# seanome/kmerseek

Hardware: AMD Instinct MI355X
Metric: k-mers hashed+matched/sec (higher is better)
Workload: dtype u64

## Files before the change

### include/kmerseek_amd.h

```cpp
#ifndef KMERSEEK_AMD_H
#define KMERSEEK_AMD_H

#include <stddef.h>
#include <stdint.h>

#ifdef __cplusplus
extern "C" {
#endif

#define KS_ABI_VERSION 1

typedef enum ks_status {
    KS_OK = 0,
    KS_ERR_INVALID_MOLTYPE = 1,
    KS_ERR_INVALID_KSIZE = 2,
    KS_ERR_INVALID_RESIDUE = 3,
    KS_ERR_INVALID_ARG = 4,
    KS_ERR_OOM = 5,
    KS_ERR_HIP = 6,
    KS_ERR_NO_DEVICE = 7,
    KS_ERR_CAPACITY = 8,
    KS_ERR_INVALID_SCALED = 9
} ks_status;

typedef enum ks_moltype { KS_PROTEIN = 0, KS_DAYHOFF = 1, KS_HP = 2 } ks_moltype;

#define KS_SEED_DEFAULT 42ull
#define KS_MAX_KSIZE 128u

typedef struct ks_params {
    uint32_t ksize;
    uint32_t scaled;
    uint32_t moltype;
    uint32_t flags;
    uint64_t seed;
} ks_params;

typedef struct ks_ctx ks_ctx;
typedef struct ks_sketches ks_sketches;
typedef struct ks_index ks_index;
typedef struct ks_hits ks_hits;
typedef struct ks_kmerpos ks_kmerpos;
typedef struct ks_matchpos ks_matchpos;
typedef struct ks_regions ks_regions;


uint32_t ks_abi_version(void);
const char *ks_status_string(int status);

int ks_moltype_from_string(const char *name, uint32_t *moltype_out);

uint64_t ks_max_hash(uint32_t scaled);

int ks_ctx_create(int device, void *hip_stream, ks_ctx **out);
void ks_ctx_destroy(ks_ctx *ctx);
const char *ks_last_error(const ks_ctx *ctx);
void *ks_ctx_stream(const ks_ctx *ctx);
int ks_ctx_synchronize(ks_ctx *ctx);
int ks_ctx_pool_stats(const ks_ctx *ctx, uint64_t *n_blocks, uint64_t *bytes_held, uint64_t *bytes_in_use,
                      uint64_t *n_mallocs);

int ks_ctx_sketch_stats(const ks_ctx *ctx, uint64_t out[4]);
int ks_ctx_search_stats(const ks_ctx *ctx, uint64_t out[2]);
int ks_ctx_fused_stats(const ks_ctx *ctx, uint64_t out[2]);
int ks_ctx_qfilter_stats(const ks_ctx *ctx, uint64_t out[2]);
int ks_ctx_reload_debug_env(ks_ctx *ctx);
int ks_debug_guard_selftest(const char *what);

int ks_dev_malloc(ks_ctx *ctx, uint64_t bytes, void **out);
int ks_dev_free(ks_ctx *ctx, void *ptr);
int ks_dev_upload(ks_ctx *ctx, void *dst_device, const void *src_host, uint64_t bytes);
int ks_dev_download(ks_ctx *ctx, void *dst_host, const void *src_device, uint64_t bytes);

int ks_host_alloc(ks_ctx *ctx, uint64_t bytes, void **out);
int ks_host_free(ks_ctx *ctx, void *ptr);


typedef struct ks_residue_error {
    uint32_t seq_index;
    uint32_t position;
    uint8_t residue;
} ks_residue_error;

int ks_validate_and_resolve(const uint8_t *seq, uint64_t len, int upper, uint64_t rng_seed,
                            uint8_t *out, uint64_t *out_len, ks_residue_error *err);


int ks_sketch_batch(ks_ctx *ctx, const uint8_t *residues, const uint64_t *seq_offsets,
                    uint32_t n_seqs, const ks_params *params, ks_sketches **out);

int ks_sketch_batch_device(ks_ctx *ctx, const uint8_t *d_residues, const uint64_t *d_seq_offsets,
                           uint32_t n_seqs, uint64_t n_residues, uint32_t max_seq_len,
                           const ks_params *params, ks_sketches **out);

int ks_sketch_queries_device(ks_ctx *ctx, const ks_index *index, const uint8_t *d_residues,
                             const uint64_t *d_seq_offsets, uint32_t n_seqs, uint64_t n_residues,
                             uint32_t max_seq_len, ks_sketches **out);

int ks_sketch_search_device(ks_ctx *ctx, const ks_index *index, const uint8_t *d_residues,
                            const uint64_t *d_seq_offsets, uint32_t n_seqs, uint64_t n_residues,
                            uint32_t max_seq_len, ks_sketches **sketches_out, ks_hits **hits_out);
int ks_sketch_search(ks_ctx *ctx, const ks_index *index, const uint8_t *residues, const uint64_t *seq_offsets,
                     uint32_t n_seqs, ks_sketches **sketches_out, ks_hits **hits_out);

uint32_t ks_sketches_n_seqs(const ks_sketches *s);
uint64_t ks_sketches_n_hashes(const ks_sketches *s);
uint64_t ks_sketches_n_windows(const ks_sketches *s);
int ks_sketches_has_postings(const ks_sketches *s);
void ks_sketches_params(const ks_sketches *s, ks_params *out);
const uint64_t *ks_sketches_device_offsets(const ks_sketches *s);
const uint64_t *ks_sketches_device_hashes(const ks_sketches *s);
const uint32_t *ks_sketches_device_abunds(const ks_sketches *s);
int ks_sketches_copy_to_host(ks_ctx *ctx, const ks_sketches *s, uint64_t *offsets,
                             uint64_t *hashes, uint32_t *abunds);
int ks_sketches_from_host(ks_ctx *ctx, const uint64_t *offsets, const uint64_t *hashes,
                          const uint32_t *abunds, uint32_t n_seqs, const ks_params *params,
                          ks_sketches **out);
int ks_sketches_union(ks_ctx *ctx, const ks_sketches *in, ks_sketches **out);
void ks_sketches_free(ks_sketches *s);


uint64_t ks_translate6_bound(uint64_t n_nt);
int ks_translate6_device(ks_ctx *ctx, const uint8_t *d_nt, const uint64_t *d_offsets, uint32_t n_seqs, uint64_t n_nt,
                         uint8_t *d_frames ,
                         uint64_t *d_frame_offsets , uint64_t *n_residues_out);
int ks_sketch_translated_device(ks_ctx *ctx, const uint8_t *d_nt, const uint64_t *d_offsets, uint32_t n_seqs, uint64_t n_nt,
                                uint32_t max_seq_len , const ks_params *params, ks_sketches **out);
int ks_sketch_translated(ks_ctx *ctx, const uint8_t *nt, const uint64_t *offsets, uint32_t n_seqs, const ks_params *params,
                         ks_sketches **out);
int ks_sketches_union_groups(ks_ctx *ctx, const ks_sketches *in, const uint32_t *group_offsets, uint32_t n_groups, ks_sketches **out);
uint32_t ks_debug_translate_chunk(void);
uint32_t ks_debug_union_rank_max(void);


int ks_kmer_positions(ks_ctx *ctx, const uint8_t *residues, const uint64_t *seq_offsets,
                      uint32_t n_seqs, const ks_params *params, ks_kmerpos **out);
int ks_kmer_positions_device(ks_ctx *ctx, const uint8_t *d_residues, const uint64_t *d_seq_offsets, uint32_t n_seqs,
                             uint64_t n_residues, const ks_params *params, ks_kmerpos **out);
uint64_t ks_kmerpos_count(const ks_kmerpos *p);
void ks_kmerpos_params(const ks_kmerpos *p, ks_params *out);
int ks_kmerpos_copy_to_host(ks_ctx *ctx, const ks_kmerpos *p, uint32_t *seq, uint32_t *start,
                            uint64_t *hash);
void ks_kmerpos_free(ks_kmerpos *p);


int ks_index_build(ks_ctx *ctx, const ks_sketches *targets, ks_index **out);
uint32_t ks_index_n_targets(const ks_index *ix);
uint64_t ks_index_n_postings(const ks_index *ix);
void ks_index_free(ks_index *ix);

int ks_search(ks_ctx *ctx, const ks_index *index, const ks_sketches *queries, ks_hits **out);
uint64_t ks_hits_count(const ks_hits *h);
uint64_t ks_hits_n_pair_instances(const ks_hits *h);
int ks_hits_partition_path(const ks_hits *h);
int ks_hits_bucket_posting_bytes(const ks_hits *h);
int ks_hits_copy_to_host(ks_ctx *ctx, const ks_hits *h, uint32_t *qid, uint32_t *tid,
                         uint32_t *intersect, uint64_t *n_weighted);
const uint32_t *ks_hits_device_qid(const ks_hits *h);
const uint32_t *ks_hits_device_tid(const ks_hits *h);
const uint32_t *ks_hits_device_intersect(const ks_hits *h);
const uint64_t *ks_hits_device_n_weighted(const ks_hits *h);
int ks_hits_copy_to_device(ks_ctx *ctx, const ks_hits *h, uint32_t qid_base, uint32_t tid_base, uint32_t *d_qid,
                           uint32_t *d_tid, uint32_t *d_intersect, uint64_t *d_n_weighted);
int ks_hits_pack64_to_device(ks_ctx *ctx, const ks_hits *h, uint32_t qid_base, uint32_t tid_base, int qbits, int tbits,
                             uint64_t *d_packed, uint32_t *d_esc_row, uint32_t *d_esc_intersect, uint64_t *d_esc_n_weighted,
                             uint32_t *d_n_esc, uint32_t esc_cap);
int ks_hits_unpack64_device(ks_ctx *ctx, const uint64_t *d_packed, uint64_t n, int qbits, int tbits, uint32_t *d_qid,
                            uint32_t *d_tid, uint32_t *d_intersect, uint64_t *d_n_weighted);
int ks_hits_merge_by_qid_device(ks_ctx *ctx, const uint32_t *d_qid, const uint32_t *d_tid, const uint32_t *d_intersect,
                                const uint64_t *d_n_weighted, const uint64_t *block_rows, uint32_t n_blocks, uint32_t n_queries,
                                uint32_t *d_out_qid, uint32_t *d_out_tid, uint32_t *d_out_intersect, uint64_t *d_out_n_weighted);
void ks_hits_free(ks_hits *h);


#define KS_SEARCH_ABUND_STATS 1u
typedef struct ks_search_opts {
    uint32_t flags;
    uint32_t reserved;
    double min_containment;
} ks_search_opts;
int ks_search_ex(ks_ctx *ctx, const ks_index *index, const ks_sketches *queries, const ks_search_opts *opts, ks_hits **out);
int ks_sketch_search_device_ex(ks_ctx *ctx, const ks_index *index, const uint8_t *d_residues, const uint64_t *d_seq_offsets,
                               uint32_t n_seqs, uint64_t n_residues, uint32_t max_seq_len, const ks_search_opts *opts,
                               ks_sketches **sketches_out, ks_hits **hits_out);
int ks_sketch_search_ex(ks_ctx *ctx, const ks_index *index, const uint8_t *residues, const uint64_t *seq_offsets,
                        uint32_t n_seqs, const ks_search_opts *opts, ks_sketches **sketches_out, ks_hits **hits_out);
int ks_hits_has_abund_stats(const ks_hits *h);
const uint64_t *ks_hits_device_median2(const ks_hits *h);
const double *ks_hits_device_abund_ss(const ks_hits *h);
int ks_hits_copy_abund_stats_to_host(ks_ctx *ctx, const ks_hits *h, uint64_t *median2, double *ss);


typedef struct ks_matchpos_opts {
    uint32_t flags;
    uint32_t reserved;
    uint64_t max_pairs;
} ks_matchpos_opts;
int ks_match_positions(ks_ctx *ctx, const ks_kmerpos *q_pos, const ks_kmerpos *t_pos, const ks_hits *hits,
                       const ks_matchpos_opts *opts, ks_matchpos **out);
uint64_t ks_matchpos_n_rows(const ks_matchpos *m);
uint64_t ks_matchpos_n_pairs(const ks_matchpos *m);
uint32_t ks_matchpos_n_slices(const ks_matchpos *m);
const uint64_t *ks_matchpos_device_row_offsets(const ks_matchpos *m);
const uint32_t *ks_matchpos_device_q_start(const ks_matchpos *m);
const uint32_t *ks_matchpos_device_t_start(const ks_matchpos *m);
const uint32_t *ks_matchpos_device_q_lo(const ks_matchpos *m);
const uint32_t *ks_matchpos_device_q_hi(const ks_matchpos *m);
const uint32_t *ks_matchpos_device_t_lo(const ks_matchpos *m);
const uint32_t *ks_matchpos_device_t_hi(const ks_matchpos *m);
int ks_matchpos_copy_to_host(ks_ctx *ctx, const ks_matchpos *m, uint64_t *row_offsets, uint32_t *q_start, uint32_t *t_start,
                             uint32_t *q_lo, uint32_t *q_hi, uint32_t *t_lo, uint32_t *t_hi);
void ks_matchpos_free(ks_matchpos *m);


typedef struct ks_regions_opts {
    uint32_t flags;
    uint32_t min_kmers;
// ... 129 lines not shown
```

### kmerseek_amd/_lib.py

```python
from __future__ import annotations

import ctypes as C
import os
import sys

HERE = os.path.dirname(os.path.abspath(__file__))
SO_PATH = os.environ.get("KMERSEEK_AMD_LIB") or os.path.join(HERE, "libkmerseek_amd.so")

KS_OK = 0
KS_ERR_INVALID_MOLTYPE = 1
KS_ERR_INVALID_KSIZE = 2
KS_ERR_INVALID_RESIDUE = 3
KS_ERR_INVALID_ARG = 4
KS_ERR_OOM = 5
KS_ERR_HIP = 6
KS_ERR_NO_DEVICE = 7
KS_ERR_CAPACITY = 8
KS_ERR_INVALID_SCALED = 9

KS_PROTEIN, KS_DAYHOFF, KS_HP = 0, 1, 2
KS_SEED_DEFAULT = 42


class ks_params(C.Structure):
    _fields_ = [("ksize", C.c_uint32), ("scaled", C.c_uint32), ("moltype", C.c_uint32),
                ("flags", C.c_uint32), ("seed", C.c_uint64)]


class ks_residue_error(C.Structure):
    _fields_ = [("seq_index", C.c_uint32), ("position", C.c_uint32), ("residue", C.c_uint8)]


KS_SEARCH_ABUND_STATS = 1


class ks_search_opts(C.Structure):
    _fields_ = [("flags", C.c_uint32), ("reserved", C.c_uint32), ("min_containment", C.c_double)]


class ks_matchpos_opts(C.Structure):
    _fields_ = [("flags", C.c_uint32), ("reserved", C.c_uint32), ("max_pairs", C.c_uint64)]


class ks_regions_opts(C.Structure):
    _fields_ = [("flags", C.c_uint32), ("min_kmers", C.c_uint32), ("max_gap", C.c_uint32), ("reserved", C.c_uint32)]


class ks_signif_opts(C.Structure):
    _fields_ = [("flags", C.c_uint32), ("reserved", C.c_uint32)]


KS_BEST_INTERSECT, KS_BEST_TARGET_CONTAINMENT, KS_BEST_MAX_CONTAINMENT, KS_BEST_JACCARD, KS_BEST_SCORE = 0, 1, 2, 3, 4


class ks_best_opts(C.Structure):
    _fields_ = [("rank_by", C.c_uint32), ("k", C.c_uint32), ("flags", C.c_uint32), ("reserved", C.c_uint32)]


class ks_cluster_opts(C.Structure):
    _fields_ = [("similarity", C.c_uint32), ("n_nodes", C.c_uint32), ("threshold", C.c_double), ("flags", C.c_uint32),
                ("reserved", C.c_uint32)]


KS_GREEDY_ASSIGN_FIRST, KS_GREEDY_ASSIGN_BEST = 0, 1


class ks_greedy_opts(C.Structure):
    _fields_ = [("similarity", C.c_uint32), ("n_nodes", C.c_uint32), ("threshold", C.c_double), ("assign", C.c_uint32),
                ("flags", C.c_uint32)]


class ks_gather_opts(C.Structure):
    _fields_ = [("min_unique", C.c_uint32), ("max_results", C.c_uint32), ("flags", C.c_uint32), ("reserved", C.c_uint32)]


class ks_kernel_time(C.Structure):
    _fields_ = [("name", C.c_char * 48), ("launches", C.c_uint64), ("total_ms", C.c_double)]


_vp = C.c_void_p
_u8p = C.POINTER(C.c_uint8)
_u32p = C.POINTER(C.c_uint32)
_u64p = C.POINTER(C.c_uint64)
_pp = C.POINTER(C.c_void_p)
_parp = C.POINTER(ks_params)

SIGNATURES = {
    "ks_abi_version": (C.c_uint32, []),
    "ks_status_string": (C.c_char_p, [C.c_int]),
    "ks_moltype_from_string": (C.c_int, [C.c_char_p, _u32p]),
    "ks_max_hash": (C.c_uint64, [C.c_uint32]),
    "ks_ctx_create": (C.c_int, [C.c_int, _vp, _pp]),
    "ks_ctx_destroy": (None, [_vp]),
    "ks_last_error": (C.c_char_p, [_vp]),
    "ks_ctx_stream": (_vp, [_vp]),
    "ks_ctx_synchronize": (C.c_int, [_vp]),
    "ks_ctx_sketch_stats": (C.c_int, [_vp, C.POINTER(C.c_uint64 * 4)]),
    "ks_ctx_search_stats": (C.c_int, [_vp, C.POINTER(C.c_uint64 * 2)]),
    "ks_ctx_fused_stats": (C.c_int, [_vp, C.POINTER(C.c_uint64 * 2)]),
    "ks_ctx_qfilter_stats": (C.c_int, [_vp, C.POINTER(C.c_uint64 * 2)]),
    "ks_ctx_reload_debug_env": (C.c_int, [_vp]),
    "ks_debug_guard_selftest": (C.c_int, [C.c_char_p]),
    "ks_host_alloc": (C.c_int, [_vp, C.c_uint64, _pp]),
    "ks_host_free": (C.c_int, [_vp, _vp]),
    "ks_dev_malloc": (C.c_int, [_vp, C.c_uint64, _pp]),
    "ks_dev_free": (C.c_int, [_vp, _vp]),
    "ks_dev_upload": (C.c_int, [_vp, _vp, _vp, C.c_uint64]),
    "ks_dev_download": (C.c_int, [_vp, _vp, _vp, C.c_uint64]),
    "ks_ctx_pool_stats": (C.c_int, [_vp, _u64p, _u64p, _u64p, _u64p]),
    "ks_validate_and_resolve": (C.c_int, [C.c_char_p, C.c_uint64, C.c_int, C.c_uint64, C.c_char_p, _u64p,
                                          C.POINTER(ks_residue_error)]),
    "ks_sketch_batch": (C.c_int, [_vp, _vp, _vp, C.c_uint32, _parp, _pp]),
    "ks_sketch_batch_device": (C.c_int, [_vp, _vp, _vp, C.c_uint32, C.c_uint64, C.c_uint32, _parp, _pp]),
    "ks_sketch_queries_device": (C.c_int, [_vp, _vp, _vp, _vp, C.c_uint32, C.c_uint64, C.c_uint32, _pp]),
    "ks_sketch_search_device": (C.c_int, [_vp, _vp, _vp, _vp, C.c_uint32, C.c_uint64, C.c_uint32, _pp, _pp]),
    "ks_sketch_search": (C.c_int, [_vp, _vp, _vp, _vp, C.c_uint32, _pp, _pp]),
    "ks_sketches_has_postings": (C.c_int, [_vp]),
    "ks_sketches_n_seqs": (C.c_uint32, [_vp]),
    "ks_sketches_n_hashes": (C.c_uint64, [_vp]),
    "ks_sketches_n_windows": (C.c_uint64, [_vp]),
    "ks_sketches_params": (None, [_vp, _parp]),
    "ks_sketches_device_offsets": (_vp, [_vp]),
    "ks_sketches_device_hashes": (_vp, [_vp]),
    "ks_sketches_device_abunds": (_vp, [_vp]),
    "ks_sketches_copy_to_host": (C.c_int, [_vp, _vp, _vp, _vp, _vp]),
    "ks_sketches_from_host": (C.c_int, [_vp, _vp, _vp, _vp, C.c_uint32, _parp, _pp]),
    "ks_sketches_union": (C.c_int, [_vp, _vp, _pp]),
    "ks_sketches_free": (None, [_vp]),
    "ks_translate6_bound": (C.c_uint64, [C.c_uint64]),
    "ks_translate6_device": (C.c_int, [_vp, _vp, _vp, C.c_uint32, C.c_uint64, _vp, _vp, _u64p]),
    "ks_sketch_translated_device": (C.c_int, [_vp, _vp, _vp, C.c_uint32, C.c_uint64, C.c_uint32, _parp, _pp]),
    "ks_sketch_translated": (C.c_int, [_vp, _vp, _vp, C.c_uint32, _parp, _pp]),
    "ks_sketches_union_groups": (C.c_int, [_vp, _vp, _u32p, C.c_uint32, _pp]),
    "ks_debug_translate_chunk": (C.c_uint32, []),
    "ks_debug_union_rank_max": (C.c_uint32, []),
    "ks_kmer_positions": (C.c_int, [_vp, _vp, _vp, C.c_uint32, _parp, _pp]),
    "ks_kmer_positions_device": (C.c_int, [_vp, _vp, _vp, C.c_uint32, C.c_uint64, _parp, _pp]),
    "ks_kmerpos_count": (C.c_uint64, [_vp]),
    "ks_kmerpos_params": (None, [_vp, _parp]),
    "ks_kmerpos_copy_to_host": (C.c_int, [_vp, _vp, _vp, _vp, _vp]),
    "ks_kmerpos_free": (None, [_vp]),
    "ks_index_build": (C.c_int, [_vp, _vp, _pp]),
    "ks_index_n_targets": (C.c_uint32, [_vp]),
    "ks_index_n_postings": (C.c_uint64, [_vp]),
    "ks_index_free": (None, [_vp]),
    "ks_search": (C.c_int, [_vp, _vp, _vp, _pp]),
    "ks_hits_count": (C.c_uint64, [_vp]),
    "ks_hits_n_pair_instances": (C.c_uint64, [_vp]),
    "ks_hits_partition_path": (C.c_int, [_vp]),
    "ks_hits_bucket_posting_bytes": (C.c_int, [_vp]),
    "ks_hits_copy_to_host": (C.c_int, [_vp, _vp, _vp, _vp, _vp, _vp]),
    "ks_hits_device_qid": (_vp, [_vp]),
    "ks_hits_device_tid": (_vp, [_vp]),
    "ks_hits_device_intersect": (_vp, [_vp]),
    "ks_hits_device_n_weighted": (_vp, [_vp]),
    "ks_hits_copy_to_device": (C.c_int, [_vp, _vp, C.c_uint32, C.c_uint32, _vp, _vp, _vp, _vp]),
    "ks_hits_pack64_to_device": (C.c_int, [_vp, _vp, C.c_uint32, C.c_uint32, C.c_int, C.c_int, _vp, _vp, _vp, _vp, _vp, C.c_uint32]),
    "ks_hits_unpack64_device": (C.c_int, [_vp, _vp, C.c_uint64, C.c_int, C.c_int, _vp, _vp, _vp, _vp]),
    "ks_hits_merge_by_qid_device": (C.c_int, [_vp, _vp, _vp, _vp, _vp, C.POINTER(C.c_uint64), C.c_uint32, C.c_uint32, _vp, _vp, _vp, _vp]),
    "ks_hits_free": (None, [_vp]),
    "ks_search_ex": (C.c_int, [_vp, _vp, _vp, C.POINTER(ks_search_opts), _pp]),
    "ks_sketch_search_device_ex": (C.c_int, [_vp, _vp, _vp, _vp, C.c_uint32, C.c_uint64, C.c_uint32, C.POINTER(ks_search_opts), _pp,
                                             _pp]),
    "ks_sketch_search_ex": (C.c_int, [_vp, _vp, _vp, _vp, C.c_uint32, C.POINTER(ks_search_opts), _pp, _pp]),
    "ks_hits_has_abund_stats": (C.c_int, [_vp]),
    "ks_hits_device_median2": (_vp, [_vp]),
    "ks_hits_device_abund_ss": (_vp, [_vp]),
    "ks_hits_copy_abund_stats_to_host": (C.c_int, [_vp, _vp, _vp, _vp]),
    "ks_match_positions": (C.c_int, [_vp, _vp, _vp, _vp, C.POINTER(ks_matchpos_opts), _pp]),
    "ks_matchpos_n_rows": (C.c_uint64, [_vp]),
    "ks_matchpos_n_pairs": (C.c_uint64, [_vp]),
    "ks_matchpos_n_slices": (C.c_uint32, [_vp]),
    "ks_matchpos_device_row_offsets": (_vp, [_vp]),
    "ks_matchpos_device_q_start": (_vp, [_vp]),
    "ks_matchpos_device_t_start": (_vp, [_vp]),
    "ks_matchpos_device_q_lo": (_vp, [_vp]),
    "ks_matchpos_device_q_hi": (_vp, [_vp]),
    "ks_matchpos_device_t_lo": (_vp, [_vp]),
    "ks_matchpos_device_t_hi": (_vp, [_vp]),
    "ks_matchpos_copy_to_host": (C.c_int, [_vp, _vp, _vp, _vp, _vp, _vp, _vp, _vp, _vp]),
    "ks_matchpos_free": (None, [_vp]),
    "ks_match_regions": (C.c_int, [_vp, _vp, C.POINTER(ks_regions_opts), _pp]),
    "ks_regions_n_rows": (C.c_uint64, [_vp]),
    "ks_regions_n_regions": (C.c_uint64, [_vp]),
    "ks_regions_n_slices": (C.c_uint32, [_vp]),
    "ks_regions_device_row_offsets": (_vp, [_vp]),
    "ks_regions_device_q_start": (_vp, [_vp]),
    "ks_regions_device_t_start": (_vp, [_vp]),
    "ks_regions_device_length": (_vp, [_vp]),
    "ks_regions_device_n_kmers": (_vp, [_vp]),
    "ks_regions_device_covered": (_vp, [_vp]),
    "ks_regions_copy_to_host": (C.c_int, [_vp, _vp, _vp, _vp, _vp, _vp, _vp, _vp]),
    "ks_regions_free": (None, [_vp]),
    "ks_corpus_build": (C.c_int, [_vp, _vp, _pp]),
    "ks_corpus_n_hashes": (C.c_uint64, [_vp]),
    "ks_corpus_n_docs": (C.c_uint32, [_vp]),
    "ks_corpus_total_abund": (C.c_uint64, [_vp]),
    "ks_corpus_copy_to_host": (C.c_int, [_vp, _vp, _vp, _vp, _vp]),
    "ks_corpus_free": (None, [_vp]),
    "ks_hits_significance": (C.c_int, [_vp, _vp, _vp, _vp, _vp, _vp, C.POINTER(ks_signif_opts), _pp]),
    "ks_signif_n_rows": (C.c_uint64, [_vp]),
    "ks_signif_device_prob_overlap": (_vp, [_vp]),
    "ks_signif_device_tf_idf": (_vp, [_vp]),
    "ks_signif_copy_to_host": (C.c_int, [_vp, _vp, _vp, _vp]),
    "ks_signif_free": (None, [_vp]),
    "ks_hits_best": (C.c_int, [_vp, _vp, _vp, _vp, _vp, C.POINTER(ks_best_opts), _pp]),
    "ks_hits_device_rank": (_vp, [_vp]),
    "ks_hits_device_src_row": (_vp, [_vp]),
    "ks_hits_copy_best_to_host": (C.c_int, [_vp, _vp, _vp, _vp]),
    "ks_hits_gather": (C.c_int, [_vp, _vp, _vp, _vp, C.POINTER(ks_gather_opts), _pp]),
    "ks_hits_device_unique_intersect": (_vp, [_vp]),
    "ks_hits_device_remaining": (_vp, [_vp]),
    "ks_hits_device_unique_weighted": (_vp, [_vp]),
    "ks_hits_copy_gather_to_host": (C.c_int, [_vp, _vp, _vp, _vp, _vp]),
    "ks_hits_cluster": (C.c_int, [_vp, _vp, _vp, _vp, C.POINTER(ks_cluster_opts), _pp]),
    "ks_clusters_n_nodes": (C.c_uint32, [_vp]),
    "ks_clusters_n_clusters": (C.c_uint32, [_vp]),
    "ks_clusters_n_edges": (C.c_uint64, [_vp]),
    "ks_clusters_largest": (C.c_uint32, [_vp]),
    "ks_clusters_device_label": (_vp, [_vp]),
    "ks_clusters_device_cluster_id": (_vp, [_vp]),
    "ks_clusters_device_offsets": (_vp, [_vp]),
    "ks_clusters_device_members": (_vp, [_vp]),
    "ks_clusters_device_representative": (_vp, [_vp]),
    "ks_clusters_copy_to_host": (C.c_int, [_vp, _vp, _vp, _vp, _vp, _vp, _vp]),
    "ks_clusters_free": (None, [_vp]),
    "ks_hits_cluster_greedy": (C.c_int, [_vp, _vp, _vp, _vp, C.POINTER(ks_greedy_opts), _pp]),
    "ks_clusters_n_rounds": (C.c_uint32, [_vp]),
    "ks_debug_greedy_tail_edges": (C.c_uint32, []),
    "ks_timing_enable": (C.c_int, [_vp, C.c_int]),
    "ks_timing_reset": (C.c_int, [_vp]),
    "ks_timing_get": (C.c_int, [_vp, C.POINTER(ks_kernel_time), C.c_uint32, _u32p]),
    "ks_bench_gather_rates": (C.c_int, [_vp, C.POINTER(C.c_double * 2)]),
    "ks_bench_device_rates": (C.c_int, [_vp, C.POINTER(C.c_double), C.POINTER(C.c_double), C.POINTER(C.c_double)]),
}

_lib = None


class KmerseekLibraryError(RuntimeError):
    pass


def load():
    global _lib
    if _lib is not None:
        return _lib
    if not os.path.exists(SO_PATH):
        raise KmerseekLibraryError(
            f"{SO_PATH} not found: build it with `python -m kmerseek_amd.build` (hipcc, gfx950). "
            "There is no CPU fallback.")
    if "torch" not in sys.modules and os.environ.get("KS_NO_TORCH_PRELOAD") != "1":
# ... 18 lines not shown
```

### kmerseek_amd/csrc/ks_api.hip

```cpp
#include "ks_device.h"

extern "C" int ks_sketch_batch_device(ks_ctx *ctx, const uint8_t *d_residues, const uint64_t *d_seq_offsets,
                                      uint32_t n_seqs, uint64_t n_residues, uint32_t max_seq_len,
                                      const ks_params *params, ks_sketches **out) {
    return ks_guard(ctx, [&]() -> int {
    if (!ctx) return KS_ERR_INVALID_ARG;
    if (!out || (!d_seq_offsets) || (!d_residues && n_residues)) return ks_fail(ctx, KS_ERR_INVALID_ARG, "NULL argument");
    return ks_sketch_device_impl(ctx, d_residues, d_seq_offsets, n_seqs, n_residues, max_seq_len, params, 0, 0, 0, out);
    });
}

extern "C" int ks_sketch_queries_device(ks_ctx *ctx, const ks_index *index, const uint8_t *d_residues,
                                        const uint64_t *d_seq_offsets, uint32_t n_seqs, uint64_t n_residues,
                                        uint32_t max_seq_len, ks_sketches **out) {
    return ks_guard(ctx, [&]() -> int {
    if (!ctx) return KS_ERR_INVALID_ARG;
    if (!index || !out || (!d_seq_offsets) || (!d_residues && n_residues)) return ks_fail(ctx, KS_ERR_INVALID_ARG, "NULL argument");
    return ks_sketch_device_impl(ctx, d_residues, d_seq_offsets, n_seqs, n_residues, max_seq_len, &index->params,
                                 index->pbits, (index->fp_layout && index->fp_shift == 32 - index->pbits) ? 1 : 0, 0, out);
    });
}

struct ks_upload {
    ks_ctx *ctx;
// ... 133 lines not shown
    return ks_guard(ctx, [&]() -> int {
    if (!ctx) return KS_ERR_INVALID_ARG;
    if (!offsets || !out) return ks_fail(ctx, KS_ERR_INVALID_ARG, "NULL argument");
    KS_TRY(ks_check_params(ctx, params));
    if (offsets[0] != 0) return ks_fail(ctx, KS_ERR_INVALID_ARG, "offsets[0] must be 0");
    const u64 n = offsets[n_seqs];
    if (n && (!hashes || !abunds)) return ks_fail(ctx, KS_ERR_INVALID_ARG, "hashes/abunds is NULL");
    const u64 max_hash = ks_max_hash(params->scaled);
    for (u32 s = 0; s < n_seqs; s++) {
        if (offsets[s + 1] < offsets[s]) return ks_fail(ctx, KS_ERR_INVALID_ARG, "offsets must be ascending");
        for (u64 j = offsets[s]; j < offsets[s + 1]; j++) {
            if (hashes[j] == 0 || hashes[j] > max_hash)
                return ks_fail(ctx, KS_ERR_INVALID_ARG, "sketch %u holds hash %llu outside (0, max_hash(scaled=%u)]", s,
                               (unsigned long long)hashes[j], params->scaled);
            if (j > offsets[s] && hashes[j] <= hashes[j - 1])
                return ks_fail(ctx, KS_ERR_INVALID_ARG, "sketch %u is not strictly ascending", s);
        }
    }
    KS_HIP(ctx, hipSetDevice(ctx->device));
    ks_result<ks_sketches> S(ctx, out, ks_sketches_free);
    S->params = *params; S->n_seqs = n_seqs; S->n_hashes = S->n_slots = n;
    KS_TRY(ks_alloc(ctx, &S->d_offsets, (size_t)n_seqs + 1));
    KS_TRY(ks_alloc(ctx, &S->d_hashes, (size_t)n));
    KS_TRY(ks_alloc(ctx, &S->d_abunds, (size_t)n));
    KS_HIP(ctx, hipMemcpyAsync(S->d_offsets, offsets, ((size_t)n_seqs + 1) * sizeof(u64), hipMemcpyHostToDevice, ctx->stream));
    if (n) {
        KS_HIP(ctx, hipMemcpyAsync(S->d_hashes, hashes, (size_t)n * sizeof(u64), hipMemcpyHostToDevice, ctx->stream));
        KS_HIP(ctx, hipMemcpyAsync(S->d_abunds, abunds, (size_t)n * sizeof(u32), hipMemcpyHostToDevice, ctx->stream));
    }
    KS_HIP(ctx, hipStreamSynchronize(ctx->stream));
    return S.commit();
    });
}

extern "C" int ks_sketches_union(ks_ctx *ctx, const ks_sketches *in, ks_sketches **out) {
    return ks_guard(ctx, [&]() -> int {
    if (!ctx) return KS_ERR_INVALID_ARG;
    return ks_union_impl(ctx, in, out);
    });
}

extern "C" void ks_sketches_free(ks_sketches *s) {
    if (!s) return;
    ks_pool_free(s->ctx, s->d_offsets);
    ks_pool_free(s->ctx, s->d_hashes);
    ks_pool_free(s->ctx, s->d_abunds);
    ks_pool_free(s->ctx, s->d_counts);
    ks_pool_free(s->ctx, s->part_keys);
    ks_pool_free(s->ctx, s->part_vals);
    if (s->ctl_block) ks_pool_free(s->ctx, s->ctl_block);
    else ks_pool_free(s->ctx, s->part_len);
    delete s;
}

int ks_kmerpos_device_impl(ks_ctx *ctx, const u8 *d_res, const u64 *d_offs, u32 n_seqs, u64 n_res, const ks_params *p,
                           ks_kmerpos **out) {
    KS_TRY(ks_check_params(ctx, p));
    if (((uintptr_t)d_res & 15) != 0) return ks_fail(ctx, KS_ERR_INVALID_ARG, "d_residues must be 16-byte aligned");
    KS_HIP(ctx, hipSetDevice(ctx->device));
    ks_result<ks_kmerpos> K(ctx, out, ks_kmerpos_free);
    K->params = *p; K->n_seqs = n_seqs;
    const size_t cap = (n_res == 0 || n_seqs == 0) ? 1 : (size_t)n_res;
    KS_TRY(ks_alloc(ctx, &K->d_seq, cap));
    KS_TRY(ks_alloc(ctx, &K->d_start, cap));
    KS_TRY(ks_alloc(ctx, &K->d_hash, cap));
    if (n_res != 0 && n_seqs != 0)
        KS_TRY(ks_kmerpos_tiles_launch(ctx, d_res, d_offs, n_seqs, n_res, p, K->d_seq, K->d_start, K->d_hash, &K->n));
    return K.commit();
}

extern "C" int ks_kmer_positions(ks_ctx *ctx, const uint8_t *residues, const uint64_t *seq_offsets, uint32_t n_seqs,
                                 const ks_params *params, ks_kmerpos **out) {
    return ks_guard(ctx, [&]() -> int {
    if (!ctx) return KS_ERR_INVALID_ARG;
    if (!out) return ks_fail(ctx, KS_ERR_INVALID_ARG, "out is NULL");
    KS_TRY(ks_check_params(ctx, params));
    ks_upload U(ctx);
    KS_TRY(U.upload(residues, seq_offsets, n_seqs));
    return ks_kmerpos_device_impl(ctx, U.d_res, U.d_offs, n_seqs, U.n_res, params, out);
    });
}

extern "C" int ks_kmer_positions_device(ks_ctx *ctx, const uint8_t *d_residues, const uint64_t *d_seq_offsets, uint32_t n_seqs,
                                        uint64_t n_residues, const ks_params *params, ks_kmerpos **out) {
    return ks_guard(ctx, [&]() -> int {
    if (!ctx) return KS_ERR_INVALID_ARG;
    if (!out) return ks_fail(ctx, KS_ERR_INVALID_ARG, "out is NULL");
    if (n_seqs && (!d_seq_offsets || (n_residues && !d_residues))) return ks_fail(ctx, KS_ERR_INVALID_ARG, "NULL device buffer");
    return ks_kmerpos_device_impl(ctx, d_residues, d_seq_offsets, n_seqs, n_residues, params, out);
    });
}

extern "C" uint64_t ks_kmerpos_count(const ks_kmerpos *p) { return p ? p->n : 0; }
extern "C" void ks_kmerpos_params(const ks_kmerpos *p, ks_params *out) { if (p && out) *out = p->params; }

extern "C" int ks_kmerpos_copy_to_host(ks_ctx *ctx, const ks_kmerpos *p, uint32_t *seq, uint32_t *start, uint64_t *hash) {
    return ks_guard(ctx, [&]() -> int {
    if (!ctx || !p) return KS_ERR_INVALID_ARG;
    const size_t n = (size_t)p->n;
    return ks_columns_to_host(ctx, {{seq, p->d_seq, n * sizeof(u32)}, {start, p->d_start, n * sizeof(u32)}, {hash, p->d_hash, n * sizeof(u64)}});
    });
}

extern "C" void ks_kmerpos_free(ks_kmerpos *p) {
    if (!p) return;
    ks_pool_free(p->ctx, p->d_seq);
    ks_pool_free(p->ctx, p->d_start);
    ks_pool_free(p->ctx, p->d_hash);
    delete p;
}

extern "C" int ks_index_build(ks_ctx *ctx, const ks_sketches *targets, ks_index **out) {
    return ks_guard(ctx, [&]() -> int {
    if (!ctx) return KS_ERR_INVALID_ARG;
    return ks_index_build_impl(ctx, targets, out);
    });
}
extern "C" uint32_t ks_index_n_targets(const ks_index *ix) { return ix ? ix->n_targets : 0; }
extern "C" uint64_t ks_index_n_postings(const ks_index *ix) { return ix ? ix->n_postings : 0; }
extern "C" void ks_index_free(ks_index *ix) {
    if (!ix) return;
    ks_pool_free(ix->ctx, ix->d_keys);
    ks_pool_free(ix->ctx, ix->d_tids);
    ks_pool_free(ix->ctx, ix->d_abunds);
    ks_pool_free(ix->ctx, ix->d_fp);
    ks_pool_free(ix->ctx, ix->d_post);
    ks_pool_free(ix->ctx, ix->d_bmeta);
    ks_pool_free(ix->ctx, ix->d_presence);
    ks_pool_free(ix->ctx, ix->d_dir);
    delete ix;
}

extern "C" int ks_search(ks_ctx *ctx, const ks_index *index, const ks_sketches *queries, ks_hits **out) {
    return ks_guard(ctx, [&]() -> int {
    if (!ctx) return KS_ERR_INVALID_ARG;
    return ks_search_impl(ctx, index, queries, out);
    });
}
extern "C" int ks_search_ex(ks_ctx *ctx, const ks_index *index, const ks_sketches *queries, const ks_search_opts *opts, ks_hits **out) {
    return ks_guard(ctx, [&]() -> int {
    KS_TRY(ks_search_opts_check(ctx, opts));
    if (!ctx) return KS_ERR_INVALID_ARG;
    return ks_search_impl(ctx, index, queries, out, nullptr, opts);
    });
}
static int sketch_search_impl(ks_ctx *ctx, const ks_index *index, const uint8_t *d_residues, const uint64_t *d_seq_offsets, uint32_t n_seqs,
                              uint64_t n_residues, uint32_t max_seq_len, const ks_search_opts *opts, ks_sketches **sketches_out,
                              ks_hits **hits_out) {
    *hits_out = nullptr;
    if (sketches_out) *sketches_out = nullptr;
    const int fmt10 = (index->fp_layout && index->fp_shift == 32 - index->pbits) ? 1 : 0;
    ks_sketches *S = nullptr;
    ks_hits *H = nullptr;
    int st = ks_sketch_device_impl(ctx, d_residues, d_seq_offsets, n_seqs, n_residues, max_seq_len, &index->params, index->pbits, fmt10,
                                   ks_dbg(ctx, KS_DBG_NO_DEFER) ? 0 : 1, &S);
    if (st != KS_OK) return st;
    const bool deferred = S->pending != 0;
    int redo = 0;
    st = ks_search_impl(ctx, index, S, &H, &redo, opts);
    if (S->pending) {
        const ks_fetch_seg f = ks_sketch_pending_seg(S);
        int r2 = 0;
        int st2 = ks_stream_wait_fetch(ctx, &f, 1);
        if (st2 == KS_OK) st2 = ks_sketch_finish_pending(S, &r2);
        if (st == KS_OK) { st = st2; redo = r2; }
    }
    if (st == KS_OK && redo) {
        ks_hits_free(H); H = nullptr;
        ks_sketches_free(S); S = nullptr;
        ctx->fused_redos++;
        st = ks_sketch_device_impl(ctx, d_residues, d_seq_offsets, n_seqs, n_residues, max_seq_len, &index->params, index->pbits, fmt10, 0, &S);
        if (st == KS_OK) st = ks_search_impl(ctx, index, S, &H, nullptr, opts);
    }
    if (st != KS_OK) { ks_hits_free(H); ks_sketches_free(S); return st; }
    if (deferred) ctx->fused_deferred++;
    *hits_out = H;
    if (sketches_out) *sketches_out = S; else ks_sketches_free(S);
    return KS_OK;
}

extern "C" int ks_sketch_search_device_ex(ks_ctx *ctx, const ks_index *index, const uint8_t *d_residues,
                                          const uint64_t *d_seq_offsets, uint32_t n_seqs, uint64_t n_residues,
                                          uint32_t max_seq_len, const ks_search_opts *opts, ks_sketches **sketches_out,
                                          ks_hits **hits_out) {
    return ks_guard(ctx, [&]() -> int {
    KS_TRY(ks_search_opts_check(ctx, opts));
    if (!ctx) return KS_ERR_INVALID_ARG;
    if (!index || !hits_out || (!d_seq_offsets) || (!d_residues && n_residues)) return ks_fail(ctx, KS_ERR_INVALID_ARG, "NULL argument");
    return sketch_search_impl(ctx, index, d_residues, d_seq_offsets, n_seqs, n_residues, max_seq_len, opts, sketches_out, hits_out);
    });
}
extern "C" int ks_sketch_search_device(ks_ctx *ctx, const ks_index *index, const uint8_t *d_residues,
                                       const uint64_t *d_seq_offsets, uint32_t n_seqs, uint64_t n_residues,
                                       uint32_t max_seq_len, ks_sketches **sketches_out, ks_hits **hits_out) {
    return ks_guard(ctx, [&]() -> int {
    return ks_sketch_search_device_ex(ctx, index, d_residues, d_seq_offsets, n_seqs, n_residues, max_seq_len, nullptr, sketches_out,
                                      hits_out);
    });
}

extern "C" int ks_sketch_search_ex(ks_ctx *ctx, const ks_index *index, const uint8_t *residues, const uint64_t *seq_offsets,
                                   uint32_t n_seqs, const ks_search_opts *opts, ks_sketches **sketches_out, ks_hits **hits_out) {
    return ks_guard(ctx, [&]() -> int {
    KS_TRY(ks_search_opts_check(ctx, opts));
    if (!ctx) return KS_ERR_INVALID_ARG;
    if (!index || !hits_out) return ks_fail(ctx, KS_ERR_INVALID_ARG, "NULL argument");
    ks_upload U(ctx);
    KS_TRY(U.upload(residues, seq_offsets, n_seqs));
    return sketch_search_impl(ctx, index, U.d_res, U.d_offs, n_seqs, U.n_res, U.max_len, opts, sketches_out, hits_out);
    });
}
extern "C" int ks_sketch_search(ks_ctx *ctx, const ks_index *index, const uint8_t *residues, const uint64_t *seq_offsets,
                                uint32_t n_seqs, ks_sketches **sketches_out, ks_hits **hits_out) {
    return ks_guard(ctx, [&]() -> int {
    return ks_sketch_search_ex(ctx, index, residues, seq_offsets, n_seqs, nullptr, sketches_out, hits_out);
    });
}
extern "C" uint64_t ks_hits_count(const ks_hits *h) { return h ? h->n_hits : 0; }
extern "C" uint64_t ks_hits_n_pair_instances(const ks_hits *h) { return h ? h->n_pair_instances : 0; }
extern "C" int ks_hits_partition_path(const ks_hits *h) {
    return ks_guard(nullptr, [&]() -> int { return h ? h->partition_path : -1; 
    });
}
extern "C" int ks_hits_bucket_posting_bytes(const ks_hits *h) {
    return ks_guard(nullptr, [&]() -> int { return h ? h->bucket_posting_bytes : -1;
    });
}
extern "C" int ks_hits_copy_to_host(ks_ctx *ctx, const ks_hits *h, uint32_t *qid, uint32_t *tid, uint32_t *intersect,
                                    uint64_t *n_weighted) {
    return ks_guard(ctx, [&]() -> int {
    if (!ctx || !h) return KS_ERR_INVALID_ARG;
    const size_t n = (size_t)h->n_hits;
    return ks_columns_to_host(ctx, {{qid, h->d_qid, n * sizeof(u32)}, {tid, h->d_tid, n * sizeof(u32)},
                                    {intersect, h->d_isect, n * sizeof(u32)}, {n_weighted, h->d_nw, n * sizeof(u64)}});
    });
}
extern "C" const uint32_t *ks_hits_device_qid(const ks_hits *h) { return h ? h->d_qid : nullptr; }
extern "C" const uint32_t *ks_hits_device_tid(const ks_hits *h) { return h ? h->d_tid : nullptr; }
extern "C" const uint32_t *ks_hits_device_intersect(const ks_hits *h) { return h ? h->d_isect : nullptr; }
extern "C" const uint64_t *ks_hits_device_n_weighted(const ks_hits *h) { return h ? h->d_nw : nullptr; }

__global__ __launch_bounds__(256) void k_copy_add_u32(const u32 *in, u32 *out, u64 n, u32 add) {
    const u64 i = (u64)blockIdx.x * blockDim.x + threadIdx.x;
    if (i < n) out[i] = in[i] + add;
}

extern "C" int ks_hits_copy_to_device(ks_ctx *ctx, const ks_hits *h, uint32_t qid_base, uint32_t tid_base, uint32_t *d_qid,
                                      uint32_t *d_tid, uint32_t *d_intersect, uint64_t *d_n_weighted) {
    return ks_guard(ctx, [&]() -> int {
    if (!ctx || !h) return KS_ERR_INVALID_ARG;
    KS_HIP(ctx, hipSetDevice(ctx->device));
    const u64 n = h->n_hits;
    if (n == 0) return KS_OK;
    const u32 g = (u32)((n + 255) / 256);
    if (d_qid) KS_LAUNCH(ctx, "hits_copy", k_copy_add_u32, g, 256, (const u32 *)h->d_qid, d_qid, n, qid_base);
    if (d_tid) KS_LAUNCH(ctx, "hits_copy", k_copy_add_u32, g, 256, (const u32 *)h->d_tid, d_tid, n, tid_base);
    if (d_intersect) KS_HIP(ctx, hipMemcpyAsync(d_intersect, h->d_isect, (size_t)n * sizeof(u32), hipMemcpyDeviceToDevice, ctx->stream));
    if (d_n_weighted) KS_HIP(ctx, hipMemcpyAsync(d_n_weighted, h->d_nw, (size_t)n * sizeof(u64), hipMemcpyDeviceToDevice, ctx->stream));
    return KS_OK;
    });
}

__global__ __launch_bounds__(256) void k_hits_pack64(const u32 *qid, const u32 *tid, const u32 *isect, const u64 *nw, u64 n, u32 qid_base,
                                                     u32 tid_base, int qbits, int tbits, int vbits, u64 *packed, u32 *esc_row, u32 *esc_isect,
                                                     u64 *esc_nw, u32 *n_esc, u32 esc_cap) {
    const u64 i = (u64)blockIdx.x * blockDim.x + threadIdx.x;
    if (i >= n) return;
    const u64 vmax = (1ULL << vbits) - 1ULL;
    u64 a = isect[i], b = nw[i];
    if (a >= vmax || b >= vmax) {
        const u32 e = atomicAdd(n_esc, 1u);
        if (e < esc_cap) { esc_row[e] = (u32)i; esc_isect[e] = (u32)a; esc_nw[e] = b; }
        a = vmax; b = vmax;
    }
    const u64 q = (u64)qid[i] + qid_base, t = (u64)tid[i] + tid_base;
    if ((q >> qbits) != 0 || (t >> tbits) != 0) atomicOr(n_esc, 0x80000000u);
    packed[i] = (((q << tbits) | t) << (2 * vbits)) | (a << vbits) | b;
}

extern "C" int ks_hits_pack64_to_device(ks_ctx *ctx, const ks_hits *h, uint32_t qid_base, uint32_t tid_base, int qbits, int tbits,
                                        uint64_t *d_packed, uint32_t *d_esc_row, uint32_t *d_esc_intersect, uint64_t *d_esc_n_weighted,
                                        uint32_t *d_n_esc, uint32_t esc_cap) {
    return ks_guard(ctx, [&]() -> int {
    if (!ctx || !h) return KS_ERR_INVALID_ARG;
    if (qbits < 1 || tbits < 1 || qbits + tbits > 48) return ks_fail(ctx, KS_ERR_INVALID_ARG, "pack64: %d + %d id bits leave fewer than 8 value bits", qbits, tbits);
    KS_HIP(ctx, hipSetDevice(ctx->device));
    const u64 n = h->n_hits;
    if (!d_n_esc) return ks_fail(ctx, KS_ERR_INVALID_ARG, "NULL argument");
    KS_HIP(ctx, hipMemsetAsync(d_n_esc, 0, sizeof(u32), ctx->stream));
    if (n == 0) return KS_OK;
    if (n >= 0xffffffffULL) return ks_fail(ctx, KS_ERR_CAPACITY, "pack64: %llu rows (escape rows are 32-bit indices)", (unsigned long long)n);
    if (!d_packed || (esc_cap && (!d_esc_row || !d_esc_intersect || !d_esc_n_weighted))) return ks_fail(ctx, KS_ERR_INVALID_ARG, "NULL argument");
    KS_LAUNCH(ctx, "hits_pack", k_hits_pack64, (u32)((n + 255) / 256), 256, (const u32 *)h->d_qid, (const u32 *)h->d_tid, (const u32 *)h->d_isect,
              (const u64 *)h->d_nw, n, qid_base, tid_base, qbits, tbits, (64 - qbits - tbits) / 2, d_packed, d_esc_row, d_esc_intersect, d_esc_n_weighted,
              d_n_esc, esc_cap);
    return KS_OK;
    });
}

__global__ __launch_bounds__(256) void k_hits_unpack64(const u64 *packed, u64 n, int qbits, int tbits, int vbits, u32 *qid, u32 *tid,
                                                       u32 *isect, u64 *nw) {
    const u64 i = (u64)blockIdx.x * blockDim.x + threadIdx.x;
    if (i >= n) return;
    const u64 w = packed[i], vmax = (1ULL << vbits) - 1ULL;
    qid[i] = (u32)((w >> (tbits + 2 * vbits)) & ((1ULL << qbits) - 1ULL));
    tid[i] = (u32)((w >> (2 * vbits)) & ((1ULL << tbits) - 1ULL));
    isect[i] = (u32)((w >> vbits) & vmax);
    nw[i] = w & vmax;
}

extern "C" int ks_hits_unpack64_device(ks_ctx *ctx, const uint64_t *d_packed, uint64_t n, int qbits, int tbits, uint32_t *d_qid,
                                       uint32_t *d_tid, uint32_t *d_intersect, uint64_t *d_n_weighted) {
    return ks_guard(ctx, [&]() -> int {
    if (!ctx) return KS_ERR_INVALID_ARG;
    if (qbits < 1 || tbits < 1 || qbits + tbits > 48) return ks_fail(ctx, KS_ERR_INVALID_ARG, "unpack64: %d + %d id bits leave fewer than 8 value bits", qbits, tbits);
    if (n == 0) return KS_OK;
    if (!d_packed || !d_qid || !d_tid || !d_intersect || !d_n_weighted) return ks_fail(ctx, KS_ERR_INVALID_ARG, "NULL argument");
    if (n > 0xffffffffULL * 256ULL) return ks_fail(ctx, KS_ERR_INVALID_ARG, "unpack64: too many rows");
    KS_HIP(ctx, hipSetDevice(ctx->device));
    KS_LAUNCH(ctx, "hits_unpack", k_hits_unpack64, (u32)((n + 255) / 256), 256, (const u64 *)d_packed, n, qbits, tbits, (64 - qbits - tbits) / 2,
              d_qid, d_tid, d_intersect, (u64 *)d_n_weighted);
    return KS_OK;
    });
}

struct hm_blocks { u64 base[65]; u32 n; };

__global__ __launch_bounds__(256) void k_hm_starts(const u32 *qid, hm_blocks B, u32 nq, u32 *first) {
// ... 99 lines not shown
```

### kmerseek_amd/csrc/ks_common.h

```cpp
#pragma once

#include <hip/hip_runtime.h>

#include <cstdint>
#include <cstdio>
#include <cstring>
#include <functional>
#include <initializer_list>
#include <new>
#include <stdexcept>
#include <string>
#include <vector>

#include "../../include/kmerseek_amd.h"

typedef uint8_t u8;
typedef uint16_t u16;
typedef uint32_t u32;
typedef uint64_t u64;
typedef int32_t i32;
typedef int64_t i64;

#define KS_WAVE 64

struct ks_pool_block {
    void *ptr;
    size_t size;
    bool in_use;
};

struct ks_timer_slot {
    hipEvent_t a, b;
    int name_id;
};

struct ks_copy_engine;

#define KS_DBG_LIST(X)                                                                                                   \
    X(STAGED_H2D) X(PLAIN_COPIES) X(PAIRS_LSD) X(MSD_LDS_CAP) X(SCAN_3PASS) X(INDEX_LSD) X(JOIN_FP) X(FP_COARSEN)        \
    X(PAIR_LIMIT) X(PBITS_MAX) X(RECORD_BITS) X(ONE_CURSOR) X(JOIN_SEGS) X(JOIN_SEG_CAP) X(JOIN_SPARSE)                \
    X(NO_ROWS_HINT) X(ROWS_TICKET) X(FORCE_ROWS_TICKET_RETRY) X(FORCE_TICKET_RETRY) X(NO_PLAN) X(NO_COMPACT) X(SPAN)      \
    X(NO_PACK) X(PLAN_SYNC) X(TILE_R) X(OUT_CAP) X(POOL_CAP) X(THROW) X(QCAP) X(LOOKBACK_SKIP) X(SYNC_API) X(POSTINGS12) X(POSTINGS10) X(NO_DEFER) X(BUCKET) X(JOIN_SPLIT) X(SUBSHIFT) X(MATCHPOS_ROW_BITS) X(SIGNIF_WAVE_ROWS) X(BEST_PATH) X(REGIONS_ROW_BITS) X(QFILTER) X(QFILTER_OCC) X(CLUSTER_PATH) X(GATHER_PATH) X(GREEDY_PATH) X(UNION_PATH)
enum ks_dbg_id {
#define KS_DBG_ENUM(n) KS_DBG_##n,
    KS_DBG_LIST(KS_DBG_ENUM)
#undef KS_DBG_ENUM
    KS_DBG_COUNT
};
struct ks_debug {
    bool set[KS_DBG_COUNT];
    char val[KS_DBG_COUNT][32];
};
void ks_debug_load(ks_debug *d);

struct ks_ctx {
    int device = 0;
    ks_copy_engine *copy = nullptr;
    hipStream_t stream = nullptr;
    bool own_stream = false;
    int n_cus = 256;
    ks_debug dbg;
    u64 pool_cap = 0;
    std::string err;
    std::vector<ks_pool_block> pool;
    u64 pool_mallocs = 0;
    int timing = 0;
    std::vector<std::string> t_names;
    std::vector<u64> t_launches;
    std::vector<double> t_ms;
    std::vector<ks_timer_slot> t_pending;
    std::vector<std::pair<hipEvent_t, hipEvent_t>> t_free;
    bool t_open = false;
    u64 *h_pin = nullptr;
    u64 pair_cap_hint = 0;
    u64 rows_hint = 0;
    bool sketch_use_ticket = false;
    u64 sketch_ticket_fallbacks = 0, sketch_compact_fallbacks = 0, sketch_cap_fallbacks = 0;
    bool rows_use_ticket = false; u64 rows_ticket_fallbacks = 0;
    u64 fused_deferred = 0, fused_redos = 0;
    u64 join_retries = 0;
    bool qfilter_pays = true;
    u64 qfilter_seen = 0, qfilter_dropped = 0;
    unsigned long long *scan_ring = nullptr;
    u32 *scan_ticket = nullptr;
    u32 scan_ticket_base = 0;
    u8 *d_lut = nullptr;
    unsigned long long *h_flag = nullptr;
    unsigned long long wait_seq = 0;
};

int ks_stream_wait(ks_ctx *ctx);
#define KS_FETCH_MAX 4
struct ks_fetch_seg {
    const void *src;
    u32 *dst;
    u32 rows, row_words, src_stride;
};
static inline ks_fetch_seg ks_fetch_words(const void *src, void *dst, u32 n_words32) { return ks_fetch_seg{src, (u32 *)dst, 1u, n_words32, n_words32}; }
int ks_stream_wait_fetch(ks_ctx *ctx, const ks_fetch_seg *segs, int n);

void *ks_pool_alloc(ks_ctx *ctx, size_t bytes);
void ks_pool_free(ks_ctx *ctx, void *ptr);
void ks_pool_trim(ks_ctx *ctx);

int ks_fail(ks_ctx *ctx, int status, const char *fmt, ...);
static inline const char *ks_dbg(const ks_ctx *ctx, int id) { return (ctx && ctx->dbg.set[id]) ? ctx->dbg.val[id] : nullptr; }

int ks_guard_fail(ks_ctx *ctx, int status, const char *what) noexcept;
void ks_guard_enter(ks_ctx *ctx);
template <typename F>
static inline int ks_guard(ks_ctx *ctx, F &&body) noexcept {
    try {
        ks_guard_enter(ctx);
        return body();
    } catch (const std::bad_alloc &) {
        return ks_guard_fail(ctx, KS_ERR_OOM, "out of host memory (std::bad_alloc)");
    } catch (const std::exception &e) {
        return ks_guard_fail(ctx, KS_ERR_HIP, e.what());
    } catch (...) {
        return ks_guard_fail(ctx, KS_ERR_HIP, "unknown exception");
    }
}

void ks_timer_begin(ks_ctx *ctx, const char *name);
void ks_timer_end(ks_ctx *ctx);

#define KS_HIP(ctx, expr)                                                                          \
    do {                                                                                           \
        hipError_t e__ = (expr);                                                                   \
        if (e__ != hipSuccess)                                                                     \
            return ks_fail(ctx, KS_ERR_HIP, "%s failed: %s (%s:%d)", #expr, hipGetErrorString(e__), \
                           __FILE__, __LINE__);                                                    \
    } while (0)

#define KS_TRY(expr)                        \
    do {                                    \
        int s__ = (expr);                   \
        if (s__ != KS_OK) return s__;       \
    } while (0)

#define KS_LAUNCH(ctx, name, kernel, grid, block, ...)                                   \
    do {                                                                                 \
        ks_timer_begin(ctx, name);                                                       \
        hipLaunchKernelGGL(kernel, dim3(grid), dim3(block), 0, (ctx)->stream, __VA_ARGS__); \
        ks_timer_end(ctx);                                                               \
        KS_HIP(ctx, hipGetLastError());                                                  \
    } while (0)

template <typename T>
static inline int ks_alloc(ks_ctx *ctx, T **out, size_t count) {
    void *p = ks_pool_alloc(ctx, (count ? count : 1) * sizeof(T));
    if (!p) return KS_ERR_OOM;
    *out = (T *)p;
    return KS_OK;
}

struct ks_scratch {
    ks_ctx *ctx;
    void *blk[16];
    int n = 0;
    explicit ks_scratch(ks_ctx *c) : ctx(c) {}
    ks_scratch(const ks_scratch &) = delete;
    ~ks_scratch() { for (int i = 0; i < n; i++) ks_pool_free(ctx, blk[i]); }
    template <typename T> int alloc(T **out, size_t count) {
        if (n == 16) return ks_fail(ctx, KS_ERR_HIP, "internal error: scratch table full");
        KS_TRY(ks_alloc(ctx, out, count));
        blk[n++] = *out;
        return KS_OK;
    }
    void free(void *p) { if (forget(p)) ks_pool_free(ctx, p); }
    template <typename T> T *keep(T *p) { forget(p); return p; }
    bool forget(void *p) {
        for (int i = 0; p && i < n; i++)
            if (blk[i] == p) { blk[i] = blk[--n]; return true; }
        return false;
    }
};

struct ks_ctl {
    u64 *dev = nullptr;
    u64 *host = nullptr;
    u32 n_words = 0;
    int init(ks_ctx *ctx, ks_scratch &sc, u32 pin_slot, u32 n_bad, u32 n_count) {
        n_words = n_bad + n_count;
        host = ctx->h_pin + pin_slot;
        KS_TRY(sc.alloc(&dev, n_words));
        KS_HIP(ctx, hipMemsetAsync(dev, 0xff, n_bad * sizeof(u64), ctx->stream));
        KS_HIP(ctx, hipMemsetAsync(dev + n_bad, 0, n_count * sizeof(u64), ctx->stream));
        return KS_OK;
    }
    unsigned long long *words() const { return (unsigned long long *)dev; }
    u32 *low32(u32 i) const { return (u32 *)(dev + i); }
    ks_fetch_seg fetch() const { return ks_fetch_words(dev, host, 2 * n_words); }
    u64 operator[](u32 i) const { return host[i]; }
    bool bad(u32 i) const { return host[i] != ~0ULL; }
};

template <typename T>
struct ks_result {
    T *obj = nullptr;
    T **out;
    void (*free_fn)(T *);
    ks_result(ks_ctx *ctx, T **out_, void (*f)(T *)) : out(out_), free_fn(f) {
        *out = nullptr;
        obj = new T();
        obj->ctx = ctx;
    }
    ks_result(const ks_result &) = delete;
    ~ks_result() {
        if (!obj) return;
        (void)hipStreamSynchronize(obj->ctx->stream);
        free_fn(obj);
    }
    T *operator->() const { return obj; }
    operator T *() const { return obj; }
    int commit() { *out = obj; obj = nullptr; return KS_OK; }
};

struct ks_sketches {
    ks_ctx *ctx;
    ks_params params;
    u32 n_seqs;
    u64 n_hashes;
    u64 n_windows;
    u64 *d_offsets;
    u64 *d_hashes;
    u32 *d_abunds;
    u32 *d_counts;
    u64 n_slots;
    bool gapped;
    u64 *part_keys;
    u32 *part_vals;
    u32 *part_len;
// ... 46 lines not shown
};

struct __attribute__((aligned(16))) ks_bmeta {
    u64 base;
    u32 slot_mul;
    u32 pad;
};

struct ks_index {
    ks_ctx *ctx;
    ks_params params;
    u32 n_targets;
    u64 n_postings;
    u64 *d_keys;
    u32 *d_tids;
    u32 *d_abunds;
    u32 *d_fp;
    ks_post *d_post;
    ks_bmeta *d_bmeta;
    bool fp_layout;
    int fp_shift;
    u32 max_abund;
    u64 *d_dir;
    int pbits;
    u32 *d_presence;
    u32 pres_K;
    int pres_bits;
};

struct ks_hits {
    ks_ctx *ctx;
    u64 n_hits;
    u64 n_pair_instances;
    int partition_path;
    int bucket_posting_bytes;
    u32 *d_qid, *d_tid, *d_isect;
    u64 *d_nw;
    u64 *d_block;
    bool has_stats;
    u64 *d_median2;
    double *d_ss;
    u32 *d_rank, *d_src_row;
    u32 *d_ga_unique, *d_ga_remaining;
    u64 *d_ga_weighted;
};

struct ks_kmerpos {
    ks_ctx *ctx;
    ks_params params;
    u32 n_seqs;
    u64 n;
    u32 *d_seq, *d_start;
    u64 *d_hash;
};

struct ks_matchpos {
    ks_ctx *ctx;
    ks_params params;
    u64 n_rows, n_pairs;
    u32 n_slices;
    u32 max_qs, max_ts;
    u64 *d_row_offsets;
    u32 *d_qstart, *d_tstart;
    u32 *d_qlo, *d_qhi, *d_tlo, *d_thi;
};

struct ks_regions {
    ks_ctx *ctx;
    u64 n_rows, n_regions;
    u32 n_slices;
    u64 *d_row_offsets;
    u32 *d_qstart, *d_tstart, *d_length, *d_nkmers, *d_covered;
};

struct ks_clusters {
    ks_ctx *ctx;
    u32 n_nodes, n_clusters, largest;
    u64 n_edges;
    u32 n_rounds;
    u32 *d_label, *d_cluster_id, *d_members, *d_rep;
    u64 *d_offsets;
};
enum { CL_BAD_ID = 0, CL_BAD_SIZE = 1, CL_EDGES = 2, CL_CLUSTERS = 3, CL_LARGEST = 4 };
int ks_clusters_alloc(ks_ctx *ctx, ks_clusters *K, u32 n);
struct ks_label_scratch { u32 *root_idx, *sizes; u64 *rep, *ka, *kb; };
int ks_clusters_from_labels(ks_ctx *ctx, ks_clusters *K, const ks_sketches *nodes, const ks_label_scratch &W, const ks_ctl &ctl);
int ks_clusters_finish(ks_ctx *ctx, const char *what, ks_clusters *K, const ks_ctl &ctl);
int ks_cluster_words_check(ks_ctx *ctx, const char *what, u32 similarity, u32 n_nodes, double threshold, const ks_sketches *nodes,
                           const double *d_score);

struct ks_slice_fmt {
    int pt, pqt;
    u32 row0, slice_rows;
};
struct ks_row_slices {
    u64 per_slice, n_slices;
    int low_bits;
    ks_slice_fmt fmt(u64 s, u64 n_rows, int pt) const {
        ks_slice_fmt F;
        F.pt = pt; F.pqt = low_bits;
        F.row0 = (u32)(s * per_slice);
        F.slice_rows = (u32)(n_rows - F.row0 < per_slice ? n_rows - F.row0 : per_slice);
        return F;
    }
};
int ks_key_bits(u64 v);
int ks_row_slices_plan(ks_ctx *ctx, int dbg_id, const char *what, int low_bits, u64 n_rows, ks_row_slices *out);
int ks_sort_live_keys(ks_ctx *ctx, u64 *ka, u64 *kb, u64 n, int nbits, u64 **sorted);

enum : u32 { KS_COLS_RANKED = 1u, KS_COLS_GATHER = 2u };
int ks_hits_alloc_cols(ks_ctx *ctx, ks_hits *H, size_t n, u32 extra);
void ks_hits_inherit(ks_hits *B, const ks_hits *H);
#define KS_RANK_NONE 0xffffffffu
struct ks_gather_cols { const u32 *unique, *remaining; const u64 *weighted; };
int ks_hits_move_ranked(ks_ctx *ctx, const ks_hits *H, u32 n_rows, const u32 *dst, const u32 *rank, u32 cap, ks_hits *B,
                        const ks_gather_cols *ga);
int ks_hits_select_plan(ks_ctx *ctx, const char *what, const ks_hits *H, const ks_sketches *Q, u32 per_query, u32 *n, u64 *cap);
int ks_hits_select_tail(ks_ctx *ctx, const char *what, const ks_hits *H, u32 n_rows, u32 *flags, const u32 *rank, u64 cap,
                        const ks_gather_cols *ga, const ks_ctl &ctl, u32 kept, const std::function<int()> &checks, ks_hits *B);

int ks_scan_u32_to_u64(ks_ctx *ctx, const u32 *in, u64 *out, u64 n);
int ks_scan_status_fetch(ks_ctx *ctx);
int ks_scan_status_check(ks_ctx *ctx);
int ks_stream_wait_fetch_scans(ks_ctx *ctx, std::initializer_list<ks_fetch_seg> segs);
int ks_scan_u32_inplace(ks_ctx *ctx, u32 *data, u64 n, u32 *d_total);

enum { KS_SORT_INDEX = 0, KS_SORT_QPART = 1, KS_SORT_PAIRS = 2 };
struct ks_rs_segments {
    const u32 *len;
    u64 cap;
    u32 regions;
    u32 sub_shift;
};
int ks_radix_sort_u32(ks_ctx *ctx, int tag, const u64 *keys_in, const u32 *vals_in, u64 *ka, u32 *va, u64 *kb, u32 *vb,
                      u64 n, const int *shifts, int n_shifts, u64 **keys_out, u32 **vals_out,
                      const ks_rs_segments *seg = nullptr, u32 pfxK = 0);
int ks_radix_sort_keys(ks_ctx *ctx, int tag, const u64 *keys_in, u64 *ka, u64 *kb, u64 n, const int *shifts, int n_shifts,
                       u64 **keys_out);
#define KS_BSLOT(d, r, n_hi) ((r) * (n_hi) + (d))
#define KS_QF_KEPT 1
int ks_bucket_scatter_u32(ks_ctx *ctx, const u64 *keys_in, const u32 *vals_in, const ks_rs_segments *seg, int shift,
                          u32 pfxK, u64 *bkeys, u32 *bvals, u32 *bcur, u32 bcap, unsigned long long *status, u32 n_hi, int vfmt,
                          const u32 *presence, u32 presK, u32 fix_s);
int ks_index_sort_partitioned(ks_ctx *ctx, const u64 *keys_in, const u64 *vals_in, u64 n, u64 max_hash, u64 *okeys, u32 *otids,
                              u32 *oabunds, u32 *d_max_abund, int *overflowed);
#define KS_MSD_MAX_SEGS 64
struct ks_msd_segs {
    u32 n;
    u32 tile_start[KS_MSD_MAX_SEGS + 1];
    u32 count[KS_MSD_MAX_SEGS];
    u64 seg_cap;
};
int ks_sort_pairs_msd(ks_ctx *ctx, u64 *ka, u64 *kb, u64 n, int lo_bit, int nbits, int *done, const ks_msd_segs *segs = nullptr);
int ks_radix_sort_u64(ks_ctx *ctx, int tag, const u64 *keys_in, const u64 *vals_in, u64 *ka, u64 *va, u64 *kb, u64 *vb,
                      u64 n, const int *shifts, int n_shifts, u64 **keys_out, u64 **vals_out);

struct ks_runs { u64 *keys; u32 *vals; u64 *row_start; u32 n_rows; };
int ks_sorted_runs(ks_ctx *ctx, const ks_sketches *in, ks_scratch &sc, ks_runs *out);
int ks_row_list_alloc(ks_ctx *ctx, ks_scratch &sc, size_t n_rows, u32 **list);
int ks_seg_list_alloc(ks_ctx *ctx, ks_scratch &sc, size_t cap, u32 **list);
int ks_seg_path_knob(const ks_ctx *ctx, int dbg_id, bool *small);
struct ks_rows_in { const ks_sketches *q; u64 n_pairs; int tbits, abits; bool stats; double min_c; };
int ks_search_rows(ks_ctx *ctx, const ks_rows_in &R, ks_hits *H, const u64 *pk);

int ks_sketch_device_impl(ks_ctx *ctx, const u8 *d_res, const u64 *d_offs, u32 n_seqs, u64 n_res,
                          u32 max_seq_len, const ks_params *p, int part_pbits, int part_fmt10, int allow_defer, ks_sketches **out);
int ks_sketch_finish_pending(ks_sketches *S, int *redo);
ks_fetch_seg ks_sketch_pending_seg(const ks_sketches *S);
int ks_join_pbits(const ks_ctx *ctx, u64 n_postings, u64 per_bucket);
u32 ks_join_prefix_mul(int pbits, u64 max_hash);
struct sk_args;
struct ks_deferred { u32 *med_ids, *long_ids, *n_cls; u64 *lg_hash; u32 *lg_abund; };
int ks_sketch_long_launch(ks_ctx *ctx, const sk_args &A, const ks_deferred &D, u64 n_long, u32 max_len, ks_scratch &sc);
int ks_sketch_place_launch(ks_ctx *ctx, const sk_args &A, const ks_deferred &D, u64 n_med, u64 n_long);
int ks_kmerpos_tiles_launch(ks_ctx *ctx, const u8 *d_res, const u64 *d_offs, u32 n_seqs, u64 n_res, const ks_params *p, u32 *d_seq,
                            u32 *d_start, u64 *d_hash, u64 *n_out);
int ks_kmerpos_device_impl(ks_ctx *ctx, const u8 *d_res, const u64 *d_offs, u32 n_seqs, u64 n_res,
                           const ks_params *p, ks_kmerpos **out);
int ks_index_build_impl(ks_ctx *ctx, const ks_sketches *t, ks_index **out);
int ks_search_impl(ks_ctx *ctx, const ks_index *ix, const ks_sketches *q, ks_hits **out, int *sketch_redo = nullptr,
                   const ks_search_opts *opts = nullptr);
int ks_search_opts_check(ks_ctx *ctx, const ks_search_opts *opts);
int ks_union_impl(ks_ctx *ctx, const ks_sketches *in, ks_sketches **out);
int ks_union_groups_impl(ks_ctx *ctx, const ks_sketches *in, const u32 *group_offsets, u32 n_groups, ks_sketches **out);
int ks_sketch_translated_impl(ks_ctx *ctx, const u8 *d_nt, const u64 *d_offs, u32 n_seqs, u64 n_nt, u32 max_seq_len, const ks_params *p,
                              ks_sketches **out);

int ks_check_params(ks_ctx *ctx, const ks_params *p);
bool ks_same_params(const ks_params &a, const ks_params &b);
int ks_params_check_same(ks_ctx *ctx, const char *pass, const char *noun, const ks_params &a, const ks_params &b);
template <typename... In>
static inline int ks_inputs_check_ctx(ks_ctx *ctx, const char *pass, const In *...in) {
    if (((!in || in->ctx == ctx) && ...)) return KS_OK;
    return ks_fail(ctx, KS_ERR_INVALID_ARG, "%s: an input of another context", pass);
}
int ks_opts_words_check(ks_ctx *ctx, const char *what, u32 flags, u32 allowed, u32 reserved);
int ks_sketches_make_dense(ks_ctx *ctx, ks_sketches *s);

int ks_copy_h2d(ks_ctx *ctx, void *dst_device, const void *src_host, size_t bytes);
int ks_copy_d2h(ks_ctx *ctx, void *dst_host, const void *src_device, size_t bytes);
struct ks_column { void *dst; const void *src; size_t bytes; };
int ks_columns_to_host(ks_ctx *ctx, std::initializer_list<ks_column> cols);
void ks_copy_engine_destroy(ks_ctx *ctx);
```

### kmerseek_amd/csrc/ks_ctx.hip

```cpp
#include <cstdarg>
#include <algorithm>

#include "ks_common.h"

int ks_fail(ks_ctx *ctx, int status, const char *fmt, ...) {
    char buf[512];
    va_list ap;
    va_start(ap, fmt);
    vsnprintf(buf, sizeof buf, fmt, ap);
    va_end(ap);
    if (ctx) {
        try { ctx->err = buf; } catch (...) { }
    }
    return status;
}

extern "C" uint32_t ks_abi_version(void) { return KS_ABI_VERSION; }

extern "C" const char *ks_status_string(int s) {
    switch (s) {
    case KS_OK: return "ok";
    case KS_ERR_INVALID_MOLTYPE: return "invalid moltype";
    case KS_ERR_INVALID_KSIZE: return "invalid k-mer size";
    case KS_ERR_INVALID_RESIDUE: return "invalid amino acid";
// ... 60 lines not shown
                case 'C': e = 'a'; break;
                case 'A': case 'G': case 'P': case 'S': case 'T': e = 'b'; break;
                case 'D': case 'E': case 'N': case 'Q': e = 'c'; break;
                case 'H': case 'K': case 'R': e = 'd'; break;
                case 'I': case 'L': case 'M': case 'V': e = 'e'; break;
                case 'F': case 'W': case 'Y': e = 'f'; break;
                default: e = 'X';
                }
            } else if (m == KS_HP) {
                switch (c) {
                case 'A': case 'F': case 'G': case 'I': case 'L': case 'M': case 'P': case 'V':
                case 'W': case 'Y': e = 'h'; break;
                case 'N': case 'C': case 'S': case 'T': case 'D': case 'E': case 'R': case 'H':
                case 'K': case 'Q': e = 'p'; break;
                default: e = 'X';
                }
            }
            lut[m * 256 + b] = e;
        }
}

void ks_debug_load(ks_debug *d) {
    static const char *const names[KS_DBG_COUNT] = {
#define KS_DBG_NAME(n) "KS_DEBUG_" #n,
        KS_DBG_LIST(KS_DBG_NAME)
#undef KS_DBG_NAME
    };
    for (int i = 0; i < KS_DBG_COUNT; i++) {
        const char *v = getenv(names[i]);
        d->set[i] = v != nullptr;
        d->val[i][0] = 0;
        if (v) { strncpy(d->val[i], v, sizeof d->val[i] - 1); d->val[i][sizeof d->val[i] - 1] = 0; }
    }
}
static void debug_apply(ks_ctx *ctx) {
    ks_debug_load(&ctx->dbg);
    const char *cap = ks_dbg(ctx, KS_DBG_POOL_CAP);
    ctx->pool_cap = cap ? strtoull(cap, nullptr, 10) : 0;
}
extern "C" int ks_ctx_reload_debug_env(ks_ctx *ctx) {
    if (!ctx) return KS_ERR_INVALID_ARG;
    debug_apply(ctx);
    return KS_OK;
}

int ks_guard_fail(ks_ctx *ctx, int status, const char *what) noexcept {
    if (ctx) {
        try {
            ctx->err.assign(status == KS_ERR_OOM ? "" : "internal error: ");
            ctx->err.append(what ? what : "?");
        } catch (...) {
        }
    }
    return status;
}
void ks_guard_enter(ks_ctx *ctx) {
    const char *t = ks_dbg(ctx, KS_DBG_THROW);
    if (!t) return;
    if (!strcmp(t, "bad_alloc")) throw std::bad_alloc();
    if (!strcmp(t, "runtime")) throw std::runtime_error("KS_DEBUG_THROW");
    if (!strcmp(t, "other")) throw 42;
}

extern "C" int ks_debug_guard_selftest(const char *what) {
    return ks_guard(nullptr, [&]() -> int {
        if (what && !strcmp(what, "bad_alloc")) { std::vector<char> v; v.reserve((size_t)-1 / 2); }
        if (what && !strcmp(what, "runtime")) throw std::runtime_error("selftest");
        if (what && !strcmp(what, "other")) throw 42;
        return KS_OK;
    });
}

extern "C" int ks_ctx_create(int device, void *hip_stream, ks_ctx **out) {
    if (!out) return KS_ERR_INVALID_ARG;
    *out = nullptr;
    int n = 0;
    if (hipGetDeviceCount(&n) != hipSuccess || n <= 0) return KS_ERR_NO_DEVICE;
    if (device < 0 || device >= n) return KS_ERR_INVALID_ARG;
    ks_ctx *ctx = new (std::nothrow) ks_ctx();
    if (!ctx) return KS_ERR_OOM;
    ctx->device = device;
    try { ctx->err.reserve(640); ctx->pool.reserve(256); } catch (...) { delete ctx; return KS_ERR_OOM; }
    debug_apply(ctx);
    if (hipSetDevice(device) != hipSuccess) { delete ctx; return KS_ERR_HIP; }
    hipDeviceProp_t prop;
    if (hipGetDeviceProperties(&prop, device) == hipSuccess) ctx->n_cus = prop.multiProcessorCount;
    if (hip_stream) {
        ctx->stream = (hipStream_t)hip_stream;
    } else {
        if (hipStreamCreateWithFlags(&ctx->stream, hipStreamNonBlocking) != hipSuccess) { delete ctx; return KS_ERR_HIP; }
        ctx->own_stream = true;
    }
    if (hipHostMalloc((void **)&ctx->h_pin, KS_PIN_WORDS * sizeof(u64), hipHostMallocCoherent) != hipSuccess) { delete ctx; return KS_ERR_HIP; }
    if (hipHostMalloc((void **)&ctx->h_flag, 64, hipHostMallocCoherent) != hipSuccess) { (void)hipGetLastError(); ctx->h_flag = nullptr; }
    else *ctx->h_flag = 0;
    if (hipMalloc((void **)&ctx->d_lut, 3 * 256) != hipSuccess) { delete ctx; return KS_ERR_OOM; }
    u8 lut[768];
    build_luts(lut);
    if (hipMemcpy(ctx->d_lut, lut, sizeof lut, hipMemcpyHostToDevice) != hipSuccess) { delete ctx; return KS_ERR_HIP; }
    *out = ctx;
    return KS_OK;
}

extern "C" void ks_ctx_destroy(ks_ctx *ctx) {
    if (!ctx) return;
    (void)hipSetDevice(ctx->device);
    (void)hipStreamSynchronize(ctx->stream);
    ks_copy_engine_destroy(ctx);
    for (auto &t : ctx->t_pending) { (void)hipEventDestroy(t.a); (void)hipEventDestroy(t.b); }
    for (auto &t : ctx->t_free) { (void)hipEventDestroy(t.first); (void)hipEventDestroy(t.second); }
    for (auto &b : ctx->pool) (void)hipFree(b.ptr);
    if (ctx->d_lut) (void)hipFree(ctx->d_lut);
    if (ctx->h_pin) (void)hipHostFree(ctx->h_pin);
    if (ctx->h_flag) (void)hipHostFree(ctx->h_flag);
    if (ctx->scan_ring) (void)hipFree(ctx->scan_ring);
    if (ctx->scan_ticket) (void)hipFree(ctx->scan_ticket);
    if (ctx->own_stream) (void)hipStreamDestroy(ctx->stream);
    delete ctx;
}

extern "C" const char *ks_last_error(const ks_ctx *ctx) { return ctx ? ctx->err.c_str() : "no context"; }
extern "C" void *ks_ctx_stream(const ks_ctx *ctx) { return ctx ? (void *)ctx->stream : nullptr; }
extern "C" int ks_ctx_synchronize(ks_ctx *ctx) {
    return ks_guard(ctx, [&]() -> int {
    if (!ctx) return KS_ERR_INVALID_ARG;
    KS_HIP(ctx, hipStreamSynchronize(ctx->stream));
    return KS_OK;
    });
}

extern "C" int ks_ctx_pool_stats(const ks_ctx *ctx, uint64_t *n_blocks, uint64_t *bytes_held, uint64_t *bytes_in_use,
                                 uint64_t *n_mallocs) {
    return ks_guard((ks_ctx *)ctx, [&]() -> int {
    if (!ctx) return KS_ERR_INVALID_ARG;
    u64 held = 0, used = 0;
    for (auto &b : ctx->pool) { held += b.size; if (b.in_use) used += b.size; }
    if (n_blocks) *n_blocks = ctx->pool.size();
    if (bytes_held) *bytes_held = held;
    if (bytes_in_use) *bytes_in_use = used;
    if (n_mallocs) *n_mallocs = ctx->pool_mallocs;
    return KS_OK;
    });
}

extern "C" int ks_ctx_sketch_stats(const ks_ctx *ctx, uint64_t out[4]) {
    return ks_guard((ks_ctx *)ctx, [&]() -> int {
    if (!ctx || !out) return KS_ERR_INVALID_ARG;
    out[0] = ctx->sketch_ticket_fallbacks; out[1] = ctx->sketch_use_ticket ? 1 : 0;
    out[2] = ctx->sketch_compact_fallbacks; out[3] = ctx->sketch_cap_fallbacks;
    return KS_OK;
    });
}

extern "C" int ks_ctx_search_stats(const ks_ctx *ctx, uint64_t out[2]) {
    return ks_guard((ks_ctx *)ctx, [&]() -> int {
    if (!ctx || !out) return KS_ERR_INVALID_ARG;
    out[0] = ctx->join_retries; out[1] = ctx->rows_ticket_fallbacks;
    return KS_OK;
    });
}

extern "C" int ks_ctx_qfilter_stats(const ks_ctx *ctx, uint64_t out[2]) {
    return ks_guard((ks_ctx *)ctx, [&]() -> int {
    if (!ctx || !out) return KS_ERR_INVALID_ARG;
    out[0] = ctx->qfilter_seen; out[1] = ctx->qfilter_dropped;
    return KS_OK;
    });
}

extern "C" int ks_ctx_fused_stats(const ks_ctx *ctx, uint64_t out[2]) {
    return ks_guard((ks_ctx *)ctx, [&]() -> int {
    if (!ctx || !out) return KS_ERR_INVALID_ARG;
    out[0] = ctx->fused_deferred; out[1] = ctx->fused_redos;
    return KS_OK;
    });
}

extern "C" int ks_dev_malloc(ks_ctx *ctx, uint64_t bytes, void **out) {
    return ks_guard(ctx, [&]() -> int {
    if (!ctx || !out) return KS_ERR_INVALID_ARG;
    KS_HIP(ctx, hipSetDevice(ctx->device));
    if (hipMalloc(out, bytes ? bytes : 256) != hipSuccess) { (void)hipGetLastError(); return ks_fail(ctx, KS_ERR_OOM, "hipMalloc(%llu) failed", (unsigned long long)bytes); }
    return KS_OK;
    });
}
extern "C" int ks_dev_free(ks_ctx *ctx, void *ptr) {
    return ks_guard(ctx, [&]() -> int {
    if (!ctx) return KS_ERR_INVALID_ARG;
    KS_HIP(ctx, hipStreamSynchronize(ctx->stream));
    KS_HIP(ctx, hipFree(ptr));
    return KS_OK;
    });
}
extern "C" int ks_dev_upload(ks_ctx *ctx, void *dst, const void *src, uint64_t bytes) {
    return ks_guard(ctx, [&]() -> int {
    if (!ctx || (bytes && (!dst || !src))) return KS_ERR_INVALID_ARG;
    KS_HIP(ctx, hipSetDevice(ctx->device));
    KS_TRY(ks_copy_h2d(ctx, dst, src, (size_t)bytes));
    KS_HIP(ctx, hipStreamSynchronize(ctx->stream));
    return KS_OK;
    });
}
extern "C" int ks_dev_download(ks_ctx *ctx, void *dst, const void *src, uint64_t bytes) {
    return ks_guard(ctx, [&]() -> int {
    if (!ctx || (bytes && (!dst || !src))) return KS_ERR_INVALID_ARG;
    KS_HIP(ctx, hipSetDevice(ctx->device));
    KS_TRY(ks_copy_d2h(ctx, dst, src, (size_t)bytes));
    KS_HIP(ctx, hipStreamSynchronize(ctx->stream));
    return KS_OK;
    });
}

__global__ void k_host_stamp(unsigned long long *flag, unsigned long long seq) {
    __hip_atomic_store(flag, seq, __ATOMIC_RELEASE, __HIP_MEMORY_SCOPE_SYSTEM);
}
struct ks_fetch_args { ks_fetch_seg seg[KS_FETCH_MAX]; int n; };
__global__ __launch_bounds__(256) void k_host_report(ks_fetch_args F, unsigned long long *flag, unsigned long long seq) {
    for (int s = 0; s < F.n; s++) {
        const ks_fetch_seg g = F.seg[s];
        const u32 total = g.rows * g.row_words;
        for (u32 i = threadIdx.x; i < total; i += blockDim.x) {
            const u32 r = i / g.row_words, c = i - r * g.row_words;
            const u32 v = __hip_atomic_load((const u32 *)g.src + (size_t)r * g.src_stride + c, __ATOMIC_RELAXED, __HIP_MEMORY_SCOPE_AGENT);
            __hip_atomic_store(g.dst + i, v, __ATOMIC_RELAXED, __HIP_MEMORY_SCOPE_SYSTEM);
        }
    }
    __threadfence_system();
    __syncthreads();
    if (threadIdx.x == 0) __hip_atomic_store(flag, seq, __ATOMIC_RELEASE, __HIP_MEMORY_SCOPE_SYSTEM);
}

static int stream_wait_poll(ks_ctx *ctx, unsigned long long seq);

int ks_stream_wait_fetch(ks_ctx *ctx, const ks_fetch_seg *segs, int n) {
    if (n > KS_FETCH_MAX) return ks_fail(ctx, KS_ERR_INVALID_ARG, "too many fetch segments");
    if (!ctx->h_flag || ks_dbg(ctx, KS_DBG_SYNC_API)) {
        for (int i = 0; i < n; i++) {
            const ks_fetch_seg &g = segs[i];
            if (g.rows == 1 || g.src_stride == g.row_words)
                KS_HIP(ctx, hipMemcpyAsync(g.dst, g.src, (size_t)g.rows * g.row_words * sizeof(u32), hipMemcpyDeviceToHost, ctx->stream));
            else
                KS_HIP(ctx, hipMemcpy2DAsync(g.dst, (size_t)g.row_words * sizeof(u32), g.src, (size_t)g.src_stride * sizeof(u32),
                                            (size_t)g.row_words * sizeof(u32), g.rows, hipMemcpyDeviceToHost, ctx->stream));
        }
        KS_HIP(ctx, hipStreamSynchronize(ctx->stream));
        return KS_OK;
    }
    ks_fetch_args F;
    memset(&F, 0, sizeof F);
    for (int i = 0; i < n; i++) F.seg[i] = segs[i];
    F.n = n;
    const unsigned long long seq = ++ctx->wait_seq;
    hipLaunchKernelGGL(k_host_report, dim3(1), dim3(256), 0, ctx->stream, F, ctx->h_flag, seq);
    if (hipGetLastError() != hipSuccess) return ks_fail(ctx, KS_ERR_HIP, "k_host_report launch failed");
    return stream_wait_poll(ctx, seq);
}

int ks_stream_wait(ks_ctx *ctx) {
    if (!ctx->h_flag || ks_dbg(ctx, KS_DBG_SYNC_API)) {
        KS_HIP(ctx, hipStreamSynchronize(ctx->stream));
        return KS_OK;
    }
    const unsigned long long seq = ++ctx->wait_seq;
    hipLaunchKernelGGL(k_host_stamp, dim3(1), dim3(1), 0, ctx->stream, ctx->h_flag, seq);
    if (hipGetLastError() != hipSuccess) { KS_HIP(ctx, hipStreamSynchronize(ctx->stream)); return KS_OK; }
    return stream_wait_poll(ctx, seq);
}

static int stream_wait_poll(ks_ctx *ctx, unsigned long long seq) {
    for (unsigned spins = 1;; spins++) {
        if (__atomic_load_n(ctx->h_flag, __ATOMIC_ACQUIRE) == seq) return KS_OK;
        if ((spins & 0xfffu) == 0) {
            const hipError_t q = hipStreamQuery(ctx->stream);
            if (q == hipSuccess) {
                if (__atomic_load_n(ctx->h_flag, __ATOMIC_ACQUIRE) == seq) return KS_OK;
                KS_HIP(ctx, hipStreamSynchronize(ctx->stream));
                return KS_OK;
            }
            if (q != hipErrorNotReady) return ks_fail(ctx, KS_ERR_HIP, "stream failed: %s", hipGetErrorString(q));
            if (spins > (1u << 26)) { KS_HIP(ctx, hipStreamSynchronize(ctx->stream)); return KS_OK; }
        }
#if defined(__x86_64__)
        __builtin_ia32_pause();
#endif
    }
}

static size_t pool_class(size_t bytes) {
    if (bytes <= 4096) return (bytes + 255) & ~(size_t)255;
    const int e = 63 - __builtin_clzll((unsigned long long)(bytes - 1));
    const size_t step = (size_t)1 << (e - 2);
    return (bytes + step - 1) & ~(step - 1);
}

void *ks_pool_alloc(ks_ctx *ctx, size_t bytes) {
    if (bytes == 0) bytes = 256;
    const size_t want = pool_class(bytes);
    for (size_t i = 0; i < ctx->pool.size(); i++) {
        auto &b = ctx->pool[i];
        if (!b.in_use && b.size == want) { b.in_use = true; return b.ptr; }
    }
    if (ctx->pool_cap) {
        size_t held = 0;
        for (auto &b : ctx->pool) held += b.size;
        if (held + want > ctx->pool_cap) {
            ks_fail(ctx, KS_ERR_OOM, "device pool cap: %zu bytes held, %zu wanted, cap %llu", held, want, (unsigned long long)ctx->pool_cap);
            return nullptr;
        }
    }
    void *p = nullptr;
    hipError_t e = hipMalloc(&p, want);
    if (e != hipSuccess) {
        (void)hipGetLastError();
        int best = -1;
        for (size_t i = 0; i < ctx->pool.size(); i++) {
            auto &b = ctx->pool[i];
            if (!b.in_use && b.size >= want && (best < 0 || b.size < ctx->pool[best].size)) best = (int)i;
        }
        if (best >= 0) { ctx->pool[best].in_use = true; return ctx->pool[best].ptr; }
        ks_pool_trim(ctx);
        e = hipMalloc(&p, want);
    }
    if (e != hipSuccess) {
        (void)hipGetLastError();
        ks_fail(ctx, KS_ERR_OOM, "hipMalloc(%zu) failed: %s", want, hipGetErrorString(e));
        return nullptr;
// ... 259 lines not shown
```

### kmerseek_amd/csrc/ks_msd.hip

```cpp
#include <type_traits>

#include "ks_device.h"

#define MS_THREADS 512
#define MS_IPT 16
#define MS_TILE (MS_THREADS * MS_IPT)
#define MS_WAVES (MS_THREADS / 64)
static_assert(MS_TILE == 8192, "ks_search.hip counts the level-1 tiles of a segmented list in units of 8192 records");
#define MS_SUB 8u

template <int NB>
KS_DEV u32 ms_digit(u64 key, int shift, u32 base, u32 mask) {
    if constexpr (NB == 256) return (u32)(key >> shift) & 255u;
    else return ((u32)(key >> shift) & mask) - base;
}
template <int NB>
KS_DEV u32 ms_base(const u64 *keys, u64 tile_base, int shift, u32 mask, int bits2) {
    if constexpr (NB == 256) return 0u;
    else return (((u32)(keys[tile_base] >> shift) & mask) >> bits2) << bits2;
}

template <int SEG>
KS_DEV void ms_tile_range(u32 t, u64 n, const ks_msd_segs &S, u64 *base, u32 *nvalid) {
    if constexpr (SEG == 0) {
// ... 176 lines not shown
            if (r < nr) {
                const u32 li = (u32)r * 64 + lane;
                const u32 d = li < nb ? ((u32)(key[r] >> shift) & mask) : 255u;
                rank[r] = ks_match8_rank(d, wc);
            }
        }
        __builtin_amdgcn_wave_barrier();
        {
            const uint4 c = *(const uint4 *)&wc[4 * lane];
            const u32 tot = c.x + c.y + c.z + c.w;
            u32 ex = ks_wave_incl_scan(tot) - tot;
            uint4 o;
            o.x = ex; ex += c.x; o.y = ex; ex += c.y; o.z = ex; ex += c.z; o.w = ex;
            *(uint4 *)&wc[4 * lane] = o;
        }
        __builtin_amdgcn_wave_barrier();
#pragma unroll
        for (int r = 0; r < ML_IPT; r++)
            if (r < nr) wstage[wc[rank[r] >> 16] + (rank[r] & 0xffffu)] = key[r];
        __builtin_amdgcn_wave_barrier();
#pragma unroll
        for (int r = 0; r < ML_IPT; r++) {
            const u32 li = (u32)r * 64 + lane;
            if (r < nr) key[r] = li < nb ? wstage[li] : ~0ULL;
        }
        __builtin_amdgcn_wave_barrier();
    }
#pragma unroll
    for (int r = 0; r < ML_IPT; r++) {
        const u32 li = (u32)r * 64 + lane;
        if (r < nr && li < nb) keys[s + li] = key[r];
    }
}

__global__ __launch_bounds__(ML_THREADS) void k_msd_local(u64 *keys, const u32 *off, u32 n_buckets, int lo_bit, int rem_bits, u32 lds_cap,
                                                          u32 *big ) {
    __shared__ u32 wcnt[ML_WAVES][256];
    __shared__ __attribute__((aligned(16))) u64 stage[ML_CAP];
    const u32 lane = threadIdx.x & 63, wave = threadIdx.x >> 6;
    if (rem_bits <= 0) return;
    const u32 wave_cap = lds_cap < ML_WCAP ? lds_cap : ML_WCAP;
    const u32 bw = blockIdx.x * ML_WAVES + wave;
    if (bw < n_buckets) {
        const u64 s = bw ? off[bw - 1] : 0, nb64 = (u64)off[bw] - s;
        if (nb64 > 1 && nb64 <= wave_cap) ml_sort_wave(keys, s, (u32)nb64, lo_bit, rem_bits, wcnt[wave], stage + wave * ML_WCAP, lane);
        else if (nb64 > wave_cap && lane == 0) big[1 + atomicAdd(&big[0], 1u)] = bw;
    }
}

__global__ __launch_bounds__(ML_THREADS) void k_msd_local_big(u64 *keys, u64 *scratch, const u32 *off, const u32 *big, int lo_bit, int rem_bits,
                                                              u32 lds_cap) {
    __shared__ u32 wcnt[ML_WAVES][256];
    __shared__ u32 dcount[256], dstart[256], cursor[256];
    __shared__ u32 scan_smem[ML_WAVES + 1];
    __shared__ __attribute__((aligned(16))) u64 stage[ML_CAP];
    const u32 tid = threadIdx.x, lane = tid & 63, wave = tid >> 6;
    if (rem_bits <= 0) return;
    const int n_pass = (rem_bits + 7) / 8;
    const u32 wloc = wave * (64 * ML_IPT);
    const u32 n_big = big[0];
    for (u32 w = blockIdx.x; w < n_big; w += gridDim.x) {
        const u32 bb = big[1 + w];
        const u64 s = bb ? off[bb - 1] : 0, e = off[bb];
        const u64 nb64 = e - s;
        __syncthreads();
        u64 key[ML_IPT];
        u32 rank[ML_IPT];
        if (nb64 <= lds_cap) {
            const u32 nb = (u32)nb64;
#pragma unroll
            for (int r = 0; r < ML_IPT; r++) {
                const u32 li = wloc + (u32)r * 64 + lane;
                key[r] = li < nb ? keys[s + li] : ~0ULL;
            }
            for (int p = 0; p < n_pass; p++) {
                const int shift = lo_bit + 8 * p;
                const u32 mask = (rem_bits - 8 * p) >= 8 ? 255u : ((1u << (rem_bits - 8 * p)) - 1u);
                for (int ww = 0; ww < ML_WAVES; ww++) wcnt[ww][tid] = 0;
                __syncthreads();
                ml_rank(key, rank, nb, wloc, lane, wave, shift, mask, wcnt);
                __syncthreads();
                ml_offsets(wcnt, dcount, dstart, scan_smem);
                __syncthreads();
#pragma unroll
                for (int r = 0; r < ML_IPT; r++) stage[wcnt[wave][rank[r] >> 16] + (rank[r] & 0xffffu)] = key[r];
                __syncthreads();
#pragma unroll
                for (int r = 0; r < ML_IPT; r++) {
                    const u32 li = wloc + (u32)r * 64 + lane;
                    key[r] = li < nb ? stage[li] : ~0ULL;
                }
                __syncthreads();
            }
#pragma unroll
            for (int r = 0; r < ML_IPT; r++) {
                const u32 li = wloc + (u32)r * 64 + lane;
                if (li < nb) keys[s + li] = key[r];
            }
            continue;
        }
        u64 *src = keys + s, *dst = scratch + s;
        for (int p = 0; p < n_pass; p++) {
            const int shift = lo_bit + 8 * p;
            const u32 mask = (rem_bits - 8 * p) >= 8 ? 255u : ((1u << (rem_bits - 8 * p)) - 1u);
            cursor[tid] = 0;
            __syncthreads();
            for (u64 t0 = 0; t0 < nb64; t0 += ML_CAP)
                for (u32 i = tid; i < ML_CAP && t0 + i < nb64; i += ML_THREADS) atomicAdd(&cursor[(u32)(src[t0 + i] >> shift) & mask], 1u);
            __syncthreads();
            {
                u32 total;
                const u32 ex = ks_block_excl_scan(cursor[tid], scan_smem, &total);
                __syncthreads();
                cursor[tid] = ex;
            }
            __syncthreads();
            for (u64 t0 = 0; t0 < nb64; t0 += ML_CAP) {
                const u32 nv = (nb64 - t0) < ML_CAP ? (u32)(nb64 - t0) : ML_CAP;
#pragma unroll
                for (int r = 0; r < ML_IPT; r++) {
                    const u32 li = wloc + (u32)r * 64 + lane;
                    key[r] = li < nv ? src[t0 + li] : ~0ULL;
                }
                for (int ww = 0; ww < ML_WAVES; ww++) wcnt[ww][tid] = 0;
                __syncthreads();
                ml_rank(key, rank, nv, wloc, lane, wave, shift, mask, wcnt);
                __syncthreads();
                ml_offsets(wcnt, dcount, dstart, scan_smem);
                __syncthreads();
#pragma unroll
                for (int r = 0; r < ML_IPT; r++) {
                    const u32 li = wloc + (u32)r * 64 + lane;
                    if (li < nv) {
                        const u32 d = rank[r] >> 16;
                        dst[(u64)cursor[d] + (wcnt[wave][d] - dstart[d]) + (rank[r] & 0xffffu)] = key[r];
                    }
                }
                __syncthreads();
                if (tid == mask && nv < ML_CAP) dcount[mask] -= ML_CAP - nv;
                __syncthreads();
                cursor[tid] += dcount[tid];
                __syncthreads();
            }
            __threadfence();
            __syncthreads();
            u64 *t = src; src = dst; dst = t;
        }
        if (src != keys + s) {
            for (u64 i = tid; i < nb64; i += ML_THREADS) dst[i] = src[i];
        }
    }
}

int ks_sort_pairs_msd(ks_ctx *ctx, u64 *ka, u64 *kb, u64 n, int lo_bit, int nbits, int *done, const ks_msd_segs *segs) {
    *done = 0;
    if (nbits <= 16 || n < 65536 || n >= 0xffffffffULL || ks_dbg(ctx, KS_DBG_PAIRS_LSD)) return KS_OK;
    int bits2 = 0;
    while (bits2 < 9 && (n >> (8 + bits2)) > (bits2 < 8 ? 768u : 560u)) bits2++;
    for (int b = bits2 + 1; b <= 8 && nbits - 8 - b > 0; b++)
        if ((nbits - 8 - b + 7) / 8 < (nbits - 8 - bits2 + 7) / 8) { bits2 = b; break; }
    if (nbits - 8 - bits2 <= 0) bits2 = nbits - 9 > 0 ? nbits - 9 : 0;
    const int shift1 = lo_bit + nbits - 8, shift2 = shift1 - bits2;
    const u32 mask2 = (1u << (8 + bits2)) - 1u, n_buckets = 1u << (8 + bits2);
    const u32 n_tiles = (u32)((n + MS_TILE - 1) / MS_TILE);
    const u32 n_tiles1 = segs ? segs->tile_start[segs->n] : n_tiles;
    ks_msd_segs no_segs;
    no_segs.n = 0;
    u32 lds_cap = ML_CAP;
    if (const char *f = ks_dbg(ctx, KS_DBG_MSD_LDS_CAP)) {
        const u32 v = (u32)atoi(f);
        if (v >= 2 && v < ML_CAP) lds_cap = v;
    }
    u32 *blk = nullptr;
    const u32 n_sub = bits2 > 0 ? MS_SUB : 1u, sub_stride = bits2 > 0 ? 256u : 0u;
    const size_t off2_words = bits2 > 0 ? (size_t)n_buckets + 1 : 0, n_zero = 256 * MS_SUB + off2_words + 1;
    int st = ks_alloc(ctx, &blk, n_zero + (size_t)(n_buckets > 65536u ? n_buckets : 65536u) + 1);
    u32 *off1 = blk, *off2 = blk ? blk + 256 * MS_SUB : nullptr, *big = blk ? blk + 256 * MS_SUB + off2_words : nullptr;
    u64 *sorted_in = ka;
    if (st == KS_OK) {
        (void)hipMemsetAsync(blk, 0, n_zero * sizeof(u32), ctx->stream);
        ks_timer_begin(ctx, "msd_hist");
        if (segs) hipLaunchKernelGGL((k_msd_hist<256, 1>), dim3(n_tiles1), dim3(MS_THREADS), 0, ctx->stream, (const u64 *)ka, n, shift1, off1, 255u, 0, sub_stride, *segs);
        else hipLaunchKernelGGL((k_msd_hist<256, 0>), dim3(n_tiles), dim3(MS_THREADS), 0, ctx->stream, (const u64 *)ka, n, shift1, off1, 255u, 0, sub_stride, no_segs);
        ks_timer_end(ctx);
        ks_timer_begin(ctx, "msd_scan");
        hipLaunchKernelGGL(k_msd_scan256, dim3(1), dim3(256), 0, ctx->stream, off1, n_sub);
        ks_timer_end(ctx);
        ks_timer_begin(ctx, "msd_scatter");
        if (segs) hipLaunchKernelGGL((k_msd_scatter<256, 1>), dim3(n_tiles1), dim3(MS_THREADS), 0, ctx->stream, (const u64 *)ka, kb, n, shift1, off1, 255u, 0,
                                     sub_stride, *segs);
        else hipLaunchKernelGGL((k_msd_scatter<256, 0>), dim3(n_tiles), dim3(MS_THREADS), 0, ctx->stream, (const u64 *)ka, kb, n, shift1, off1, 255u, 0,
                                sub_stride, no_segs);
        ks_timer_end(ctx);
        sorted_in = kb;
    }
    const u32 *off = off1;
    if (st == KS_OK && bits2 > 0) {
        ks_timer_begin(ctx, "msd_hist");
        if (bits2 <= 8) hipLaunchKernelGGL((k_msd_hist<512>), dim3(n_tiles), dim3(MS_THREADS), 0, ctx->stream, (const u64 *)kb, n, shift2, off2, mask2, bits2, 0u, no_segs);
        else hipLaunchKernelGGL((k_msd_hist<1024>), dim3(n_tiles), dim3(MS_THREADS), 0, ctx->stream, (const u64 *)kb, n, shift2, off2, mask2, bits2, 0u, no_segs);
        ks_timer_end(ctx);
        st = ks_scan_u32_inplace(ctx, off2, n_buckets, nullptr);
        if (st == KS_OK) {
            ks_timer_begin(ctx, "msd_scatter");
            if (bits2 <= 8) hipLaunchKernelGGL((k_msd_scatter<512>), dim3(n_tiles), dim3(MS_THREADS), 0, ctx->stream, (const u64 *)kb, ka, n, shift2, off2, mask2, bits2, 0u, no_segs);
            else hipLaunchKernelGGL((k_msd_scatter<1024>), dim3(n_tiles), dim3(MS_THREADS), 0, ctx->stream, (const u64 *)kb, ka, n, shift2, off2, mask2, bits2, 0u, no_segs);
            ks_timer_end(ctx);
            sorted_in = ka;
            off = off2;
        }
    }
    if (st == KS_OK) {
        u64 *other = sorted_in == ka ? kb : ka;
        ks_timer_begin(ctx, "msd_local");
        hipLaunchKernelGGL(k_msd_local, dim3((n_buckets + ML_WAVES - 1) / ML_WAVES), dim3(ML_THREADS), 0, ctx->stream, sorted_in, off,
                           n_buckets, lo_bit, shift2 - lo_bit, lds_cap, big);
        ks_timer_end(ctx);
        ks_timer_begin(ctx, "msd_local_big");
        hipLaunchKernelGGL(k_msd_local_big, dim3(n_buckets < 2048 ? n_buckets : 2048), dim3(ML_THREADS), 0, ctx->stream, sorted_in, other, off,
                           (const u32 *)big, lo_bit, shift2 - lo_bit, lds_cap);
        ks_timer_end(ctx);
        if (sorted_in != ka)
            if (hipMemcpyAsync(ka, kb, (size_t)n * sizeof(u64), hipMemcpyDeviceToDevice, ctx->stream) != hipSuccess)
                st = ks_fail(ctx, KS_ERR_HIP, "msd sort: copy back failed");
        if (st == KS_OK && hipGetLastError() != hipSuccess) st = ks_fail(ctx, KS_ERR_HIP, "msd sort launch failed");
        if (st == KS_OK) *done = 1;
    }
    ks_pool_free(ctx, blk);
    return st;
}
```

### kmerseek_amd/csrc/ks_rows.hip

```cpp
#include "ks_device.h"

__global__ __launch_bounds__(256) void k_pair_heads(const u64 *keys, u64 n, u32 *heads) {
    u64 i = (u64)blockIdx.x * blockDim.x + threadIdx.x;
    if (i >= n) return;
    heads[i] = (i == 0 || keys[i] != keys[i - 1]) ? 1u : 0u;
}

__global__ __launch_bounds__(256) void k_pair_rows(const u64 *keys, const u32 *hidx, u64 n, u32 n_rows, u64 *row_start) {
    u64 i = (u64)blockIdx.x * blockDim.x + threadIdx.x;
    if (i >= n) return;
    bool head = (i == 0) || keys[i] != keys[i - 1];
    if (head) row_start[hidx[i]] = i;
    if (i == 0) row_start[n_rows] = n;
}

int ks_sorted_runs(ks_ctx *ctx, const ks_sketches *in, ks_scratch &sc, ks_runs *out) {
    const u64 n = in->n_hashes;
    u64 *k0 = nullptr, *k1 = nullptr;
    u32 *v0 = nullptr, *v1 = nullptr, *heads = nullptr, *d_nrows = nullptr;
    KS_TRY(sc.alloc(&k0, (size_t)n)); KS_TRY(sc.alloc(&k1, (size_t)n));
    KS_TRY(sc.alloc(&v0, (size_t)n)); KS_TRY(sc.alloc(&v1, (size_t)n));
    const int shifts[8] = {0, 8, 16, 24, 32, 40, 48, 56};
    KS_TRY(ks_radix_sort_u32(ctx, KS_SORT_PAIRS, in->d_hashes, in->d_abunds, k0, v0, k1, v1, n, shifts, 8, &out->keys, &out->vals));
    KS_TRY(sc.alloc(&heads, (size_t)n));
    KS_TRY(sc.alloc(&d_nrows, 1));
    const u32 g = (u32)((n + 255) / 256);
    KS_LAUNCH(ctx, "run_heads", k_pair_heads, g, 256, (const u64 *)out->keys, n, heads);
    KS_TRY(ks_scan_u32_inplace(ctx, heads, n, d_nrows));
    u64 *const rb = ctx->h_pin + KS_PIN_READ;
    KS_HIP(ctx, hipMemcpyAsync(rb, d_nrows, sizeof(u32), hipMemcpyDeviceToHost, ctx->stream));
    KS_TRY(ks_scan_status_fetch(ctx));
    KS_HIP(ctx, hipStreamSynchronize(ctx->stream));
    KS_TRY(ks_scan_status_check(ctx));
    const u32 n_rows = *(u32 *)rb;
    if (n_rows == 0 || n_rows > n) return ks_fail(ctx, KS_ERR_HIP, "internal error: %u runs in %llu sorted postings", n_rows, (unsigned long long)n);
    out->n_rows = n_rows;
    KS_TRY(sc.alloc(&out->row_start, (size_t)n_rows + 1));
    KS_LAUNCH(ctx, "run_starts", k_pair_rows, g, 256, (const u64 *)out->keys, (const u32 *)heads, n, n_rows, out->row_start);
    return KS_OK;
}

#define PF_THREADS 256
#define PF_IPT 8
#define PF_TILE (PF_THREADS * PF_IPT)
#define PF_WAVES (PF_THREADS / 64)

__global__ __launch_bounds__(PF_THREADS) void k_pair_rows_fused(const u64 *keys, u64 n, u32 *qid, u32 *tid, u32 *isect, unsigned long long *nw,
                                                                int tbits, int abits, u32 rows_cap, unsigned long long *status,
                                                                u32 *ticket , u32 *n_rows_out,
                                                                int use_ticket) {
    __shared__ u32 tile_s;
    __shared__ u32 wcount[PF_IPT][PF_WAVES];
    __shared__ unsigned long long base_s;
    const u32 tid_ = threadIdx.x, lane = tid_ & 63, wave = tid_ >> 6;
    if (use_ticket) {
        if (tid_ == 0) tile_s = atomicAdd(&ticket[0], 1u);
        __syncthreads();
    }
    const u32 tile = use_ticket ? tile_s : blockIdx.x;
    const u64 b0 = (u64)tile * PF_TILE;
    u64 key[PF_IPT];
    u32 headbits = 0;
#pragma unroll
    for (int r = 0; r < PF_IPT; r++) {
        const u64 i = b0 + (u64)r * PF_THREADS + tid_;
        key[r] = i < n ? keys[i] : 0;
    }
    u64 pp = 0;
    {
        const u64 iw = b0 + (u64)lane * PF_THREADS + (tid_ & ~63u);
        if (lane < PF_IPT && iw > 0 && iw < n) pp = keys[iw - 1];
    }
#pragma unroll
    for (int r = 0; r < PF_IPT; r++) {
        const u64 i = b0 + (u64)r * PF_THREADS + tid_;
        const u64 below = ((u64)ks_lane_below((u32)(key[r] >> 32)) << 32) | ks_lane_below((u32)key[r]);
        const u64 first = ((u64)(u32)__builtin_amdgcn_readlane((int)(u32)(pp >> 32), r) << 32) | (u32)__builtin_amdgcn_readlane((int)(u32)pp, r);
        const u64 prev = lane ? below : first;
        const bool head = i < n && (i == 0 || (prev >> abits) != (key[r] >> abits));
        headbits |= head ? (1u << r) : 0u;
        const u64 m = __ballot(head);
        if (lane == 0) wcount[r][wave] = (u32)__popcll(m);
    }
    __syncthreads();
    if (wave == 0) {
        const u32 c = lane < PF_IPT * PF_WAVES ? wcount[lane / PF_WAVES][lane % PF_WAVES] : 0u;
        const u32 incl = ks_wave_incl_scan(c);
        const u32 total = (u32)__builtin_amdgcn_readlane((int)incl, 63);
        if (lane < PF_IPT * PF_WAVES) wcount[lane / PF_WAVES][lane % PF_WAVES] = incl - c;
        if (lane == 0)
            __hip_atomic_store(&status[tile], (tile == 0 ? KS_LB_PRE : KS_LB_AGG) | (u64)total, __ATOMIC_RELAXED, __HIP_MEMORY_SCOPE_AGENT);
        u64 excl = 0;
        if (tile > 0) {
            excl = ks_lookback_walk(tile, lane, ks_lookback_words(status), &ticket[1]);
            if (lane == 0)
                __hip_atomic_store(&status[tile], KS_LB_PRE | (excl + total), __ATOMIC_RELAXED, __HIP_MEMORY_SCOPE_AGENT);
        }
        if (lane == 0) {
            base_s = excl;
            if (b0 + PF_TILE >= n) *n_rows_out = (u32)(excl + total);
        }
    }
    __syncthreads();
    const u64 base = base_s;
#pragma unroll
    for (int r = 0; r < PF_IPT; r++) {
        const u64 i = b0 + (u64)r * PF_THREADS + tid_;
        const bool live = i < n;
        const bool head = (headbits >> r) & 1u;
        const u64 m = __ballot(head);
        const u64 row64 = base + wcount[r][wave] + ks_lane_lt_count(m) + (head ? 1u : 0u) - 1u;
        const u32 row = live ? (u32)row64 : 0xffffffffu;
        u64 w = live ? (key[r] & ((1ULL << abits) - 1ULL)) : 0;
        u32 c = live ? 1u : 0u;
        if (head && row < rows_cap) {
            const u64 ids = key[r] >> abits;
            qid[row] = (u32)(ids >> tbits);
            tid[row] = (u32)(ids & ((1ULL << tbits) - 1ULL));
        }
        {
            const u32 rowx = row ^ 1u;
            u32 wl = (u32)w, wh = (u32)(w >> 32);
#define PF_SEG_STEP(CTRL, RMASK) do { \
                const u32 orow = (u32)__builtin_amdgcn_update_dpp((int)rowx, (int)row, CTRL, RMASK, 0xf, false); \
                const u32 oc = (u32)__builtin_amdgcn_update_dpp(0, (int)c, CTRL, RMASK, 0xf, false); \
                const u32 ol = (u32)__builtin_amdgcn_update_dpp(0, (int)wl, CTRL, RMASK, 0xf, false); \
                const u32 oh = (u32)__builtin_amdgcn_update_dpp(0, (int)wh, CTRL, RMASK, 0xf, false); \
                const bool same = orow == row; \
                const u64 nw_ = (((u64)wh << 32) | wl) + (same ? (((u64)oh << 32) | ol) : 0ULL); \
                c += same ? oc : 0u; wl = (u32)nw_; wh = (u32)(nw_ >> 32); } while (0)
            PF_SEG_STEP(0x111, 0xf);
            PF_SEG_STEP(0x112, 0xf);
            PF_SEG_STEP(0x114, 0xf);
            PF_SEG_STEP(0x118, 0xf);
            PF_SEG_STEP(0x142, 0xa);
            PF_SEG_STEP(0x143, 0xc);
#undef PF_SEG_STEP
            w = ((u64)wh << 32) | wl;
        }
        const u32 nrow = (u32)__builtin_amdgcn_update_dpp((int)(row ^ 1u), (int)row, 0x130, 0xf, 0xf, false);
        if (live && (lane == 63 || nrow != row) && row < rows_cap) {
            atomicAdd(&isect[row], c);
            atomicAdd(&nw[row], (unsigned long long)w);
        }
    }
}

#define RA_LONG 64

__global__ __launch_bounds__(256) void k_row_abund_stats(const u64 *pk, const u64 *row_start, const u32 *isect, const u32 *n_rows_dev,
                                                         u32 rows_cap, int abits, u64 *median2, double *ss, u32 *long_rows) {
#pragma clang fp contract(off)
    const u32 r = blockIdx.x * blockDim.x + threadIdx.x;
    const u32 n_rows = *n_rows_dev < rows_cap ? *n_rows_dev : rows_cap;
    if (r >= n_rows) return;
    const u32 n = isect[r];
    const u64 *a = pk + row_start[r];
    const u64 am = (1ULL << abits) - 1ULL;
    if (n > RA_LONG) { ks_row_list_push(long_rows, r); return; }
    if (n == 0) { median2[r] = 0; ss[r] = 0.0; return; }
    double sum = 0.0;
    for (u32 j = 0; j < n; j++) sum += (double)(a[j] & am);
    const double mean = sum / (double)n;
    double acc = 0.0;
    for (u32 j = 0; j < n; j++) {
        const double d = (double)(a[j] & am) - mean;
        acc += d * d;
    }
    ss[r] = acc;
    median2[r] = (n & 1u) ? 2ULL * (a[n / 2] & am) : (a[n / 2 - 1] & am) + (a[n / 2] & am);
}

__global__ __launch_bounds__(256) void k_row_abund_stats_long(const u64 *pk, const u64 *row_start, const u32 *isect, const u32 *long_rows,
                                                              u32 rows_cap, int abits, u64 *median2, double *ss) {
    const u32 lane = threadIdx.x & 63;
    const u64 am = (1ULL << abits) - 1ULL;
    ks_row_list_walk(long_rows, rows_cap, [&](u32 r) {
#pragma clang fp contract(off)
        const u32 n = isect[r];
        const u64 *a = pk + row_start[r];
        double sum = 0.0;
        for (u32 c = 0; c < n; c += 64) {
            const double x = c + lane < n ? (double)(a[c + lane] & am) : 0.0;
            ks_wave_add_ordered(ks_lanes_below(n - c), sum, x);
        }
        const double mean = sum / (double)n;
        double acc = 0.0;
        for (u32 c = 0; c < n; c += 64) {
            const double d = c + lane < n ? (double)(a[c + lane] & am) - mean : 0.0;
            const double t = d * d;
            ks_wave_add_ordered(ks_lanes_below(n - c), acc, t);
        }
        if (lane == 0) {
            ss[r] = acc;
            median2[r] = (n & 1u) ? 2ULL * (a[n / 2] & am) : (a[n / 2 - 1] & am) + (a[n / 2] & am);
        }
    });
}

KS_DEV bool rf_kept(const rf_cols &in, u32 r, const u64 *q_offsets, const u32 *q_counts, u32 n_queries, double min_c) {
    const u32 q = in.qid[r];
    if (q >= n_queries) return false;
    const u64 nq = q_counts ? (u64)q_counts[q] : q_offsets[q + 1] - q_offsets[q];
    return (double)in.isect[r] / (double)nq >= min_c;
}

__global__ __launch_bounds__(256) void k_rows_keep(rf_cols in, const u32 *n_rows_dev, u32 rows_cap, const u64 *q_offsets, const u32 *q_counts,
                                                   u32 n_queries, double min_c, u32 *flags) {
    const u32 r = blockIdx.x * blockDim.x + threadIdx.x;
    if (r >= rows_cap) return;
    const u32 n_rows = *n_rows_dev < rows_cap ? *n_rows_dev : rows_cap;
    flags[r] = (r < n_rows && rf_kept(in, r, q_offsets, q_counts, n_queries, min_c)) ? 1u : 0u;
}

__global__ __launch_bounds__(256) void k_rows_filter(rf_cols in, const u32 *n_rows_dev, u32 rows_cap, const u64 *q_offsets, const u32 *q_counts,
                                                     u32 n_queries, double min_c, const u32 *dst, u32 *qid, u32 *tid, u32 *isect, u64 *nw,
                                                     u64 *median2, double *ss) {
    const u32 r = blockIdx.x * blockDim.x + threadIdx.x;
    const u32 n_rows = *n_rows_dev < rows_cap ? *n_rows_dev : rows_cap;
    if (r >= n_rows || !rf_kept(in, r, q_offsets, q_counts, n_queries, min_c)) return;
    rf_move(in, r, dst[r], qid, tid, isect, nw, median2, ss);
}

static void se_free_cols(ks_ctx *ctx, ks_hits *H) {
    ks_pool_free(ctx, H->d_qid); ks_pool_free(ctx, H->d_tid);
    if (H->d_block) ks_pool_free(ctx, H->d_block);
    else { ks_pool_free(ctx, H->d_isect); ks_pool_free(ctx, H->d_nw); }
    ks_pool_free(ctx, H->d_median2); ks_pool_free(ctx, H->d_ss);
    H->d_qid = H->d_tid = H->d_isect = nullptr;
    H->d_nw = H->d_block = H->d_median2 = nullptr;
    H->d_ss = nullptr;
}

#define RA_LONG_GRID 256

int ks_row_list_alloc(ks_ctx *ctx, ks_scratch &sc, size_t n_rows, u32 **list) {
    KS_TRY(sc.alloc(list, n_rows + 1));
    KS_HIP(ctx, hipMemsetAsync(*list, 0, sizeof(u32), ctx->stream));
    return KS_OK;
}
int ks_seg_list_alloc(ks_ctx *ctx, ks_scratch &sc, size_t cap, u32 **list) { return ks_row_list_alloc(ctx, sc, 2 * cap, list); }
int ks_seg_path_knob(const ks_ctx *ctx, int dbg_id, bool *small) {
    const char *f = ks_dbg(ctx, dbg_id);
    const int v = f ? atoi(f) : 0;
    *small = v == 3;
    return v == 1 ? 1 : (v == 2 || v == 3) ? 2 : 0;
}

static int se_rows_post(ks_ctx *ctx, const ks_rows_in &Q, ks_hits *H, ks_hits *F, const u64 *pk, u32 rows_cap, u32 *ticket, ks_scratch &sc) {
    const u32 *n_rows_dev = ticket + 2;
    const u32 g = (rows_cap + 255) / 256;
    if (Q.stats) {
        u64 *row_start = nullptr;
        u32 *long_rows = nullptr;
        KS_TRY(sc.alloc(&row_start, (size_t)rows_cap + 1));
        KS_TRY(ks_row_list_alloc(ctx, sc, rows_cap, &long_rows));
        KS_TRY(ks_alloc(ctx, &H->d_median2, rows_cap));
        KS_TRY(ks_alloc(ctx, &H->d_ss, rows_cap));
        KS_TRY(ks_scan_u32_to_u64(ctx, H->d_isect, row_start, rows_cap));
        KS_LAUNCH(ctx, "row_abund_stats", k_row_abund_stats, g, 256, pk, (const u64 *)row_start, (const u32 *)H->d_isect, n_rows_dev,
                  rows_cap, Q.abits, H->d_median2, H->d_ss, long_rows);
        KS_LAUNCH(ctx, "row_abund_stats_long", k_row_abund_stats_long, RA_LONG_GRID, 256, pk, (const u64 *)row_start,
                  (const u32 *)H->d_isect, (const u32 *)long_rows, rows_cap, Q.abits, H->d_median2, H->d_ss);
    }
    if (Q.min_c > 0) {
        const ks_sketches *q = Q.q;
        const u32 *counts = q->gapped ? q->d_counts : nullptr;
        const rf_cols in{H->d_qid, H->d_tid, H->d_isect, H->d_nw, H->d_median2, H->d_ss};
        u32 *flags = nullptr;
        KS_TRY(sc.alloc(&flags, rows_cap));
        KS_LAUNCH(ctx, "rows_keep", k_rows_keep, g, 256, in, n_rows_dev, rows_cap, (const u64 *)q->d_offsets, counts, q->n_seqs, Q.min_c,
                  flags);
        KS_TRY(ks_scan_u32_inplace(ctx, flags, rows_cap, ticket + 3));
        F->has_stats = Q.stats;
        KS_TRY(ks_hits_alloc_cols(ctx, F, rows_cap, 0));
        KS_LAUNCH(ctx, "rows_filter", k_rows_filter, g, 256, in, n_rows_dev, rows_cap, (const u64 *)q->d_offsets, counts, q->n_seqs, Q.min_c,
                  (const u32 *)flags, F->d_qid, F->d_tid, F->d_isect, F->d_nw, F->d_median2, F->d_ss);
    }
    return KS_OK;
}

static int se_rows_run(ks_ctx *ctx, const ks_rows_in &Q, ks_hits *H, ks_hits &F, const u64 *pk) {
    const u64 n_pairs = Q.n_pairs;
    const int tbits = Q.tbits, abits = Q.abits;
    const u32 pf_tiles = (u32)((n_pairs + PF_TILE - 1) / PF_TILE);
    u64 rows_cap = n_pairs;
    if (ctx->rows_hint && ctx->rows_hint < rows_cap && !ks_dbg(ctx, KS_DBG_NO_ROWS_HINT)) rows_cap = ctx->rows_hint;
    u32 n_rows = 0;
    const u32 *pin = (const u32 *)(ctx->h_pin + KS_PIN_ROWS);
    const bool post = Q.stats || Q.min_c > 0;
    for (int attempt = 0; attempt < 3; attempt++) {
        ks_scratch sc(ctx);
        KS_TRY(ks_alloc(ctx, &H->d_qid, (size_t)rows_cap)); KS_TRY(ks_alloc(ctx, &H->d_tid, (size_t)rows_cap));
        const size_t st_words = (size_t)pf_tiles + 2, is_words = ((size_t)rows_cap + 1) / 2;
        KS_TRY(ks_alloc(ctx, &H->d_block, (size_t)rows_cap + st_words + is_words));
        H->d_nw = H->d_block;
        H->d_isect = (u32 *)(H->d_block + rows_cap + st_words);
        unsigned long long *const pf_status = (unsigned long long *)(H->d_block + rows_cap);
        u32 *const pf_ticket = (u32 *)(pf_status + pf_tiles);
        KS_HIP(ctx, hipMemsetAsync(H->d_block, 0, ((size_t)rows_cap + st_words + is_words) * sizeof(u64), ctx->stream));
        KS_LAUNCH(ctx, "pair_rows", k_pair_rows_fused, pf_tiles, PF_THREADS, pk, n_pairs, H->d_qid, H->d_tid, H->d_isect,
                  (unsigned long long *)H->d_nw, tbits, abits, (u32)rows_cap, pf_status, pf_ticket, pf_ticket + 2,
                  (ctx->rows_use_ticket || ks_dbg(ctx, KS_DBG_ROWS_TICKET)) ? 1 : 0);
        if (post) KS_TRY(se_rows_post(ctx, Q, H, &F, pk, (u32)rows_cap, pf_ticket, sc));
        KS_TRY(ks_stream_wait_fetch_scans(ctx, {ks_fetch_words(pf_ticket, ctx->h_pin + KS_PIN_ROWS, 4)}));
        bool gave_up = pin[1] != 0;
        if (ks_dbg(ctx, KS_DBG_FORCE_ROWS_TICKET_RETRY) && !ctx->rows_use_ticket) gave_up = true;
        if (gave_up) {
            if (ctx->rows_use_ticket || attempt == 2) return ks_fail(ctx, KS_ERR_HIP, "search: row look-back gave up waiting for a predecessor tile");
            ctx->rows_use_ticket = true;
            ctx->rows_ticket_fallbacks++;
        } else {
            n_rows = pin[2];
            if (n_rows <= rows_cap) break;
            rows_cap = n_rows;
        }
        se_free_cols(ctx, H);
        se_free_cols(ctx, &F);
    }
    if (!H->d_qid) return ks_fail(ctx, KS_ERR_HIP, "search: the row pass did not settle");
    H->n_hits = n_rows;
    const u64 want = (u64)n_rows + n_rows / 4 + 4096;
    ctx->rows_hint = want > ctx->rows_hint / 2 ? want : ctx->rows_hint / 2;
    if (Q.min_c > 0) {
        se_free_cols(ctx, H);
        H->d_qid = F.d_qid; H->d_tid = F.d_tid; H->d_isect = F.d_isect; H->d_nw = F.d_nw;
        H->d_median2 = F.d_median2; H->d_ss = F.d_ss;
        H->n_hits = pin[3];
        memset(&F, 0, sizeof F);
    }
    return KS_OK;
}

int ks_search_rows(ks_ctx *ctx, const ks_rows_in &Q, ks_hits *H, const u64 *pk) {
    if (Q.n_pairs == 0) return ks_hits_alloc_cols(ctx, H, 0, 0);
    ks_hits F;
    memset(&F, 0, sizeof F);
    const int st = se_rows_run(ctx, Q, H, F, pk);
    se_free_cols(ctx, &F);
    return st;
}

__global__ __launch_bounds__(256) void k_union_emit(const u64 *keys, const u32 *vals, const u64 *row_start, u32 n_rows,
                                                    u64 *hashes, u32 *abunds) {
    u32 r = blockIdx.x * blockDim.x + threadIdx.x;
    if (r >= n_rows) return;
    const u64 b = row_start[r], w = ks_run_abund_sum(vals, b, row_start[r + 1]);
    hashes[r] = keys[b];
    abunds[r] = w > 0xffffffffULL ? 0xffffffffu : (u32)w;
}

static int union_run(ks_ctx *ctx, const ks_sketches *in, ks_sketches *U) {
    const u64 n = in->n_hashes;
    KS_TRY(ks_alloc(ctx, &U->d_offsets, 2));
    if (n == 0) {
        KS_HIP(ctx, hipMemsetAsync(U->d_offsets, 0, 2 * sizeof(u64), ctx->stream));
        KS_TRY(ks_alloc(ctx, &U->d_hashes, 1)); KS_TRY(ks_alloc(ctx, &U->d_abunds, 1));
        KS_HIP(ctx, hipStreamSynchronize(ctx->stream));
        return KS_OK;
    }
    ks_scratch sc(ctx);
    ks_runs R;
    KS_TRY(ks_sorted_runs(ctx, in, sc, &R));
    U->n_hashes = U->n_slots = R.n_rows;
    KS_TRY(ks_alloc(ctx, &U->d_hashes, (size_t)R.n_rows)); KS_TRY(ks_alloc(ctx, &U->d_abunds, (size_t)R.n_rows));
    KS_LAUNCH(ctx, "union_emit", k_union_emit, (R.n_rows + 255) / 256, 256, (const u64 *)R.keys, (const u32 *)R.vals,
              (const u64 *)R.row_start, R.n_rows, U->d_hashes, U->d_abunds);
    u64 *const rb = ctx->h_pin + KS_PIN_READ;
    rb[0] = 0; rb[1] = R.n_rows;
    KS_HIP(ctx, hipMemcpyAsync(U->d_offsets, rb, 2 * sizeof(u64), hipMemcpyHostToDevice, ctx->stream));
    KS_HIP(ctx, hipStreamSynchronize(ctx->stream));
    return KS_OK;
}

int ks_union_impl(ks_ctx *ctx, const ks_sketches *in, ks_sketches **out) {
    if (!in || !out) return ks_fail(ctx, KS_ERR_INVALID_ARG, "NULL argument");
    KS_HIP(ctx, hipSetDevice(ctx->device));
    KS_TRY(ks_sketches_make_dense(ctx, const_cast<ks_sketches *>(in)));
    ks_result<ks_sketches> U(ctx, out, ks_sketches_free);
    U->params = in->params; U->n_seqs = 1; U->n_windows = in->n_windows;
    KS_TRY(union_run(ctx, in, U));
    return U.commit();
}
```

### kmerseek_amd/csrc/ks_search.hip

```cpp
#include "ks_device.h"

__global__ __launch_bounds__(256) void k_fill_index_vals(const u64 *csr, const u32 *abunds, u32 n_seqs, u64 *vals) {
    const u32 s = blockIdx.x * 4 + (threadIdx.x >> 6);
    if (s >= n_seqs) return;
    const u64 b = csr[s], e = csr[s + 1];
    for (u64 j = b + (threadIdx.x & 63); j < e; j += 64) vals[j] = ((u64)abunds[j] << 32) | s;
}

__global__ __launch_bounds__(256) void k_fill_query_vals(const u64 *csr, u32 n_seqs, u32 *vals) {
    const u32 s = blockIdx.x * 4 + (threadIdx.x >> 6);
    if (s >= n_seqs) return;
    const u64 b = csr[s], e = csr[s + 1];
    for (u64 j = b + (threadIdx.x & 63); j < e; j += 64) vals[j] = s;
}

__global__ __launch_bounds__(256) void k_split_vals(const u64 *vals, u64 n, u32 *tids, u32 *abunds, u32 *max_abund) {
    u64 i = (u64)blockIdx.x * blockDim.x + threadIdx.x;
    u32 a = 0;
    if (i < n) {
        u64 v = vals[i];
        tids[i] = (u32)v;
        a = (u32)(v >> 32);
        abunds[i] = a;
    }
// ... 929 lines not shown
};

static int se_finish_pending(se_search &Q, int *sketch_redo) {
    if (!Q.q->pending) return KS_OK;
    int redo = 0;
    KS_TRY(ks_sketch_finish_pending(const_cast<ks_sketches *>(Q.q), &redo));
    Q.n_q = Q.q->n_hashes;
    if (redo) {
        if (sketch_redo) *sketch_redo = redo;
        Q.stop = true;
    }
    return KS_OK;
}

static int se_wait_pending(ks_ctx *ctx, se_search &Q, int *sketch_redo) {
    const ks_fetch_seg f = ks_sketch_pending_seg(Q.q);
    KS_TRY(ks_stream_wait_fetch(ctx, &f, 1));
    return se_finish_pending(Q, sketch_redo);
}

static int se_partition(ks_ctx *ctx, se_search &Q, int way, ks_scratch &sc, se_qview *V) {
    const ks_sketches *q = Q.q;
    const int pbits = Q.pbits;
    const u32 n_buckets = Q.n_buckets;
    memset(V, 0, sizeof *V);
    if (way == 1 && Q.f10) Q.pre = false;
    const u32 q_s = (way == 0 && Q.f10) ? q->part_s : 0u;
    V->q_fmt = q_s ? ((pbits == 16 && q_s == 48u && !ks_dbg(ctx, KS_DBG_POSTINGS10)) ? 2 : 1) : 0;
    KS_HIP(ctx, hipMemsetAsync(Q.cursor, 0, ((size_t)JN_SEGS * JN_CUR_STRIDE + (way == 0 ? (n_buckets + 1) / 2 : 0)) * sizeof(u64), ctx->stream));
    if (way == 0) {
        const u64 per = Q.n_q / n_buckets;
        const u32 bcap = (u32)(per + per / 8 + 512);
        KS_TRY(sc.alloc(&V->qk0, (size_t)n_buckets * bcap));
        KS_TRY(sc.alloc(&V->qv0, (size_t)n_buckets * bcap));
        ks_rs_segments seg{q->part_len, q->part_cap, q->part_regions << q->part_sub_shift, q->part_sub_shift};
        const char *qf_knob = ks_dbg(ctx, KS_DBG_QFILTER);
        Q.qf = Q.ix->d_presence && (qf_knob ? atoi(qf_knob) != 0 : ctx->qfilter_pays);
        KS_TRY(ks_bucket_scatter_u32(ctx, q->part_keys, q->part_vals, &seg, 8, Q.pfxK, V->qk0, V->qv0, Q.bcur, bcap, Q.cursor, n_buckets >> 8,
                                     V->q_fmt,
                                     Q.qf ? Q.ix->d_presence : nullptr, Q.ix->pres_K, q_s ? q_s - 32u : 0u));
        V->bucket_posting_bytes = V->q_fmt == 2 ? 9 : (V->q_fmt == 1 ? 10 : 12);
        KS_LAUNCH(ctx, "bucket_dir", k_region_dir, (n_buckets + 255) / 256, 256, (const u32 *)Q.bcur, (u64)bcap, n_buckets, Q.dir_q,
                  Q.dir_q + n_buckets, n_buckets >> 8);
        V->qk = V->qk0; V->qv = V->qv0; V->q_lo = Q.dir_q; V->q_hi = Q.dir_q + n_buckets;
        V->partition_path = 1;
    } else if (Q.pre && pbits <= 8) {
        V->qk = q->part_keys; V->qv = q->part_vals;
        KS_LAUNCH(ctx, "bucket_dir", k_region_dir, (n_buckets + 255) / 256, 256, (const u32 *)q->part_len, q->part_cap, n_buckets, Q.dir_q,
                  Q.dir_q + n_buckets, 0u);
        V->q_lo = Q.dir_q; V->q_hi = Q.dir_q + n_buckets;
        V->partition_path = 0;
    } else {
        const u64 n_q = Q.n_q;
        if (!Q.pre) KS_TRY(ks_sketches_make_dense(ctx, const_cast<ks_sketches *>(q)));
        KS_TRY(sc.alloc(&V->qk0, (size_t)n_q)); KS_TRY(sc.alloc(&V->qk1, (size_t)n_q));
        KS_TRY(sc.alloc(&V->qv0, (size_t)n_q)); KS_TRY(sc.alloc(&V->qv1, (size_t)n_q));
        if (Q.pre) {
            int shifts[2], nsh = 0;
            for (int sh = 8; sh < pbits; sh += 8) shifts[nsh++] = sh;
            ks_rs_segments seg{q->part_len, q->part_cap, q->part_regions << q->part_sub_shift, q->part_sub_shift};
            KS_TRY(ks_radix_sort_u32(ctx, KS_SORT_QPART, q->part_keys, q->part_vals, V->qk1, V->qv1, V->qk0, V->qv0, n_q, shifts, nsh,
                                     &V->qk, &V->qv, &seg, Q.pfxK));
        } else {
            KS_LAUNCH(ctx, "fill_query_vals", k_fill_query_vals, (q->n_seqs + 3) / 4, 256, (const u64 *)q->d_offsets, q->n_seqs, V->qv0);
            int shifts[3], ns = 0;
            for (int sh = 0; sh < pbits; sh += 8) shifts[ns++] = sh;
            KS_TRY(ks_radix_sort_u32(ctx, KS_SORT_QPART, q->d_hashes, V->qv0, V->qk1, V->qv1, V->qk0, V->qv0, n_q, shifts, ns, &V->qk,
                                     &V->qv, nullptr, Q.pfxK));
        }
        KS_LAUNCH(ctx, "bucket_dir", k_bucket_dir, (n_buckets + 256) / 256, 256, (const u64 *)V->qk, n_q, pbits, Q.pfxK, Q.dir_q);
        V->q_lo = Q.dir_q; V->q_hi = Q.dir_q + 1;
        V->partition_path = Q.pre ? 2 : 3;
    }
    return KS_OK;
}

static int se_join(ks_ctx *ctx, se_search &Q, const se_qview &V, int way, u64 cap, ks_scratch &sc, u64 *split_pairs, int *sketch_redo,
                   bool *overflowed) {
    const ks_index *ix = Q.ix;
    const u32 n_buckets = Q.n_buckets;
    const int q_fmt = V.q_fmt;
    *overflowed = false;
    {
        const u64 per_bucket = Q.n_q / n_buckets, round = (u64)JN_THREADS * JN_E;
        const u64 reservations = (u64)n_buckets * ((per_bucket + round - 1) / round ? (per_bucket + round - 1) / round : 1);
        Q.n_segs = (ix->fp_layout && reservations >= 8192 && n_buckets >= JN_SEGS && !ks_dbg(ctx, KS_DBG_ONE_CURSOR)) ? JN_SEGS : 1;
        if (ix->fp_layout && ks_dbg(ctx, KS_DBG_JOIN_SEGS) && n_buckets >= JN_SEGS) Q.n_segs = JN_SEGS;
    }
    const u32 n_segs = Q.n_segs;
    Q.seg_cap = n_segs == 1 ? cap : cap / n_segs + cap / n_segs / 8 + 4096;
    if (ks_dbg(ctx, KS_DBG_JOIN_SEG_CAP)) Q.seg_cap = strtoull(ks_dbg(ctx, KS_DBG_JOIN_SEG_CAP), nullptr, 10);
    const u64 *dir_t = ix->d_dir;
    const u64 *pin = ctx->h_pin + KS_PIN_JOIN;
    for (int attempt = 0; attempt < 2; attempt++) {
        const u64 seg_cap = Q.seg_cap;
        KS_TRY(sc.alloc(&Q.pk0, (size_t)(seg_cap * n_segs)));
        if (attempt > 0)
            KS_HIP(ctx, hipMemset2DAsync(Q.cursor, (size_t)JN_CUR_STRIDE * sizeof(u64), 0, sizeof(u64), JN_SEGS, ctx->stream));
        const bool sparse = ix->fp_layout && (ks_dbg(ctx, KS_DBG_JOIN_SPARSE) ? atoi(ks_dbg(ctx, KS_DBG_JOIN_SPARSE)) != 0
                                                                             : Q.n_q / n_buckets <= (u64)JS_QCAP * 3 / 4);
        if (sparse)
            KS_LAUNCH(ctx, "join_buckets", (q_fmt == 2 ? k_join_sparse<2> : (q_fmt ? k_join_sparse<1> : k_join_sparse<0>)), n_buckets, JS_THREADS,
                      (const u64 *)V.qk, (const u32 *)V.qv, (const u32 *)ix->d_fp, (const ks_post *)ix->d_post, (const ks_bmeta *)ix->d_bmeta,
                      V.q_lo, V.q_hi, dir_t, Q.pk0, seg_cap, Q.cursor, n_segs - 1, Q.tbits, Q.abits, ix->fp_shift);
        else if (ix->fp_layout)
            KS_LAUNCH(ctx, "join_buckets", (q_fmt == 2 ? k_join_buckets<2> : (q_fmt ? k_join_buckets<1> : k_join_buckets<0>)), n_buckets, JN_THREADS,
                      (const u64 *)V.qk, (const u32 *)V.qv, (const u32 *)ix->d_fp, (const ks_post *)ix->d_post, (const ks_bmeta *)ix->d_bmeta,
                      V.q_lo, V.q_hi, dir_t, Q.pk0, seg_cap, Q.cursor, n_segs - 1, Q.tbits, Q.abits, ix->fp_shift);
        else {
            u32 split = 1;
            if (ctx->pair_cap_hint > Q.n_q && Q.n_q / n_buckets >= 1024) {
                const u64 dens2 = 2 * ctx->pair_cap_hint / Q.n_q;
                split = dens2 >= 6 ? 4u : (dens2 >= 3 ? 2u : 1u);
            }
            if (const char *f = ks_dbg(ctx, KS_DBG_JOIN_SPLIT)) { const int v = atoi(f); if (v >= 1 && v <= 16) split = (u32)v; }
            KS_LAUNCH(ctx, "join_buckets", k_join_buckets_keys, n_buckets * split, JN_THREADS, (const u64 *)V.qk, (const u32 *)V.qv,
                      (const u64 *)ix->d_keys, (const u32 *)ix->d_tids, (const u32 *)ix->d_abunds, V.q_lo, V.q_hi, dir_t, Q.pk0, seg_cap,
                      Q.cursor, Q.tbits, Q.abits, split);
        }
        {
            ks_fetch_seg f[2];
            f[0] = ks_fetch_seg{Q.cursor, (u32 *)pin, n_segs == 1 ? 1u : (u32)JN_SEGS, 4u, (u32)JN_CUR_STRIDE * 2u};
            int nf = 1;
            if (Q.q->pending) f[nf++] = ks_sketch_pending_seg(Q.q);
            KS_TRY(ks_stream_wait_fetch(ctx, f, nf));
        }
        KS_TRY(se_finish_pending(Q, sketch_redo));
        if (Q.stop) return KS_OK;
        Q.n_pairs = 0;
        u64 seg_max = 0;
        for (u32 s_ = 0; s_ < n_segs; s_++) {
            Q.seg_count[s_] = pin[2 * s_];
            Q.n_pairs += Q.seg_count[s_];
            if (Q.seg_count[s_] > seg_max) seg_max = Q.seg_count[s_];
        }
        *overflowed = way == 0 && (pin[1] & 1ULL) != 0;
        Q.qf_kept = pin[1] >> KS_QF_KEPT;
        if (!*overflowed && Q.n_pairs >= KS_PAIR_LIMIT) {
            *split_pairs = Q.n_pairs;
            Q.stop = true;
            return KS_OK;
        }
        if (*overflowed || seg_max <= seg_cap) return KS_OK;
        if (attempt == 1)
            return ks_fail(ctx, KS_ERR_CAPACITY, "search produced %llu matched posting pairs (segment cap %llu)",
                           (unsigned long long)Q.n_pairs, (unsigned long long)seg_cap);
        sc.free(Q.pk0); Q.pk0 = nullptr;
        Q.seg_cap = seg_max;
        ctx->join_retries++;
    }
    return KS_OK;
}

static int se_sort(ks_ctx *ctx, se_search &Q, ks_scratch &sc, u64 **pk) {
    const u64 n_pairs = Q.n_pairs;
    const u32 n_segs = Q.n_segs;
    const int tbits = Q.tbits, qbits = Q.qbits, abits = Q.abits;
    const int lo_bit = Q.stats ? 0 : abits, nbits = tbits + qbits + (Q.stats ? abits : 0);
    KS_TRY(sc.alloc(&Q.pk1, (size_t)n_pairs));
    int msd = 0;
    if (n_segs > 1) {
        static_assert(JN_SEGS <= KS_MSD_MAX_SEGS, "segment table of the match sort");
        ks_msd_segs sg;
        sg.n = n_segs; sg.seg_cap = Q.seg_cap;
        u32 t = 0;
        for (u32 s_ = 0; s_ < n_segs; s_++) {
            sg.tile_start[s_] = t; sg.count[s_] = (u32)Q.seg_count[s_];
            t += (u32)((Q.seg_count[s_] + 8191) / 8192);
        }
        sg.tile_start[n_segs] = t;
        for (u32 s_ = n_segs + 1; s_ <= KS_MSD_MAX_SEGS; s_++) sg.tile_start[s_] = t;
        KS_TRY(ks_sort_pairs_msd(ctx, Q.pk0, Q.pk1, n_pairs, lo_bit, nbits, &msd, &sg));
    }
    if (n_segs > 1 && !msd) {
        jn_seg_table tab;
        u64 acc = 0;
        for (u32 s_ = 0; s_ < n_segs; s_++) { tab.prefix[s_] = acc; acc += Q.seg_count[s_]; }
        tab.prefix[n_segs] = acc;
        u64 seg_max = 0;
        for (u32 s_ = 0; s_ < n_segs; s_++) if (Q.seg_count[s_] > seg_max) seg_max = Q.seg_count[s_];
        KS_LAUNCH(ctx, "pairs_compact", k_pairs_compact, dim3((u32)((seg_max + 2047) / 2048), n_segs), 256, (const u64 *)Q.pk0, Q.seg_cap,
                  tab, Q.pk1);
        u64 *tk = Q.pk0; Q.pk0 = Q.pk1; Q.pk1 = tk;
    }
    if (!msd) KS_TRY(ks_sort_pairs_msd(ctx, Q.pk0, Q.pk1, n_pairs, lo_bit, nbits, &msd));
    if (msd) {
        *pk = Q.pk0;
        return KS_OK;
    }
    int shifts[8], ns = 0;
    for (int sh = 0; sh < nbits; sh += 8) shifts[ns++] = lo_bit + sh;
    return ks_radix_sort_keys(ctx, KS_SORT_PAIRS, Q.pk0, Q.pk0, Q.pk1, n_pairs, shifts, ns, pk);
}

static ks_rows_in se_rows_in(const se_search &Q) { return ks_rows_in{Q.q, Q.n_pairs, Q.tbits, Q.abits, Q.stats, Q.min_c}; }

struct se_split {
    u64 pairs;
    u32 seqs;
};

static int search_run(ks_ctx *ctx, const ks_index *ix, const ks_sketches *q, const ks_search_opts *opts, ks_hits *H, se_split *split,
                      int *sketch_redo, bool *stop) {
    se_search Q;
    memset(&Q, 0, sizeof Q);
    Q.ix = ix; Q.q = q; Q.n_q = q->n_hashes;
    Q.stats = opts && (opts->flags & KS_SEARCH_ABUND_STATS);
    Q.min_c = opts ? opts->min_containment : 0.0;
    H->has_stats = Q.stats;
    const u64 n_t = ix->n_postings;
    if (q->pending && (n_t == 0 || !(q->part_keys && q->part_pbits == ix->pbits && ix->pbits > 0))) {
        KS_TRY(se_wait_pending(ctx, Q, sketch_redo));
        if ((*stop = Q.stop)) return KS_OK;
    }
    if (Q.n_q == 0 || n_t == 0) return ks_search_rows(ctx, se_rows_in(Q), H, nullptr);
    Q.pbits = ix->pbits;
    Q.n_buckets = 1u << Q.pbits;
    Q.tbits = bits_for(ix->n_targets);
    Q.qbits = bits_for(q->n_seqs);
    Q.abits = bits_for_value(ix->max_abund);
    int width = 64;
    if (const char *f = ks_dbg(ctx, KS_DBG_RECORD_BITS)) { const int v = atoi(f); if (v >= 1 && v < 64) width = v; }
    if (Q.tbits + Q.qbits + Q.abits > width) {
        if (q->pending) {
            KS_TRY(se_wait_pending(ctx, Q, sketch_redo));
            if ((*stop = Q.stop)) return KS_OK;
        }
        if (Q.tbits + Q.abits >= width)
            return ks_fail(ctx, KS_ERR_CAPACITY, "search: %d target id bits + %d abundance bits leave no query id bit in a %d-bit match record",
                           Q.tbits, Q.abits, width);
        split->seqs = 1u << (width - Q.tbits - Q.abits);
        *stop = true;
        return KS_OK;
    }
    Q.pfxK = ks_join_prefix_mul(Q.pbits, ks_max_hash(ix->params.scaled));
    ks_scratch sc(ctx);
    KS_TRY(sc.alloc(&Q.dir_q, (size_t)2 * Q.n_buckets + 2));
    KS_TRY(sc.alloc((u64 **)&Q.cursor, (size_t)JN_SEGS * JN_CUR_STRIDE + (Q.n_buckets + 1) / 2));
    Q.bcur = (u32 *)(Q.cursor + (size_t)JN_SEGS * JN_CUR_STRIDE);
    const bool pre_any = q->part_keys && q->part_pbits == Q.pbits && q->part_K == Q.pfxK && Q.pbits > 0;
    const bool f10_fits = ix->fp_layout && Q.pbits > 8 && q->part_s == 32u + (u32)ix->fp_shift;
    Q.pre = pre_any && (q->part_s == 0 || f10_fits);
    Q.f10 = Q.pre && q->part_s != 0;
    if (q->pending && !Q.pre) {
        KS_TRY(se_wait_pending(ctx, Q, sketch_redo));
        if ((*stop = Q.stop)) return KS_OK;
    }
    u64 cap = Q.n_q < (1u << 20) ? (1u << 20) : Q.n_q;
    if (ctx->pair_cap_hint > cap) cap = ctx->pair_cap_hint;
    for (int way = (Q.pre && Q.pbits > 8) ? 0 : 1; way < 2; way++) {
        se_qview V;
        KS_TRY(se_partition(ctx, Q, way, sc, &V));
        if (V.bucket_posting_bytes) H->bucket_posting_bytes = V.bucket_posting_bytes;
        bool overflowed = false;
        KS_TRY(se_join(ctx, Q, V, way, cap, sc, &split->pairs, sketch_redo, &overflowed));
        if ((*stop = Q.stop)) return KS_OK;
        sc.free(V.qk0); sc.free(V.qk1); sc.free(V.qv0); sc.free(V.qv1);
        if (!overflowed) {
            H->partition_path = V.partition_path;
            if (way == 0 && Q.qf) {
                const u64 dropped = Q.n_q > Q.qf_kept ? Q.n_q - Q.qf_kept : 0;
                ctx->qfilter_seen += Q.n_q;
                ctx->qfilter_dropped += dropped;
                ctx->qfilter_pays = dropped >= Q.n_q / 2;
            } else if (way == 0 && ix->d_presence && Q.n_pairs < Q.n_q / 4) {
                ctx->qfilter_pays = true;
            }
            break;
        }
        sc.free(Q.pk0); Q.pk0 = nullptr;
    }
    H->n_pair_instances = Q.n_pairs;
    const u64 want = Q.n_pairs + Q.n_pairs / 8;
    ctx->pair_cap_hint = want > ctx->pair_cap_hint / 2 ? want : ctx->pair_cap_hint / 2;
    u64 *pk = nullptr;
    if (Q.n_pairs) KS_TRY(se_sort(ctx, Q, sc, &pk));
    return ks_search_rows(ctx, se_rows_in(Q), H, pk);
}

static int search_core(ks_ctx *ctx, const ks_index *ix, const ks_sketches *q, const ks_search_opts *opts, ks_hits **out, se_split *split,
                       int *sketch_redo = nullptr) {
    *split = se_split{};
    *out = nullptr;
    if (sketch_redo) *sketch_redo = 0;
    if (!ix || !q || !out) return ks_fail(ctx, KS_ERR_INVALID_ARG, "NULL argument");
    if (ix->params.ksize != q->params.ksize || ix->params.scaled != q->params.scaled ||
        ix->params.moltype != q->params.moltype || ix->params.seed != q->params.seed)
        return ks_fail(ctx, KS_ERR_INVALID_ARG, "query sketches and index were built with different parameters");
    KS_HIP(ctx, hipSetDevice(ctx->device));
    ks_result<ks_hits> H(ctx, out, ks_hits_free);
    bool stop = false;
    KS_TRY(search_run(ctx, ix, q, opts, H, split, sketch_redo, &stop));
    return stop ? KS_OK : H.commit();
}

__global__ __launch_bounds__(256) void k_rebase_offsets(const u64 *offs, u64 base, u32 n, u64 *out) {
    const u32 i = blockIdx.x * blockDim.x + threadIdx.x;
    if (i < n) out[i] = offs[i] - base;
}
__global__ __launch_bounds__(256) void k_add_u32(u32 *a, u64 n, u32 v) {
    const u64 i = (u64)blockIdx.x * blockDim.x + threadIdx.x;
    if (i < n) a[i] += v;
}

static ks_sketches sketches_slice_view(const ks_sketches *q, const std::vector<u64> &offs, u32 a, u32 b) {
    ks_sketches V = ks_sketches();
    V.ctx = q->ctx; V.params = q->params; V.n_seqs = b - a; V.n_hashes = offs[b] - offs[a]; V.n_windows = q->n_windows;
    V.d_hashes = q->d_hashes + offs[a]; V.d_abunds = q->d_abunds + offs[a];
    return V;
}

struct se_parts {
    std::vector<ks_hits *> hits;
    std::vector<u32> firsts;
    se_parts() = default;
    se_parts(const se_parts &) = delete;
    ~se_parts() { for (ks_hits *h : hits) ks_hits_free(h); }
};

static int search_sliced(ks_ctx *ctx, const ks_index *ix, const ks_sketches *q, const ks_search_opts *opts, const se_split &need,
                         const std::vector<u64> &offs, se_parts &parts) {
    u64 n_slices = need.pairs / (KS_PAIR_LIMIT / 4) + 1;
    const u32 max_seqs = need.seqs ? need.seqs : q->n_seqs;
    u32 a = 0;
    while (a < q->n_seqs) {
        const u64 want = q->n_hashes / n_slices + 1;
        u32 b = a + 1;
        while (b < q->n_seqs && b - a < max_seqs && offs[b + 1] - offs[a] <= want) b++;
        for (;;) {
            ks_sketches V = sketches_slice_view(q, offs, a, b);
            KS_TRY(ks_alloc(ctx, &V.d_offsets, (size_t)V.n_seqs + 1));
            hipLaunchKernelGGL(k_rebase_offsets, dim3((V.n_seqs + 256) / 256), dim3(256), 0, ctx->stream, (const u64 *)q->d_offsets + a, offs[a],
                               V.n_seqs + 1, V.d_offsets);
            ks_hits *h = nullptr;
            se_split more;
            const int st = search_core(ctx, ix, &V, opts, &h, &more);
            (void)hipStreamSynchronize(ctx->stream);
            ks_pool_free(ctx, V.d_offsets);
            KS_TRY(st);
            if (more.pairs == 0 && more.seqs == 0) { parts.hits.push_back(h); parts.firsts.push_back(a); break; }
            if (b - a == 1) return ks_fail(ctx, KS_ERR_CAPACITY, "one query sequence matches %llu postings: beyond the match-list limit", (unsigned long long)more.pairs);
            b = a + (b - a) / 2;
            n_slices *= 2;
        }
        a = b;
    }
    return KS_OK;
}

struct se_hit_col {
    size_t member, elem;
    u8 *get(const ks_hits *h) const { u8 *p; memcpy(&p, (const char *)h + member, sizeof p); return p; }
    void set(ks_hits *h, u8 *p) const { memcpy((char *)h + member, &p, sizeof p); }
};
static const se_hit_col SE_HIT_COLS[6] = {{offsetof(ks_hits, d_qid), sizeof(u32)},     {offsetof(ks_hits, d_tid), sizeof(u32)},
                                          {offsetof(ks_hits, d_isect), sizeof(u32)},   {offsetof(ks_hits, d_nw), sizeof(u64)},
                                          {offsetof(ks_hits, d_median2), sizeof(u64)}, {offsetof(ks_hits, d_ss), sizeof(double)}};

static int hits_concat(ks_ctx *ctx, const se_parts &parts, bool has_stats, ks_hits **out) {
    ks_result<ks_hits> H(ctx, out, ks_hits_free);
    H->partition_path = 3;
    H->has_stats = has_stats;
    for (const ks_hits *h : parts.hits) { H->n_hits += h->n_hits; H->n_pair_instances += h->n_pair_instances; }
    const int n_cols = has_stats ? 6 : 4;
    for (int c = 0; c < n_cols; c++) {
        u8 *col = nullptr;
        KS_TRY(ks_alloc(ctx, &col, (size_t)(H->n_hits ? H->n_hits : 1) * SE_HIT_COLS[c].elem));
        SE_HIT_COLS[c].set(H, col);
    }
    u64 at = 0;
    for (size_t i = 0; i < parts.hits.size(); i++) {
        ks_hits *const h = parts.hits[i];
        const u64 n = h->n_hits;
        if (!n) continue;
        hipLaunchKernelGGL(k_add_u32, dim3((u32)((n + 255) / 256)), dim3(256), 0, ctx->stream, h->d_qid, n, parts.firsts[i]);
        for (int c = 0; c < n_cols; c++) {
            const se_hit_col &C = SE_HIT_COLS[c];
            KS_HIP(ctx, hipMemcpyAsync(C.get(H) + at * C.elem, C.get(h), n * C.elem, hipMemcpyDeviceToDevice, ctx->stream));
        }
        at += n;
    }
    KS_HIP(ctx, hipStreamSynchronize(ctx->stream));
    return H.commit();
}

int ks_search_impl(ks_ctx *ctx, const ks_index *ix, const ks_sketches *q, ks_hits **out, int *sketch_redo, const ks_search_opts *opts) {
    if (!out) return ks_fail(ctx, KS_ERR_INVALID_ARG, "NULL argument");
    se_split need;
    KS_TRY(search_core(ctx, ix, q, opts, out, &need, sketch_redo));
    if (need.pairs == 0 && need.seqs == 0) return KS_OK;
    KS_TRY(ks_sketches_make_dense(ctx, const_cast<ks_sketches *>(q)));
    std::vector<u64> offs((size_t)q->n_seqs + 1);
    KS_HIP(ctx, hipMemcpyAsync(offs.data(), q->d_offsets, offs.size() * sizeof(u64), hipMemcpyDeviceToHost, ctx->stream));
    KS_HIP(ctx, hipStreamSynchronize(ctx->stream));
    se_parts parts;
    KS_TRY(search_sliced(ctx, ix, q, opts, need, offs, parts));
    return hits_concat(ctx, parts, opts && (opts->flags & KS_SEARCH_ABUND_STATS), out);
}

int ks_search_opts_check(ks_ctx *ctx, const ks_search_opts *o) {
    if (!o) return KS_OK;
    KS_TRY(ks_opts_words_check(ctx, "search", o->flags, KS_SEARCH_ABUND_STATS, o->reserved));
    if (o->min_containment >= 0.0) return KS_OK;
    return ctx ? ks_fail(ctx, KS_ERR_INVALID_ARG, "search options: min_containment must be >= 0 (and not NaN)") : KS_ERR_INVALID_ARG;
}
```

### kmerseek_amd/engine.py

```python
from __future__ import annotations

import ctypes as C
from typing import Dict, List, Optional, Sequence, Tuple

import numpy as np

from . import _lib
from ._lib import ks_params

MOLTYPES = {"protein": _lib.KS_PROTEIN, "raw": _lib.KS_PROTEIN, "dayhoff": _lib.KS_DAYHOFF, "hp": _lib.KS_HP}
MOLTYPE_NAMES = {_lib.KS_PROTEIN: "protein", _lib.KS_DAYHOFF: "dayhoff", _lib.KS_HP: "hp"}
SEED = _lib.KS_SEED_DEFAULT


class KmerseekError(RuntimeError):
    def __init__(self, status: int, message: str):
        super().__init__(message)
        self.status = status


class InvalidAminoAcid(KmerseekError):

    def __init__(self, char: str, position: int, seq_index: int = 0):
        super().__init__(_lib.KS_ERR_INVALID_RESIDUE, f"Invalid amino acid '{char}' found at position {position}")
# ... 19 lines not shown

def validate_and_resolve(seq: bytes, upper: bool = False, rng_seed: int = 0) -> bytes:
    L = _lib.load()
    out = C.create_string_buffer(len(seq) + 1)
    out_len = C.c_uint64(0)
    err = _lib.ks_residue_error()
    st = L.ks_validate_and_resolve(seq, len(seq), 1 if upper else 0, rng_seed, out, C.byref(out_len), C.byref(err))
    if st == _lib.KS_ERR_INVALID_RESIDUE:
        raise InvalidAminoAcid(chr(err.residue), err.position)
    if st != _lib.KS_OK:
        raise KmerseekError(st, L.ks_status_string(st).decode())
    return out.raw[:out_len.value]


def pack(seqs: Sequence[bytes]) -> Tuple[np.ndarray, np.ndarray]:
    offs = np.zeros(len(seqs) + 1, dtype=np.uint64)
    if len(seqs):
        offs[1:] = np.cumsum([len(s) for s in seqs], dtype=np.uint64)
    res = np.frombuffer(b"".join(seqs), dtype=np.uint8).copy() if len(seqs) else np.zeros(0, np.uint8)
    return res, offs


def _ptr(a: Optional[np.ndarray]):
    return None if a is None else a.ctypes.data_as(C.c_void_p)


def search_opts(min_containment: float = 0.0, abund_stats: bool = False) -> Optional[_lib.ks_search_opts]:
    if not abund_stats and min_containment == 0.0:
        return None
    return _lib.ks_search_opts(_lib.KS_SEARCH_ABUND_STATS if abund_stats else 0, 0, float(min_containment))


BEST_RANK_BY = {"intersect": _lib.KS_BEST_INTERSECT, "target_containment": _lib.KS_BEST_TARGET_CONTAINMENT,
                "max_containment": _lib.KS_BEST_MAX_CONTAINMENT, "jaccard": _lib.KS_BEST_JACCARD, "score": _lib.KS_BEST_SCORE}
GREEDY_ASSIGN = {"first": _lib.KS_GREEDY_ASSIGN_FIRST, "best": _lib.KS_GREEDY_ASSIGN_BEST}


class _FollowDebugEnv:

    def __init__(self, L, ctx):
        self._L, self._ctx = L, ctx

    def __getattr__(self, name):
        f = getattr(self._L, name)
        if not name.startswith("ks_") or name in ("ks_ctx_create", "ks_ctx_destroy", "ks_ctx_reload_debug_env", "ks_last_error",
                                                    "ks_status_string"):
            return f

        def call(*a):
            if self._ctx._h:
                self._L.ks_ctx_reload_debug_env(self._ctx._h)
            return f(*a)
        return call


class Context:

    _HIP_STREAM_LEGACY = 1

    def __init__(self, device: int = 0, stream: Optional[int] = None, follow_debug_env: bool = False):
        self._L = _lib.load()
        self._h = None
        if follow_debug_env:
            self._L = _FollowDebugEnv(self._L, self)
        h = C.c_void_p()
        sp = None if stream is None else C.c_void_p(int(stream) if int(stream) != 0 else self._HIP_STREAM_LEGACY)
        st = self._L.ks_ctx_create(int(device), sp, C.byref(h))
        if st != _lib.KS_OK:
            raise KmerseekError(st, f"ks_ctx_create(device={device}) failed: {self._L.ks_status_string(st).decode()}"
                                    " — the HIP path has no CPU fallback")
        self._h = h
        self.device = device
        self._pinned, self._close_pending = 0, False

    def close(self):
        if getattr(self, "_pinned", 0) > 0:
            self._close_pending = True
            return
        if getattr(self, "_h", None):
            self._L.ks_ctx_destroy(self._h)
            self._h = None

    def __del__(self):
        try:
            self.close()
        except Exception:
            pass

    def __enter__(self):
        return self

    def __exit__(self, *a):
        self.close()

    def _check(self, st: int):
        if st != _lib.KS_OK:
            msg = self._L.ks_last_error(self._h).decode() or self._L.ks_status_string(st).decode()
            raise KmerseekError(st, msg)

    @property
    def stream(self) -> int:
        v = int(self._L.ks_ctx_stream(self._h) or 0)
        return 0 if v == self._HIP_STREAM_LEGACY else v

    def synchronize(self):
        self._check(self._L.ks_ctx_synchronize(self._h))

    def to_device(self, a: np.ndarray) -> "DeviceBuffer":
        a = np.ascontiguousarray(a)
        p = C.c_void_p()
        self._check(self._L.ks_dev_malloc(self._h, a.nbytes, C.byref(p)))
        buf = DeviceBuffer(self, p, a.nbytes)
        self._check(self._L.ks_dev_upload(self._h, p, _ptr(a), a.nbytes))
        return buf

    def _device_empty(self, nbytes: int) -> "DeviceBuffer":
        p = C.c_void_p()
        self._check(self._L.ks_dev_malloc(self._h, int(nbytes), C.byref(p)))
        return DeviceBuffer(self, p, int(nbytes))

    def pinned_empty(self, n: int, dtype) -> np.ndarray:
        dt = np.dtype(dtype)
        nbytes = max(int(n) * dt.itemsize, 1)
        p = C.c_void_p()
        self._check(self._L.ks_host_alloc(self._h, nbytes, C.byref(p)))
        buf = (C.c_char * nbytes).from_address(p.value)
        buf._owner = _PinnedBlock(self, p)
        return np.frombuffer(buf, dtype=dt, count=int(n))

    def pool_stats(self) -> Dict[str, int]:
        v = [C.c_uint64(0) for _ in range(4)]
        self._check(self._L.ks_ctx_pool_stats(self._h, *[C.byref(x) for x in v]))
        return dict(zip(("blocks", "bytes_held", "bytes_in_use", "mallocs"), (int(x.value) for x in v)))

    def sketch_stats(self) -> Dict[str, int]:
        v = (C.c_uint64 * 4)()
        self._check(self._L.ks_ctx_sketch_stats(self._h, C.byref(v)))
        return {"ticket_fallbacks": int(v[0]), "uses_ticket": int(v[1]), "compact_fallbacks": int(v[2]), "cap_fallbacks": int(v[3])}

    def unpack_hits64_device(self, d_packed: int, n: int, qbits: int, tbits: int, d_qid: int, d_tid: int, d_isect: int, d_nw: int):
        self._check(self._L.ks_hits_unpack64_device(self._h, C.c_void_p(d_packed), n, qbits, tbits, C.c_void_p(d_qid), C.c_void_p(d_tid),
                                                    C.c_void_p(d_isect), C.c_void_p(d_nw)))

    def merge_hits_by_qid_device(self, d_qid: int, d_tid: int, d_isect: int, d_nw: int, block_rows: Sequence[int], n_queries: int,
                                 o_qid: int, o_tid: int, o_isect: int, o_nw: int):
        rows = (C.c_uint64 * len(block_rows))(*[int(x) for x in block_rows])
        self._check(self._L.ks_hits_merge_by_qid_device(self._h, C.c_void_p(d_qid), C.c_void_p(d_tid), C.c_void_p(d_isect), C.c_void_p(d_nw),
                                                        rows, len(block_rows), int(n_queries), C.c_void_p(o_qid), C.c_void_p(o_tid),
                                                        C.c_void_p(o_isect), C.c_void_p(o_nw)))

    def reload_debug_env(self):
        self._check(self._L.ks_ctx_reload_debug_env(self._h))

    def search_stats(self) -> Dict[str, int]:
        v = (C.c_uint64 * 2)()
        self._check(self._L.ks_ctx_search_stats(self._h, C.byref(v)))
        return {"join_retries": int(v[0]), "rows_ticket_fallbacks": int(v[1])}

    def sketch_batch(self, residues: np.ndarray, offsets: np.ndarray, ksize: int, scaled: int, moltype: str,
                     seed: int = SEED) -> "Sketches":
        residues = np.ascontiguousarray(residues, dtype=np.uint8)
        offsets = np.ascontiguousarray(offsets, dtype=np.uint64)
        p = make_params(ksize, scaled, moltype, seed)
        out = C.c_void_p()
        self._check(self._L.ks_sketch_batch(self._h, _ptr(residues), _ptr(offsets), len(offsets) - 1, C.byref(p),
                                            C.byref(out)))
        return Sketches(self, out)

    def sketch_batch_device(self, d_residues: int, d_offsets: int, n_seqs: int, n_residues: int, ksize: int,
                            scaled: int, moltype: str, max_seq_len: int = 0, seed: int = SEED) -> "Sketches":
        p = make_params(ksize, scaled, moltype, seed)
        out = C.c_void_p()
        self._check(self._L.ks_sketch_batch_device(self._h, C.c_void_p(d_residues), C.c_void_p(d_offsets), n_seqs,
                                                   n_residues, max_seq_len, C.byref(p), C.byref(out)))
        return Sketches(self, out)

    def sketch_queries_device(self, index: "Index", d_residues: int, d_offsets: int, n_seqs: int, n_residues: int,
                              max_seq_len: int = 0) -> "Sketches":
        out = C.c_void_p()
        self._check(self._L.ks_sketch_queries_device(self._h, index._h, C.c_void_p(d_residues), C.c_void_p(d_offsets),
                                                     n_seqs, n_residues, max_seq_len, C.byref(out)))
        return Sketches(self, out)

    def sketch_search_device(self, index: "Index", d_residues: int, d_offsets: int, n_seqs: int, n_residues: int,
                             max_seq_len: int = 0, want_sketches: bool = True, *, min_containment: float = 0.0,
                             abund_stats: bool = False):
        sk, hits = C.c_void_p(), C.c_void_p()
        opts = search_opts(min_containment, abund_stats)
        if opts is None:
            st = self._L.ks_sketch_search_device(self._h, index._h, C.c_void_p(d_residues), C.c_void_p(d_offsets), n_seqs,
                                                 n_residues, max_seq_len, C.byref(sk) if want_sketches else None, C.byref(hits))
        else:
            st = self._L.ks_sketch_search_device_ex(self._h, index._h, C.c_void_p(d_residues), C.c_void_p(d_offsets), n_seqs,
                                                    n_residues, max_seq_len, C.byref(opts), C.byref(sk) if want_sketches else None,
                                                    C.byref(hits))
        self._check(st)
        return (Sketches(self, sk) if want_sketches else None), Hits(self, hits)

    def sketch_search(self, index: "Index", residues: np.ndarray, offsets: np.ndarray, want_sketches: bool = True, *,
                      min_containment: float = 0.0, abund_stats: bool = False):
        residues = np.ascontiguousarray(residues, dtype=np.uint8)
        offsets = np.ascontiguousarray(offsets, dtype=np.uint64)
        sk, hits = C.c_void_p(), C.c_void_p()
        opts = search_opts(min_containment, abund_stats)
        if opts is None:
            st = self._L.ks_sketch_search(self._h, index._h, _ptr(residues), _ptr(offsets), len(offsets) - 1,
                                          C.byref(sk) if want_sketches else None, C.byref(hits))
        else:
            st = self._L.ks_sketch_search_ex(self._h, index._h, _ptr(residues), _ptr(offsets), len(offsets) - 1, C.byref(opts),
                                             C.byref(sk) if want_sketches else None, C.byref(hits))
        self._check(st)
        return (Sketches(self, sk) if want_sketches else None), Hits(self, hits)

    def translate6(self, nt: np.ndarray, offsets: np.ndarray) -> Tuple["DeviceBuffer", "DeviceBuffer", int]:
        nt = np.ascontiguousarray(nt, dtype=np.uint8)
        offsets = np.ascontiguousarray(offsets, dtype=np.uint64)
        n, n_nt = len(offsets) - 1, int(offsets[-1])
        if nt.size != n_nt:
            raise ValueError(f"offsets end at {n_nt}, the batch holds {nt.size} bases")
        d_nt = self.to_device(nt if n_nt else np.zeros(16, np.uint8))
        d_off = self.to_device(offsets)
        frames = self._device_empty(int(self._L.ks_translate6_bound(n_nt)) + 16)
        foff = self._device_empty(8 * (6 * n + 1))
        n_res = C.c_uint64(0)
        try:
            self._check(self._L.ks_translate6_device(self._h, d_nt._p, d_off._p, n, n_nt, frames._p, foff._p, C.byref(n_res)))
        finally:
            d_nt.free(); d_off.free()
        return frames, foff, int(n_res.value)

    def sketch_translated(self, nt: np.ndarray, offsets: np.ndarray, ksize: int, scaled: int, moltype: str,
                          seed: int = SEED) -> "Sketches":
        nt = np.ascontiguousarray(nt, dtype=np.uint8)
        offsets = np.ascontiguousarray(offsets, dtype=np.uint64)
        p = make_params(ksize, scaled, moltype, seed)
        out = C.c_void_p()
        self._check(self._L.ks_sketch_translated(self._h, _ptr(nt), _ptr(offsets), len(offsets) - 1, C.byref(p), C.byref(out)))
        return Sketches(self, out)

    def sketch_translated_device(self, d_nt: int, d_offsets: int, n_seqs: int, n_nt: int, ksize: int, scaled: int, moltype: str,
                                 max_seq_len: int = 0, seed: int = SEED) -> "Sketches":
        p = make_params(ksize, scaled, moltype, seed)
        out = C.c_void_p()
        self._check(self._L.ks_sketch_translated_device(self._h, C.c_void_p(d_nt), C.c_void_p(d_offsets), n_seqs, n_nt, max_seq_len,
                                                        C.byref(p), C.byref(out)))
        return Sketches(self, out)

    def qfilter_stats(self) -> Dict[str, int]:
        v = (C.c_uint64 * 2)()
        self._check(self._L.ks_ctx_qfilter_stats(self._h, C.byref(v)))
        return {"seen": int(v[0]), "dropped": int(v[1])}

    def fused_stats(self) -> Dict[str, int]:
        v = (C.c_uint64 * 2)()
        self._check(self._L.ks_ctx_fused_stats(self._h, C.byref(v)))
        return {"deferred": int(v[0]), "redos": int(v[1])}

    def sketches_from_host(self, offsets: np.ndarray, hashes: np.ndarray, abunds: np.ndarray, ksize: int,
                           scaled: int, moltype: str, seed: int = SEED) -> "Sketches":
        offsets = np.ascontiguousarray(offsets, dtype=np.uint64)
        hashes = np.ascontiguousarray(hashes, dtype=np.uint64)
        abunds = np.ascontiguousarray(abunds, dtype=np.uint32)
        p = make_params(ksize, scaled, moltype, seed)
        out = C.c_void_p()
        self._check(self._L.ks_sketches_from_host(self._h, _ptr(offsets), _ptr(hashes), _ptr(abunds),
                                                  len(offsets) - 1, C.byref(p), C.byref(out)))
        return Sketches(self, out)

    def kmer_positions(self, residues: np.ndarray, offsets: np.ndarray, ksize: int, scaled: int, moltype: str,
                       seed: int = SEED) -> Tuple[np.ndarray, np.ndarray, np.ndarray]:
        residues = np.ascontiguousarray(residues, dtype=np.uint8)
        offsets = np.ascontiguousarray(offsets, dtype=np.uint64)
        p = make_params(ksize, scaled, moltype, seed)
        out = C.c_void_p()
        self._check(self._L.ks_kmer_positions(self._h, _ptr(residues), _ptr(offsets), len(offsets) - 1, C.byref(p),
                                              C.byref(out)))
        try:
            n = int(self._L.ks_kmerpos_count(out))
            seq = np.zeros(n, np.uint32); start = np.zeros(n, np.uint32); h = np.zeros(n, np.uint64)
            self._check(self._L.ks_kmerpos_copy_to_host(self._h, out, _ptr(seq), _ptr(start), _ptr(h)))
        finally:
            self._L.ks_kmerpos_free(out)
        return seq, start, h

    def kmer_positions_device(self, d_residues: int, d_offsets: int, n_seqs: int, n_residues: int, ksize: int, scaled: int,
                              moltype: str, seed: int = SEED, fetch: bool = True):
        p = make_params(ksize, scaled, moltype, seed)
        out = C.c_void_p()
        self._check(self._L.ks_kmer_positions_device(self._h, C.c_void_p(d_residues), C.c_void_p(d_offsets), n_seqs, n_residues,
                                                     C.byref(p), C.byref(out)))
        try:
            n = int(self._L.ks_kmerpos_count(out))
            if not fetch:
                return n
            seq = np.zeros(n, np.uint32); start = np.zeros(n, np.uint32); h = np.zeros(n, np.uint64)
            self._check(self._L.ks_kmerpos_copy_to_host(self._h, out, _ptr(seq), _ptr(start), _ptr(h)))
        finally:
            self._L.ks_kmerpos_free(out)
        return seq, start, h

    def kmer_positions_table(self, residues: np.ndarray, offsets: np.ndarray, ksize: int, scaled: int, moltype: str,
                             seed: int = SEED) -> "KmerPositions":
        residues = np.ascontiguousarray(residues, dtype=np.uint8)
        offsets = np.ascontiguousarray(offsets, dtype=np.uint64)
        p = make_params(ksize, scaled, moltype, seed)
        out = C.c_void_p()
        self._check(self._L.ks_kmer_positions(self._h, _ptr(residues), _ptr(offsets), len(offsets) - 1, C.byref(p),
                                              C.byref(out)))
        return KmerPositions(self, out)

    def kmer_positions_table_device(self, d_residues: int, d_offsets: int, n_seqs: int, n_residues: int, ksize: int, scaled: int,
                                    moltype: str, seed: int = SEED) -> "KmerPositions":
        p = make_params(ksize, scaled, moltype, seed)
        out = C.c_void_p()
        self._check(self._L.ks_kmer_positions_device(self._h, C.c_void_p(d_residues), C.c_void_p(d_offsets), n_seqs, n_residues,
                                                     C.byref(p), C.byref(out)))
        return KmerPositions(self, out)

    def match_positions(self, q_pos: "KmerPositions", t_pos: "KmerPositions", hits: "Hits", max_pairs: int = 0) -> "MatchPositions":
        out = C.c_void_p()
        opts = _lib.ks_matchpos_opts(0, 0, int(max_pairs))
        self._check(self._L.ks_match_positions(self._h, q_pos._h, t_pos._h, hits._h, C.byref(opts), C.byref(out)))
        return MatchPositions(self, out)

    def match_regions(self, mp: "MatchPositions", max_gap: int = 0, min_kmers: int = 1) -> "Regions":
        for name, v in (("max_gap", max_gap), ("min_kmers", min_kmers)):
            if not 0 <= int(v) < 2 ** 32:
                raise ValueError(f"{name} = {v} does not fit 32 bits")
        out = C.c_void_p()
        opts = _lib.ks_regions_opts(0, int(min_kmers), int(max_gap), 0)
        self._check(self._L.ks_match_regions(self._h, mp._h, C.byref(opts), C.byref(out)))
        return Regions(self, out)

    def significance(self, queries: "Sketches", targets: "Sketches", hits: "Hits", q_corpus: Optional["Corpus"] = None,
                     t_corpus: Optional["Corpus"] = None) -> "Significance":
        own = []
        try:
            if q_corpus is None:
                q_corpus = queries.corpus(); own.append(q_corpus)
            if t_corpus is None:
                t_corpus = targets.corpus(); own.append(t_corpus)
            out = C.c_void_p()
            opts = _lib.ks_signif_opts(0, 0)
            self._check(self._L.ks_hits_significance(self._h, queries._h, targets._h, q_corpus._h, t_corpus._h, hits._h, C.byref(opts),
                                                     C.byref(out)))
            return Significance(self, out)
        finally:
            for c in own:
                c.free()

    def best_hits(self, hits: "Hits", k: int, rank_by: str = "intersect", queries: Optional["Sketches"] = None,
                  targets: Optional["Sketches"] = None, score=None) -> "Hits":
        if score is not None and rank_by == "intersect":
            rank_by = "score"
        if rank_by not in BEST_RANK_BY:
            raise ValueError(f"rank_by must be one of {', '.join(BEST_RANK_BY)}, not {rank_by!r}")
        if not 0 <= int(k) < 2 ** 32:
            raise ValueError(f"k = {k} does not fit 32 bits")
        d_score = None if score is None else C.c_void_p(int(score.data_ptr()) if hasattr(score, "data_ptr") else int(score))
        opts = _lib.ks_best_opts(BEST_RANK_BY[rank_by], int(k), 0, 0)
        out = C.c_void_p()
        self._check(self._L.ks_hits_best(self._h, hits._h, None if queries is None else queries._h,
                                         None if targets is None else targets._h, d_score, C.byref(opts), C.byref(out)))
        return Hits(self, out)

    def cluster(self, hits: "Hits", similarity: Optional[str] = None, threshold: float = 0.0, nodes: Optional["Sketches"] = None,
                score=None, n_nodes: int = 0) -> "Clusters":
        if similarity is None:
            similarity = "jaccard" if score is None else "score"
        if similarity not in BEST_RANK_BY:
            raise ValueError(f"similarity must be one of {', '.join(BEST_RANK_BY)}, not {similarity!r}")
        if not 0 <= int(n_nodes) < 2 ** 32:
            raise ValueError(f"n_nodes = {n_nodes} does not fit 32 bits")
        d_score = None if score is None else C.c_void_p(int(score.data_ptr()) if hasattr(score, "data_ptr") else int(score))
        opts = _lib.ks_cluster_opts(BEST_RANK_BY[similarity], int(n_nodes), float(threshold), 0, 0)
        out = C.c_void_p()
        self._check(self._L.ks_hits_cluster(self._h, hits._h, None if nodes is None else nodes._h, d_score, C.byref(opts),
                                            C.byref(out)))
        return Clusters(self, out)

    def cluster_greedy(self, hits: "Hits", similarity: Optional[str] = None, threshold: float = 0.0, nodes: Optional["Sketches"] = None,
                       score=None, n_nodes: int = 0, assign: str = "first") -> "Clusters":
        if similarity is None:
            similarity = "jaccard" if score is None else "score"
        if similarity not in BEST_RANK_BY:
            raise ValueError(f"similarity must be one of {', '.join(BEST_RANK_BY)}, not {similarity!r}")
        if assign not in GREEDY_ASSIGN:
            raise ValueError(f"assign must be one of {', '.join(GREEDY_ASSIGN)}, not {assign!r}")
        if not 0 <= int(n_nodes) < 2 ** 32:
            raise ValueError(f"n_nodes = {n_nodes} does not fit 32 bits")
        d_score = None if score is None else C.c_void_p(int(score.data_ptr()) if hasattr(score, "data_ptr") else int(score))
        opts = _lib.ks_greedy_opts(BEST_RANK_BY[similarity], int(n_nodes), float(threshold), GREEDY_ASSIGN[assign], 0)
        out = C.c_void_p()
        self._check(self._L.ks_hits_cluster_greedy(self._h, hits._h, None if nodes is None else nodes._h, d_score, C.byref(opts),
                                                   C.byref(out)))
        return Clusters(self, out)

    def gather(self, hits: "Hits", queries: "Sketches", targets: "Sketches", min_unique: int = 1, max_results: int = 0) -> "Hits":
        for name, v in (("min_unique", min_unique), ("max_results", max_results)):
            if not 0 <= int(v) < 2 ** 32:
                raise ValueError(f"{name} = {v} does not fit 32 bits")
        opts = _lib.ks_gather_opts(int(min_unique), int(max_results), 0, 0)
        out = C.c_void_p()
        self._check(self._L.ks_hits_gather(self._h, hits._h, queries._h, targets._h, C.byref(opts), C.byref(out)))
        return Hits(self, out)

    def index_build(self, targets: "Sketches") -> "Index":
        out = C.c_void_p()
        self._check(self._L.ks_index_build(self._h, targets._h, C.byref(out)))
# ... 409 lines not shown
```

Baseline: 58.23 billion.

## Aggregate query-target pairs in LDS hash tables after first MSD pass

Splits the MSD pair sort into a level-1 pass and a finish step. When the previous call's pairs-per-row ratio suggests few distinct rows, it skips the rest of the sort and aggregates (qid, tid) pairs per region with a workgroup-local hash table, emitting hit rows directly. If a region's table overflows, it falls back to finishing the sort and running the ordinary row kernel, and remembers the overflow size to avoid retrying. This trades the second-level sort passes for atomic-heavy shared-memory hashing, with extra work when the fallback is taken.

```diff
diff --git a/include/kmerseek_amd.h b/include/kmerseek_amd.h
--- a/include/kmerseek_amd.h
+++ b/include/kmerseek_amd.h
@@ -61,8 +61,8 @@
                       uint64_t *n_mallocs);
 
 int ks_ctx_sketch_stats(const ks_ctx *ctx, uint64_t out[4]);
-int ks_ctx_search_stats(const ks_ctx *ctx, uint64_t out[2]);
-int ks_ctx_fused_stats(const ks_ctx *ctx, uint64_t out[2]);
+int ks_ctx_search_stats(const ks_ctx *ctx, uint64_t out[4]);
+int ks_ctx_fused_stats(const ks_ctx *ctx, uint64_t out[3]);
 int ks_ctx_qfilter_stats(const ks_ctx *ctx, uint64_t out[2]);
 int ks_ctx_reload_debug_env(ks_ctx *ctx);
 int ks_debug_guard_selftest(const char *what);
diff --git a/kmerseek_amd/_lib.py b/kmerseek_amd/_lib.py
--- a/kmerseek_amd/_lib.py
+++ b/kmerseek_amd/_lib.py
@@ -96,8 +96,8 @@
     "ks_ctx_stream": (_vp, [_vp]),
     "ks_ctx_synchronize": (C.c_int, [_vp]),
     "ks_ctx_sketch_stats": (C.c_int, [_vp, C.POINTER(C.c_uint64 * 4)]),
-    "ks_ctx_search_stats": (C.c_int, [_vp, C.POINTER(C.c_uint64 * 2)]),
-    "ks_ctx_fused_stats": (C.c_int, [_vp, C.POINTER(C.c_uint64 * 2)]),
+    "ks_ctx_search_stats": (C.c_int, [_vp, C.POINTER(C.c_uint64 * 4)]),
+    "ks_ctx_fused_stats": (C.c_int, [_vp, C.POINTER(C.c_uint64 * 3)]),
     "ks_ctx_qfilter_stats": (C.c_int, [_vp, C.POINTER(C.c_uint64 * 2)]),
     "ks_ctx_reload_debug_env": (C.c_int, [_vp]),
     "ks_debug_guard_selftest": (C.c_int, [C.c_char_p]),
diff --git a/kmerseek_amd/csrc/ks_api.hip b/kmerseek_amd/csrc/ks_api.hip
--- a/kmerseek_amd/csrc/ks_api.hip
+++ b/kmerseek_amd/csrc/ks_api.hip
@@ -309,6 +309,7 @@
     const int fmt10 = (index->fp_layout && index->fp_shift == 32 - index->pbits) ? 1 : 0;
     ks_sketches *S = nullptr;
     ks_hits *H = nullptr;
+    const u64 agg_before = ctx->agg_used;
     int st = ks_sketch_device_impl(ctx, d_residues, d_seq_offsets, n_seqs, n_residues, max_seq_len, &index->params, index->pbits, fmt10,
                                    ks_dbg(ctx, KS_DBG_NO_DEFER) ? 0 : 1, &S);
     if (st != KS_OK) return st;
@@ -331,6 +332,7 @@
     }
     if (st != KS_OK) { ks_hits_free(H); ks_sketches_free(S); return st; }
     if (deferred) ctx->fused_deferred++;
+    if (ctx->agg_used > agg_before) ctx->fused_aggregated++;
     *hits_out = H;
     if (sketches_out) *sketches_out = S; else ks_sketches_free(S);
     return KS_OK;
diff --git a/kmerseek_amd/csrc/ks_common.h b/kmerseek_amd/csrc/ks_common.h
--- a/kmerseek_amd/csrc/ks_common.h
+++ b/kmerseek_amd/csrc/ks_common.h
@@ -40,7 +40,7 @@
     X(STAGED_H2D) X(PLAIN_COPIES) X(PAIRS_LSD) X(MSD_LDS_CAP) X(SCAN_3PASS) X(INDEX_LSD) X(JOIN_FP) X(FP_COARSEN)        \
     X(PAIR_LIMIT) X(PBITS_MAX) X(RECORD_BITS) X(ONE_CURSOR) X(JOIN_SEGS) X(JOIN_SEG_CAP) X(JOIN_SPARSE)                \
     X(NO_ROWS_HINT) X(ROWS_TICKET) X(FORCE_ROWS_TICKET_RETRY) X(FORCE_TICKET_RETRY) X(NO_PLAN) X(NO_COMPACT) X(SPAN)      \
-    X(NO_PACK) X(PLAN_SYNC) X(TILE_R) X(OUT_CAP) X(POOL_CAP) X(THROW) X(QCAP) X(LOOKBACK_SKIP) X(SYNC_API) X(POSTINGS12) X(POSTINGS10) X(NO_DEFER) X(BUCKET) X(JOIN_SPLIT) X(SUBSHIFT) X(MATCHPOS_ROW_BITS) X(SIGNIF_WAVE_ROWS) X(BEST_PATH) X(REGIONS_ROW_BITS) X(QFILTER) X(QFILTER_OCC) X(CLUSTER_PATH) X(GATHER_PATH) X(GREEDY_PATH) X(UNION_PATH)
+    X(NO_PACK) X(PLAN_SYNC) X(TILE_R) X(OUT_CAP) X(POOL_CAP) X(THROW) X(QCAP) X(LOOKBACK_SKIP) X(SYNC_API) X(POSTINGS12) X(POSTINGS10) X(NO_DEFER) X(BUCKET) X(JOIN_SPLIT) X(SUBSHIFT) X(MATCHPOS_ROW_BITS) X(SIGNIF_WAVE_ROWS) X(BEST_PATH) X(REGIONS_ROW_BITS) X(QFILTER) X(QFILTER_OCC) X(CLUSTER_PATH) X(GATHER_PATH) X(GREEDY_PATH) X(UNION_PATH) X(AGG_CAP) X(ROWS_PATH)
 enum ks_dbg_id {
 #define KS_DBG_ENUM(n) KS_DBG_##n,
     KS_DBG_LIST(KS_DBG_ENUM)
@@ -78,7 +78,10 @@
     u64 sketch_ticket_fallbacks = 0, sketch_compact_fallbacks = 0, sketch_cap_fallbacks = 0;
     bool rows_use_ticket = false; u64 rows_ticket_fallbacks = 0;
     u64 fused_deferred = 0, fused_redos = 0;
+    u64 fused_aggregated = 0;
     u64 join_retries = 0;
+    double rows_mult = 0.0;
+    u64 agg_used = 0, agg_overflows = 0, agg_oflow_rows = 0;
     bool qfilter_pays = true;
     u64 qfilter_seen = 0, qfilter_dropped = 0;
     unsigned long long *scan_ring = nullptr;
@@ -431,6 +434,16 @@
     u64 seg_cap;
 };
 int ks_sort_pairs_msd(ks_ctx *ctx, u64 *ka, u64 *kb, u64 n, int lo_bit, int nbits, int *done, const ks_msd_segs *segs = nullptr);
+#define KS_MSD_REGIONS 256
+struct ks_msd_plan {
+    u64 *ka, *kb, n;
+    int lo_bit, nbits;
+    u32 *blk;
+    const u32 *ends;
+};
+int ks_msd_level1(ks_ctx *ctx, u64 *ka, u64 *kb, u64 n, int lo_bit, int nbits, const ks_msd_segs *segs, ks_msd_plan *P);
+int ks_msd_finish(ks_ctx *ctx, ks_msd_plan *P);
+void ks_msd_drop(ks_ctx *ctx, ks_msd_plan *P);
 int ks_radix_sort_u64(ks_ctx *ctx, int tag, const u64 *keys_in, const u64 *vals_in, u64 *ka, u64 *va, u64 *kb, u64 *vb,
                       u64 n, const int *shifts, int n_shifts, u64 **keys_out, u64 **vals_out);
 
@@ -439,8 +452,11 @@
 int ks_row_list_alloc(ks_ctx *ctx, ks_scratch &sc, size_t n_rows, u32 **list);
 int ks_seg_list_alloc(ks_ctx *ctx, ks_scratch &sc, size_t cap, u32 **list);
 int ks_seg_path_knob(const ks_ctx *ctx, int dbg_id, bool *small);
-struct ks_rows_in { const ks_sketches *q; u64 n_pairs; int tbits, abits; bool stats; double min_c; };
+struct ks_rows_in { const ks_sketches *q; u64 n_pairs; int tbits, abits; bool stats; double min_c; int qbits; };
 int ks_search_rows(ks_ctx *ctx, const ks_rows_in &R, ks_hits *H, const u64 *pk);
+int ks_search_rows_agg(ks_ctx *ctx, const ks_rows_in &R, ks_hits *H, const ks_msd_plan &P, bool *fell_back);
+bool ks_rows_agg_wanted(const ks_ctx *ctx, const ks_rows_in &R);
+void ks_rows_agg_overflowed(ks_ctx *ctx, u64 n_rows);
 
 int ks_sketch_device_impl(ks_ctx *ctx, const u8 *d_res, const u64 *d_offs, u32 n_seqs, u64 n_res,
                           u32 max_seq_len, const ks_params *p, int part_pbits, int part_fmt10, int allow_defer, ks_sketches **out);
diff --git a/kmerseek_amd/csrc/ks_ctx.hip b/kmerseek_amd/csrc/ks_ctx.hip
--- a/kmerseek_amd/csrc/ks_ctx.hip
+++ b/kmerseek_amd/csrc/ks_ctx.hip
@@ -236,10 +236,11 @@
     });
 }
 
-extern "C" int ks_ctx_search_stats(const ks_ctx *ctx, uint64_t out[2]) {
+extern "C" int ks_ctx_search_stats(const ks_ctx *ctx, uint64_t out[4]) {
     return ks_guard((ks_ctx *)ctx, [&]() -> int {
     if (!ctx || !out) return KS_ERR_INVALID_ARG;
     out[0] = ctx->join_retries; out[1] = ctx->rows_ticket_fallbacks;
+    out[2] = ctx->agg_used; out[3] = ctx->agg_overflows;
     return KS_OK;
     });
 }
@@ -252,10 +253,10 @@
     });
 }
 
-extern "C" int ks_ctx_fused_stats(const ks_ctx *ctx, uint64_t out[2]) {
+extern "C" int ks_ctx_fused_stats(const ks_ctx *ctx, uint64_t out[3]) {
     return ks_guard((ks_ctx *)ctx, [&]() -> int {
     if (!ctx || !out) return KS_ERR_INVALID_ARG;
-    out[0] = ctx->fused_deferred; out[1] = ctx->fused_redos;
+    out[0] = ctx->fused_deferred; out[1] = ctx->fused_redos; out[2] = ctx->fused_aggregated;
     return KS_OK;
     });
 }
diff --git a/kmerseek_amd/csrc/ks_msd.hip b/kmerseek_amd/csrc/ks_msd.hip
--- a/kmerseek_amd/csrc/ks_msd.hip
+++ b/kmerseek_amd/csrc/ks_msd.hip
@@ -352,18 +352,72 @@
     }
 }
 
-int ks_sort_pairs_msd(ks_ctx *ctx, u64 *ka, u64 *kb, u64 n, int lo_bit, int nbits, int *done, const ks_msd_segs *segs) {
-    *done = 0;
-    if (nbits <= 16 || n < 65536 || n >= 0xffffffffULL || ks_dbg(ctx, KS_DBG_PAIRS_LSD)) return KS_OK;
+struct ms_layout {
+    int shift1, shift2;
+    u32 mask2, n_buckets, n_sub, sub_stride;
+    size_t off2_words, n_zero;
+};
+static ms_layout ms_layout_of(u64 n, int lo_bit, int nbits, int *bits2_out) {
     int bits2 = 0;
     while (bits2 < 9 && (n >> (8 + bits2)) > (bits2 < 8 ? 768u : 560u)) bits2++;
     for (int b = bits2 + 1; b <= 8 && nbits - 8 - b > 0; b++)
         if ((nbits - 8 - b + 7) / 8 < (nbits - 8 - bits2 + 7) / 8) { bits2 = b; break; }
     if (nbits - 8 - bits2 <= 0) bits2 = nbits - 9 > 0 ? nbits - 9 : 0;
-    const int shift1 = lo_bit + nbits - 8, shift2 = shift1 - bits2;
-    const u32 mask2 = (1u << (8 + bits2)) - 1u, n_buckets = 1u << (8 + bits2);
+    ms_layout L;
+    L.shift1 = lo_bit + nbits - 8; L.shift2 = L.shift1 - bits2;
+    L.mask2 = (1u << (8 + bits2)) - 1u; L.n_buckets = 1u << (8 + bits2);
+    L.n_sub = bits2 > 0 ? MS_SUB : 1u; L.sub_stride = bits2 > 0 ? 256u : 0u;
+    L.off2_words = bits2 > 0 ? (size_t)L.n_buckets + 1 : 0; L.n_zero = 256 * MS_SUB + L.off2_words + 1;
+    *bits2_out = bits2;
+    return L;
+}
+
+int ks_msd_level1(ks_ctx *ctx, u64 *ka, u64 *kb, u64 n, int lo_bit, int nbits, const ks_msd_segs *segs, ks_msd_plan *P) {
+    memset(P, 0, sizeof *P);
+    if (nbits <= 16 || n < 65536 || n >= 0xffffffffULL || ks_dbg(ctx, KS_DBG_PAIRS_LSD)) return KS_OK;
+    int bits2;
+    const ms_layout L = ms_layout_of(n, lo_bit, nbits, &bits2);
     const u32 n_tiles = (u32)((n + MS_TILE - 1) / MS_TILE);
     const u32 n_tiles1 = segs ? segs->tile_start[segs->n] : n_tiles;
+    ks_msd_segs no_segs;
+    no_segs.n = 0;
+    u32 *blk = nullptr;
+    KS_TRY(ks_alloc(ctx, &blk, L.n_zero + (size_t)(L.n_buckets > 65536u ? L.n_buckets : 65536u) + 1));
+    u32 *off1 = blk;
+    (void)hipMemsetAsync(blk, 0, L.n_zero * sizeof(u32), ctx->stream);
+    ks_timer_begin(ctx, "msd_hist");
+    if (segs) hipLaunchKernelGGL((k_msd_hist<256, 1>), dim3(n_tiles1), dim3(MS_THREADS), 0, ctx->stream, (const u64 *)ka, n, L.shift1, off1, 255u, 0, L.sub_stride, *segs);
+    else hipLaunchKernelGGL((k_msd_hist<256, 0>), dim3(n_tiles), dim3(MS_THREADS), 0, ctx->stream, (const u64 *)ka, n, L.shift1, off1, 255u, 0, L.sub_stride, no_segs);
+    ks_timer_end(ctx);
+    ks_timer_begin(ctx, "msd_scan");
+    hipLaunchKernelGGL(k_msd_scan256, dim3(1), dim3(256), 0, ctx->stream, off1, L.n_sub);
+    ks_timer_end(ctx);
+    ks_timer_begin(ctx, "msd_scatter");
+    if (segs) hipLaunchKernelGGL((k_msd_scatter<256, 1>), dim3(n_tiles1), dim3(MS_THREADS), 0, ctx->stream, (const u64 *)ka, kb, n, L.shift1, off1, 255u, 0,
+                                 L.sub_stride, *segs);
+    else hipLaunchKernelGGL((k_msd_scatter<256, 0>), dim3(n_tiles), dim3(MS_THREADS), 0, ctx->stream, (const u64 *)ka, kb, n, L.shift1, off1, 255u, 0,
+                            L.sub_stride, no_segs);
+    ks_timer_end(ctx);
+    P->ka = ka; P->kb = kb; P->n = n;
+    P->lo_bit = lo_bit; P->nbits = nbits;
+    P->blk = blk;
+    P->ends = off1 + (size_t)(L.n_sub - 1u) * 256u;
+    return KS_OK;
+}
+
+void ks_msd_drop(ks_ctx *ctx, ks_msd_plan *P) {
+    ks_pool_free(ctx, P->blk);
+    P->blk = nullptr;
+}
+
+int ks_msd_finish(ks_ctx *ctx, ks_msd_plan *P) {
+    u64 *const ka = P->ka, *const kb = P->kb;
+    const u64 n = P->n;
+    const int lo_bit = P->lo_bit;
+    int bits2;
+    const ms_layout L = ms_layout_of(n, lo_bit, P->nbits, &bits2);
+    const u32 n_tiles = (u32)((n + MS_TILE - 1) / MS_TILE);
+    const u32 n_buckets = L.n_buckets;
     ks_msd_segs no_segs;
     no_segs.n = 0;
     u32 lds_cap = ML_CAP;
@@ -371,40 +425,20 @@
         const u32 v = (u32)atoi(f);
         if (v >= 2 && v < ML_CAP) lds_cap = v;
     }
-    u32 *blk = nullptr;
-    const u32 n_sub = bits2 > 0 ? MS_SUB : 1u, sub_stride = bits2 > 0 ? 256u : 0u;
-    const size_t off2_words = bits2 > 0 ? (size_t)n_buckets + 1 : 0, n_zero = 256 * MS_SUB + off2_words + 1;
-    int st = ks_alloc(ctx, &blk, n_zero + (size_t)(n_buckets > 65536u ? n_buckets : 65536u) + 1);
-    u32 *off1 = blk, *off2 = blk ? blk + 256 * MS_SUB : nullptr, *big = blk ? blk + 256 * MS_SUB + off2_words : nullptr;
-    u64 *sorted_in = ka;
-    if (st == KS_OK) {
-        (void)hipMemsetAsync(blk, 0, n_zero * sizeof(u32), ctx->stream);
+    u32 *const blk = P->blk, *off1 = blk, *off2 = blk + 256 * MS_SUB, *big = blk + 256 * MS_SUB + L.off2_words;
+    int st = KS_OK;
+    u64 *sorted_in = kb;
+    const u32 *off = off1;
+    if (bits2 > 0) {
         ks_timer_begin(ctx, "msd_hist");
-        if (segs) hipLaunchKernelGGL((k_msd_hist<256, 1>), dim3(n_tiles1), dim3(MS_THREADS), 0, ctx->stream, (const u64 *)ka, n, shift1, off1, 255u, 0, sub_stride, *segs);
-        else hipLaunchKernelGGL((k_msd_hist<256, 0>), dim3(n_tiles), dim3(MS_THREADS), 0, ctx->stream, (const u64 *)ka, n, shift1, off1, 255u, 0, sub_stride, no_segs);
-        ks_timer_end(ctx);
-        ks_timer_begin(ctx, "msd_scan");
-        hipLaunchKernelGGL(k_msd_scan256, dim3(1), dim3(256), 0, ctx->stream, off1, n_sub);
-        ks_timer_end(ctx);
-        ks_timer_begin(ctx, "msd_scatter");
-        if (segs) hipLaunchKernelGGL((k_msd_scatter<256, 1>), dim3(n_tiles1), dim3(MS_THREADS), 0, ctx->stream, (const u64 *)ka, kb, n, shift1, off1, 255u, 0,
-                                     sub_stride, *segs);
-        else hipLaunchKernelGGL((k_msd_scatter<256, 0>), dim3(n_tiles), dim3(MS_THREADS), 0, ctx->stream, (const u64 *)ka, kb, n, shift1, off1, 255u, 0,
-                                sub_stride, no_segs);
-        ks_timer_end(ctx);
-        sorted_in = kb;
-    }
-    const u32 *off = off1;
-    if (st == KS_OK && bits2 > 0) {
-        ks_timer_begin(ctx, "msd_hist");
-        if (bits2 <= 8) hipLaunchKernelGGL((k_msd_hist<512>), dim3(n_tiles), dim3(MS_THREADS), 0, ctx->stream, (const u64 *)kb, n, shift2, off2, mask2, bits2, 0u, no_segs);
-        else hipLaunchKernelGGL((k_msd_hist<1024>), dim3(n_tiles), dim3(MS_THREADS), 0, ctx->stream, (const u64 *)kb, n, shift2, off2, mask2, bits2, 0u, no_segs);
+        if (bits2 <= 8) hipLaunchKernelGGL((k_msd_hist<512>), dim3(n_tiles), dim3(MS_THREADS), 0, ctx->stream, (const u64 *)kb, n, L.shift2, off2, L.mask2, bits2, 0u, no_segs);
+        else hipLaunchKernelGGL((k_msd_hist<1024>), dim3(n_tiles), dim3(MS_THREADS), 0, ctx->stream, (const u64 *)kb, n, L.shift2, off2, L.mask2, bits2, 0u, no_segs);
         ks_timer_end(ctx);
         st = ks_scan_u32_inplace(ctx, off2, n_buckets, nullptr);
         if (st == KS_OK) {
             ks_timer_begin(ctx, "msd_scatter");
-            if (bits2 <= 8) hipLaunchKernelGGL((k_msd_scatter<512>), dim3(n_tiles), dim3(MS_THREADS), 0, ctx->stream, (const u64 *)kb, ka, n, shift2, off2, mask2, bits2, 0u, no_segs);
-            else hipLaunchKernelGGL((k_msd_scatter<1024>), dim3(n_tiles), dim3(MS_THREADS), 0, ctx->stream, (const u64 *)kb, ka, n, shift2, off2, mask2, bits2, 0u, no_segs);
+            if (bits2 <= 8) hipLaunchKernelGGL((k_msd_scatter<512>), dim3(n_tiles), dim3(MS_THREADS), 0, ctx->stream, (const u64 *)kb, ka, n, L.shift2, off2, L.mask2, bits2, 0u, no_segs);
+            else hipLaunchKernelGGL((k_msd_scatter<1024>), dim3(n_tiles), dim3(MS_THREADS), 0, ctx->stream, (const u64 *)kb, ka, n, L.shift2, off2, L.mask2, bits2, 0u, no_segs);
             ks_timer_end(ctx);
             sorted_in = ka;
             off = off2;
@@ -414,18 +448,27 @@
         u64 *other = sorted_in == ka ? kb : ka;
         ks_timer_begin(ctx, "msd_local");
         hipLaunchKernelGGL(k_msd_local, dim3((n_buckets + ML_WAVES - 1) / ML_WAVES), dim3(ML_THREADS), 0, ctx->stream, sorted_in, off,
-                           n_buckets, lo_bit, shift2 - lo_bit, lds_cap, big);
+                           n_buckets, lo_bit, L.shift2 - lo_bit, lds_cap, big);
         ks_timer_end(ctx);
         ks_timer_begin(ctx, "msd_local_big");
         hipLaunchKernelGGL(k_msd_local_big, dim3(n_buckets < 2048 ? n_buckets : 2048), dim3(ML_THREADS), 0, ctx->stream, sorted_in, other, off,
-                           (const u32 *)big, lo_bit, shift2 - lo_bit, lds_cap);
+                           (const u32 *)big, lo_bit, L.shift2 - lo_bit, lds_cap);
         ks_timer_end(ctx);
         if (sorted_in != ka)
             if (hipMemcpyAsync(ka, kb, (size_t)n * sizeof(u64), hipMemcpyDeviceToDevice, ctx->stream) != hipSuccess)
                 st = ks_fail(ctx, KS_ERR_HIP, "msd sort: copy back failed");
         if (st == KS_OK && hipGetLastError() != hipSuccess) st = ks_fail(ctx, KS_ERR_HIP, "msd sort launch failed");
-        if (st == KS_OK) *done = 1;
-    }
-    ks_pool_free(ctx, blk);
+    }
+    ks_msd_drop(ctx, P);
     return st;
 }
+
+int ks_sort_pairs_msd(ks_ctx *ctx, u64 *ka, u64 *kb, u64 n, int lo_bit, int nbits, int *done, const ks_msd_segs *segs) {
+    *done = 0;
+    ks_msd_plan P;
+    KS_TRY(ks_msd_level1(ctx, ka, kb, n, lo_bit, nbits, segs, &P));
+    if (!P.blk) return KS_OK;
+    KS_TRY(ks_msd_finish(ctx, &P));
+    *done = 1;
+    return KS_OK;
+}
diff --git a/kmerseek_amd/csrc/ks_rows.hip b/kmerseek_amd/csrc/ks_rows.hip
--- a/kmerseek_amd/csrc/ks_rows.hip
+++ b/kmerseek_amd/csrc/ks_rows.hip
@@ -146,6 +146,155 @@
     }
 }
 
+#define AG_THREADS 1024
+#define AG_IPT 8
+#define AG_SLOTS 4096
+#define AG_EMPTY (~0ULL)
+static_assert(AG_SLOTS % AG_THREADS == 0 && (AG_SLOTS & (AG_SLOTS - 1)) == 0, "the bitonic network walks a power of two");
+
+KS_DEV bool ag_insert(unsigned long long *keys, unsigned long long *sums, u32 *cnts, u32 *n_used, unsigned long long k,
+                      unsigned long long w, u32 slot, u32 n_slots) {
+    for (u32 p = 0; p < n_slots; p++) {
+        unsigned long long cur = __hip_atomic_load(&keys[slot], __ATOMIC_RELAXED, __HIP_MEMORY_SCOPE_WORKGROUP);
+        if (cur == AG_EMPTY) {
+            cur = atomicCAS(&keys[slot], AG_EMPTY, k);
+            if (cur == AG_EMPTY) { atomicAdd(n_used, 1u); cur = k; }
+        }
+        if (cur == k) {
+            atomicAdd(&cnts[slot], 1u);
+            atomicAdd(&sums[slot], w);
+            return true;
+        }
+        slot = slot + 1 == n_slots ? 0 : slot + 1;
+    }
+    return false;
+}
+
+__global__ __launch_bounds__(AG_THREADS) void k_pairs_aggregate(const u64 *list, const u32 *ends, u32 n_slots, u32 *qid, u32 *tid, u32 *isect,
+                                                                unsigned long long *nw, int tbits, int abits, u32 rows_cap,
+                                                                unsigned long long *status,
+                                                                u32 *ctl ) {
+    __shared__ unsigned long long keys[AG_SLOTS];
+    __shared__ unsigned long long sums[AG_SLOTS];
+    __shared__ u32 cnts[AG_SLOTS];
+    __shared__ u32 n_used, n_packed, oflow;
+    __shared__ unsigned long long base_s;
+    const u32 tid_ = threadIdx.x, lane = tid_ & 63, wave = tid_ >> 6, region = blockIdx.x;
+    for (u32 i = tid_; i < AG_SLOTS; i += AG_THREADS) { keys[i] = AG_EMPTY; sums[i] = 0; cnts[i] = 0; }
+    if (tid_ == 0) { n_used = 0; n_packed = 0; oflow = 0; }
+    const u64 s = region ? ends[region - 1] : 0, e = ends[region];
+    const u64 am = (1ULL << abits) - 1ULL;
+    const u64 last = e ? e - 1 : 0;
+    u64 nxt[AG_IPT];
+#pragma unroll
+    for (int r = 0; r < AG_IPT; r++) {
+        const u64 i = s + (u64)r * AG_THREADS + tid_;
+        nxt[r] = list[i < e ? i : last];
+    }
+    __syncthreads();
+    for (u64 t0 = s; t0 < e; t0 += AG_THREADS * AG_IPT) {
+        u64 rec[AG_IPT];
+#pragma unroll
+        for (int r = 0; r < AG_IPT; r++) rec[r] = nxt[r];
+#pragma unroll
+        for (int r = 0; r < AG_IPT; r++) {
+            const u64 i = t0 + (u64)(AG_IPT + r) * AG_THREADS + tid_;
+            nxt[r] = list[i < e ? i : last];
+        }
+        if (*(volatile u32 *)&oflow) break;
+        u32 slot[AG_IPT];
+        unsigned long long seen[AG_IPT];
+#pragma unroll
+        for (int r = 0; r < AG_IPT; r++) {
+            const unsigned long long k = rec[r] >> abits;
+            slot[r] = __umulhi((u32)((k * 0x9E3779B97F4A7C15ULL) >> 32), n_slots);
+            seen[r] = __hip_atomic_load(&keys[slot[r]], __ATOMIC_RELAXED, __HIP_MEMORY_SCOPE_WORKGROUP);
+        }
+#pragma unroll
+        for (int r = 0; r < AG_IPT; r++) {
+            const u64 i = t0 + (u64)r * AG_THREADS + tid_;
+            if (i >= e) continue;
+            const unsigned long long k = rec[r] >> abits, w = rec[r] & am;
+            if (seen[r] == k) {
+                atomicAdd(&cnts[slot[r]], 1u);
+                atomicAdd(&sums[slot[r]], w);
+            } else if (!ag_insert(keys, sums, cnts, &n_used, k, w, slot[r], n_slots)) {
+                oflow = 1u;
+            }
+        }
+    }
+    __syncthreads();
+    const u32 groups = oflow ? 0u : n_used;
+    if (tid_ == 0) {
+        if (oflow) atomicOr(&ctl[0], 1u);
+        __hip_atomic_store(&status[region], (region == 0 ? KS_LB_PRE : KS_LB_AGG) | (u64)groups, __ATOMIC_RELAXED, __HIP_MEMORY_SCOPE_AGENT);
+    }
+    if (groups > 0) {
+        unsigned long long ck[AG_SLOTS / AG_THREADS], cs[AG_SLOTS / AG_THREADS];
+        u32 cc[AG_SLOTS / AG_THREADS];
+#pragma unroll
+        for (int j = 0; j < AG_SLOTS / AG_THREADS; j++) {
+            const u32 i = (u32)j * AG_THREADS + tid_;
+            ck[j] = keys[i]; cs[j] = sums[i]; cc[j] = cnts[i];
+        }
+        u32 p2 = 1;
+        while (p2 < groups) p2 <<= 1;
+        __syncthreads();
+#pragma unroll
+        for (int j = 0; j < AG_SLOTS / AG_THREADS; j++) {
+            const bool occ = ck[j] != AG_EMPTY;
+            const u64 m = __ballot(occ);
+            u32 b = 0;
+            if (lane == 0 && m) b = atomicAdd(&n_packed, (u32)__popcll(m));
+            b = (u32)__builtin_amdgcn_readfirstlane((int)b);
+            if (occ) {
+                const u32 d = b + ks_lane_lt_count(m);
+                keys[d] = ck[j]; sums[d] = cs[j]; cnts[d] = cc[j];
+            }
+        }
+        for (u32 i = groups + tid_; i < p2; i += AG_THREADS) keys[i] = AG_EMPTY;
+        __syncthreads();
+        for (u32 k2 = 2; k2 <= p2; k2 <<= 1) {
+            for (u32 j = k2 >> 1; j > 0; j >>= 1) {
+                for (u32 t = tid_; t < p2 / 2; t += AG_THREADS) {
+                    const u32 i = ((t & ~(j - 1)) << 1) | (t & (j - 1)), o = i | j;
+                    const unsigned long long a = keys[i], b = keys[o];
+                    if ((a > b) == ((i & k2) == 0) && a != b) {
+                        keys[i] = b; keys[o] = a;
+                        const unsigned long long sa = sums[i]; sums[i] = sums[o]; sums[o] = sa;
+                        const u32 ca = cnts[i]; cnts[i] = cnts[o]; cnts[o] = ca;
+                    }
+                }
+                __syncthreads();
+            }
+        }
+    }
+    if (wave == 0) {
+        u64 excl = 0;
+        if (region > 0) {
+            excl = ks_lookback_walk(region, lane, ks_lookback_words(status), &ctl[1]);
+            if (lane == 0)
+                __hip_atomic_store(&status[region], KS_LB_PRE | (excl + groups), __ATOMIC_RELAXED, __HIP_MEMORY_SCOPE_AGENT);
+        }
+        if (lane == 0) {
+            base_s = excl;
+            if (region == gridDim.x - 1) ctl[2] = (u32)(excl + groups);
+        }
+    }
+    __syncthreads();
+    const u64 base = base_s;
+    for (u32 i = tid_; i < groups; i += AG_THREADS) {
+        const u64 row = base + i;
+        if (row < rows_cap) {
+            const unsigned long long k = keys[i];
+            qid[row] = (u32)(k >> tbits);
+            tid[row] = (u32)(k & ((1ULL << tbits) - 1ULL));
+            isect[row] = cnts[i];
+            nw[row] = sums[i];
+        }
+    }
+}
+
 #define RA_LONG 64
 
 __global__ __launch_bounds__(256) void k_row_abund_stats(const u64 *pk, const u64 *row_start, const u32 *isect, const u32 *n_rows_dev,
@@ -280,10 +429,36 @@
     return KS_OK;
 }
 
-static int se_rows_run(ks_ctx *ctx, const ks_rows_in &Q, ks_hits *H, ks_hits &F, const u64 *pk) {
+#define KS_AGG_MIN_MULT 8.0
+#define KS_AGG_REGION_ROWS (AG_SLOTS / 2)
+
+bool ks_rows_agg_wanted(const ks_ctx *ctx, const ks_rows_in &Q) {
+    if (Q.stats || Q.n_pairs == 0) return false;
+    if (const char *f = ks_dbg(ctx, KS_DBG_ROWS_PATH)) return strcmp(f, "agg") == 0;
+    if (ks_dbg(ctx, KS_DBG_MSD_LDS_CAP) || ks_dbg(ctx, KS_DBG_ROWS_TICKET) || ks_dbg(ctx, KS_DBG_FORCE_ROWS_TICKET_RETRY)) return false;
+    if (!(ctx->rows_mult > KS_AGG_MIN_MULT)) return false;
+    const u32 n_q = Q.q->n_seqs;
+    const int qbits = Q.qbits;
+    const u64 regions = qbits >= 8 && n_q ? ((u64)(n_q - 1) >> (qbits - 8)) + 1 : (u64)KS_MSD_REGIONS;
+    const double rows = (double)Q.n_pairs / ctx->rows_mult;
+    if (ctx->agg_oflow_rows && rows * 2.0 > (double)ctx->agg_oflow_rows) return false;
+    return rows <= (double)(regions * KS_AGG_REGION_ROWS);
+}
+
+void ks_rows_agg_overflowed(ks_ctx *ctx, u64 n_rows) {
+    if (ks_dbg(ctx, KS_DBG_ROWS_PATH)) return;
+    if (!ctx->agg_oflow_rows || n_rows < ctx->agg_oflow_rows) ctx->agg_oflow_rows = n_rows ? n_rows : 1;
+}
+
+static int se_rows_run(ks_ctx *ctx, const ks_rows_in &Q, ks_hits *H, ks_hits &F, const u64 *pk, const ks_msd_plan *A, bool *fell_back) {
     const u64 n_pairs = Q.n_pairs;
     const int tbits = Q.tbits, abits = Q.abits;
-    const u32 pf_tiles = (u32)((n_pairs + PF_TILE - 1) / PF_TILE);
+    const u32 pf_tiles = A ? (u32)KS_MSD_REGIONS : (u32)((n_pairs + PF_TILE - 1) / PF_TILE);
+    u32 agg_slots = AG_SLOTS;
+    if (const char *f = ks_dbg(ctx, KS_DBG_AGG_CAP)) {
+        const long v = atol(f);
+        if (v >= 1 && v < AG_SLOTS) agg_slots = (u32)v;
+    }
     u64 rows_cap = n_pairs;
     if (ctx->rows_hint && ctx->rows_hint < rows_cap && !ks_dbg(ctx, KS_DBG_NO_ROWS_HINT)) rows_cap = ctx->rows_hint;
     u32 n_rows = 0;
@@ -299,13 +474,23 @@
         unsigned long long *const pf_status = (unsigned long long *)(H->d_block + rows_cap);
         u32 *const pf_ticket = (u32 *)(pf_status + pf_tiles);
         KS_HIP(ctx, hipMemsetAsync(H->d_block, 0, ((size_t)rows_cap + st_words + is_words) * sizeof(u64), ctx->stream));
-        KS_LAUNCH(ctx, "pair_rows", k_pair_rows_fused, pf_tiles, PF_THREADS, pk, n_pairs, H->d_qid, H->d_tid, H->d_isect,
-                  (unsigned long long *)H->d_nw, tbits, abits, (u32)rows_cap, pf_status, pf_ticket, pf_ticket + 2,
-                  (ctx->rows_use_ticket || ks_dbg(ctx, KS_DBG_ROWS_TICKET)) ? 1 : 0);
+        if (A)
+            KS_LAUNCH(ctx, "pairs_aggregate", k_pairs_aggregate, pf_tiles, AG_THREADS, (const u64 *)A->kb, A->ends, agg_slots, H->d_qid,
+                      H->d_tid, H->d_isect, (unsigned long long *)H->d_nw, tbits, abits, (u32)rows_cap, pf_status, pf_ticket);
+        else
+            KS_LAUNCH(ctx, "pair_rows", k_pair_rows_fused, pf_tiles, PF_THREADS, pk, n_pairs, H->d_qid, H->d_tid, H->d_isect,
+                      (unsigned long long *)H->d_nw, tbits, abits, (u32)rows_cap, pf_status, pf_ticket, pf_ticket + 2,
+                      (ctx->rows_use_ticket || ks_dbg(ctx, KS_DBG_ROWS_TICKET)) ? 1 : 0);
         if (post) KS_TRY(se_rows_post(ctx, Q, H, &F, pk, (u32)rows_cap, pf_ticket, sc));
         KS_TRY(ks_stream_wait_fetch_scans(ctx, {ks_fetch_words(pf_ticket, ctx->h_pin + KS_PIN_ROWS, 4)}));
+        if (A && (pin[0] != 0 || pin[1] != 0)) {
+            se_free_cols(ctx, H);
+            se_free_cols(ctx, &F);
+            *fell_back = true;
+            return KS_OK;
+        }
         bool gave_up = pin[1] != 0;
-        if (ks_dbg(ctx, KS_DBG_FORCE_ROWS_TICKET_RETRY) && !ctx->rows_use_ticket) gave_up = true;
+        if (!A && ks_dbg(ctx, KS_DBG_FORCE_ROWS_TICKET_RETRY) && !ctx->rows_use_ticket) gave_up = true;
         if (gave_up) {
             if (ctx->rows_use_ticket || attempt == 2) return ks_fail(ctx, KS_ERR_HIP, "search: row look-back gave up waiting for a predecessor tile");
             ctx->rows_use_ticket = true;
@@ -322,6 +507,8 @@
     H->n_hits = n_rows;
     const u64 want = (u64)n_rows + n_rows / 4 + 4096;
     ctx->rows_hint = want > ctx->rows_hint / 2 ? want : ctx->rows_hint / 2;
+    ctx->rows_mult = (double)n_pairs / (double)(n_rows ? n_rows : 1u);
+    if (A) ctx->agg_used++;
     if (Q.min_c > 0) {
         se_free_cols(ctx, H);
         H->d_qid = F.d_qid; H->d_tid = F.d_tid; H->d_isect = F.d_isect; H->d_nw = F.d_nw;
@@ -336,7 +523,16 @@
     if (Q.n_pairs == 0) return ks_hits_alloc_cols(ctx, H, 0, 0);
     ks_hits F;
     memset(&F, 0, sizeof F);
-    const int st = se_rows_run(ctx, Q, H, F, pk);
+    const int st = se_rows_run(ctx, Q, H, F, pk, nullptr, nullptr);
+    se_free_cols(ctx, &F);
+    return st;
+}
+
+int ks_search_rows_agg(ks_ctx *ctx, const ks_rows_in &Q, ks_hits *H, const ks_msd_plan &P, bool *fell_back) {
+    *fell_back = false;
+    ks_hits F;
+    memset(&F, 0, sizeof F);
+    const int st = se_rows_run(ctx, Q, H, F, nullptr, &P, fell_back);
     se_free_cols(ctx, &F);
     return st;
 }
diff --git a/kmerseek_amd/csrc/ks_search.hip b/kmerseek_amd/csrc/ks_search.hip
--- a/kmerseek_amd/csrc/ks_search.hip
+++ b/kmerseek_amd/csrc/ks_search.hip
@@ -1105,7 +1105,7 @@
     return KS_OK;
 }
 
-static int se_sort(ks_ctx *ctx, se_search &Q, ks_scratch &sc, u64 **pk) {
+static int se_sort(ks_ctx *ctx, se_search &Q, ks_scratch &sc, u64 **pk, ks_msd_plan *agg) {
     const u64 n_pairs = Q.n_pairs;
     const u32 n_segs = Q.n_segs;
     const int tbits = Q.tbits, qbits = Q.qbits, abits = Q.abits;
@@ -1123,7 +1123,14 @@
         }
         sg.tile_start[n_segs] = t;
         for (u32 s_ = n_segs + 1; s_ <= KS_MSD_MAX_SEGS; s_++) sg.tile_start[s_] = t;
+        if (agg) {
+            KS_TRY(ks_msd_level1(ctx, Q.pk0, Q.pk1, n_pairs, lo_bit, nbits, &sg, agg));
+            if (agg->blk) return KS_OK;
+        }
         KS_TRY(ks_sort_pairs_msd(ctx, Q.pk0, Q.pk1, n_pairs, lo_bit, nbits, &msd, &sg));
+    } else if (agg) {
+        KS_TRY(ks_msd_level1(ctx, Q.pk0, Q.pk1, n_pairs, lo_bit, nbits, nullptr, agg));
+        if (agg->blk) return KS_OK;
     }
     if (n_segs > 1 && !msd) {
         jn_seg_table tab;
@@ -1146,7 +1153,7 @@
     return ks_radix_sort_keys(ctx, KS_SORT_PAIRS, Q.pk0, Q.pk0, Q.pk1, n_pairs, shifts, ns, pk);
 }
 
-static ks_rows_in se_rows_in(const se_search &Q) { return ks_rows_in{Q.q, Q.n_pairs, Q.tbits, Q.abits, Q.stats, Q.min_c}; }
+static ks_rows_in se_rows_in(const se_search &Q) { return ks_rows_in{Q.q, Q.n_pairs, Q.tbits, Q.abits, Q.stats, Q.min_c, Q.qbits}; }
 
 struct se_split {
     u64 pairs;
@@ -1227,7 +1234,22 @@
     const u64 want = Q.n_pairs + Q.n_pairs / 8;
     ctx->pair_cap_hint = want > ctx->pair_cap_hint / 2 ? want : ctx->pair_cap_hint / 2;
     u64 *pk = nullptr;
-    if (Q.n_pairs) KS_TRY(se_sort(ctx, Q, sc, &pk));
+    struct agg_plan : ks_msd_plan {
+        ks_ctx *c;
+        explicit agg_plan(ks_ctx *c_) : ks_msd_plan{}, c(c_) {}
+        ~agg_plan() { ks_msd_drop(c, this); }
+    } A(ctx);
+    if (Q.n_pairs) KS_TRY(se_sort(ctx, Q, sc, &pk, ks_rows_agg_wanted(ctx, se_rows_in(Q)) ? &A : nullptr));
+    if (A.blk) {
+        bool fell_back = false;
+        KS_TRY(ks_search_rows_agg(ctx, se_rows_in(Q), H, A, &fell_back));
+        if (!fell_back) return KS_OK;
+        ctx->agg_overflows++;
+        KS_TRY(ks_msd_finish(ctx, &A));
+        KS_TRY(ks_search_rows(ctx, se_rows_in(Q), H, A.ka));
+        ks_rows_agg_overflowed(ctx, (u64)((double)Q.n_pairs / ctx->rows_mult));
+        return KS_OK;
+    }
     return ks_search_rows(ctx, se_rows_in(Q), H, pk);
 }
 
diff --git a/kmerseek_amd/engine.py b/kmerseek_amd/engine.py
--- a/kmerseek_amd/engine.py
+++ b/kmerseek_amd/engine.py
@@ -195,10 +195,13 @@
     def reload_debug_env(self):
         self._check(self._L.ks_ctx_reload_debug_env(self._h))
 
-    def search_stats(self) -> Dict[str, int]:
-        v = (C.c_uint64 * 2)()
+    def search_stats(self, paths: bool = False) -> Dict[str, int]:
+        v = (C.c_uint64 * 4)()
         self._check(self._L.ks_ctx_search_stats(self._h, C.byref(v)))
-        return {"join_retries": int(v[0]), "rows_ticket_fallbacks": int(v[1])}
+        out = {"join_retries": int(v[0]), "rows_ticket_fallbacks": int(v[1]), "agg_overflows": int(v[3])}
+        if paths:
+            out["agg_used"] = int(v[2])
+        return out
 
     def sketch_batch(self, residues: np.ndarray, offsets: np.ndarray, ksize: int, scaled: int, moltype: str,
                      seed: int = SEED) -> "Sketches":
@@ -295,9 +298,9 @@
         return {"seen": int(v[0]), "dropped": int(v[1])}
 
     def fused_stats(self) -> Dict[str, int]:
-        v = (C.c_uint64 * 2)()
+        v = (C.c_uint64 * 3)()
         self._check(self._L.ks_ctx_fused_stats(self._h, C.byref(v)))
-        return {"deferred": int(v[0]), "redos": int(v[1])}
+        return {"deferred": int(v[0]), "redos": int(v[1]), "aggregated": int(v[2])}
 
     def sketches_from_host(self, offsets: np.ndarray, hashes: np.ndarray, abunds: np.ndarray, ksize: int,
                            scaled: int, moltype: str, seed: int = SEED) -> "Sketches":
```

Result: faster. 61.74 billion (median of 6 runs) (+6.0%).
